# urgent-challenge/urgent2026_challenge_track1

Hardware: AMD Instinct MI355X
Metric: utterances/sec (4 s @ 48 kHz) train step (higher is better)
Workload: dtype bf16

## Files before the change

### include/urse.h

```cpp
#ifndef URSE_H_
#define URSE_H_
#include <stdint.h>

#ifdef __cplusplus
extern "C" {
#endif

#define URSE_OK 0
#define URSE_ERR_INVALID_ARG (-1)
#define URSE_ERR_LAUNCH (-2)
#define URSE_ERR_UNSUPPORTED (-3)
#define URSE_ERR_RUNTIME (-4)

#define URSE_F32 0
#define URSE_BF16 1
#define URSE_F16 2
#define URSE_BF16_ACT_F16 3

#define URSE_WIN_RECT 0
#define URSE_WIN_HANN 1

int urse_version(void);
const char* urse_last_error(void);

#define URSE_KV_NT_BRES 0
#define URSE_KV_NT_RING 1
#define URSE_KV_NT_RING_WIDE 2
#define URSE_KV_NT_128 3
#define URSE_KV_NT_GROUPED_RING 4
#define URSE_KV_NT_GROUPED_128 5
#define URSE_KV_TN_RING 6
#define URSE_KV_TN_RING_T 7
#define URSE_KV_TN_DUAL 8
#define URSE_KV_TN_128 9
#define URSE_KV_TN_GROUPED 10
#define URSE_KV_LSTM_FWD_STREAM 11
#define URSE_KV_LSTM_FWD_WIDE 12
#define URSE_KV_LSTM_FWD_CLUSTER 13
#define URSE_KV_LSTM_FWD_CLUSTER2 14
#define URSE_KV_LSTM_BWD_STREAM16 15
#define URSE_KV_LSTM_BWD_STREAM32 16
#define URSE_KV_LSTM_BWD_CLUSTER 17
#define URSE_KV_LSTM_BWD_SPLIT 18
#define URSE_KV_STFT960 19
#define URSE_KV_STFT_GENERIC 20
#define URSE_KV_ISTFT_GENERIC 21
#define URSE_KV_ISTFT960 22
#define URSE_KV_LSTM_FWD_RW 23
#define URSE_KV_TN_ACT_F16 24
#define URSE_KV_LSTM_FWD_RWX 25
#define URSE_KV_LSTM_BWD_NSPLIT 26
#define URSE_KV_LSTM_FWD_CLUSTERX 27
#define URSE_KV_COUNT 32
int urse_launch_count(int variant);
int urse_launch_counts_reset(void);

int urse_stft_fwd(const float* wav, const int32_t* lens, float* spec, int B, int L, int n_fft, int hop,
                  int window, void* stream);
int urse_istft_fwd(const float* spec, float* wav, int B, int T, int n_fft, int hop, int L_out, int window,
                   void* stream);
int urse_istft_bwd(const float* grad_wav, float* grad_spec, int B, int T, int n_fft, int hop, int L_out,
                   int window, void* stream);

int urse_gemm_nt(const void* A, int64_t lda, const void* B, int64_t ldb, void* C, int64_t ldc, const float* bias,
                 const float* resid, int64_t ldr, int64_t M, int64_t N, int64_t K, int in_dtype, int out_dtype,
                 int act, void* stream);
int urse_gemm_nt_gnstats(const void* A, int64_t lda, const void* B, int64_t ldb, float* C, int64_t ldc, const float* bias,
                         const float* resid, int64_t ldr, int64_t M, int64_t N, int64_t K, int in_dtype, int act,
                         double* stats, int64_t rows_per_group, void* stream);
int urse_gemm_nt_gnbwd(const void* A, int64_t lda, const void* B, int64_t ldb, float* C, int64_t M, int64_t N, int64_t K, int in_dtype,
                       const float* x, const double* stats, const float* gamma, double* sums, float* dgamma, float* dbeta, float* part,
                       int slots, int64_t rows_per_group, float eps, void* stream);
int urse_gemm_nt_grouped(const void* descs, int groups, int max_blocks, int in_dtype, int out_dtype, int act,
                         void* stream);
int urse_gemm_nt_grouped_h(const void* descs, const int64_t* host_descs, int groups, int in_dtype, int out_dtype,
                           int act, void* stream);
int urse_gemm_tn(const void* A, int64_t lda, const void* B, int64_t ldb, float* C, int64_t ldc, float* colsum,
                 int64_t R, int64_t Mo, int64_t No, int64_t shift, int64_t inner, int64_t period,
                 int64_t invalid_step, int64_t perm_h, int dtype, int target_workgroups, void* stream);
int urse_gemm_tn_act_f16_supported(int64_t R, int64_t Mo, int64_t No, int64_t No2, int with_colsum, int64_t inner, int64_t period);
int urse_gemm_tn_dual(const void* A, int64_t lda, const void* B, int64_t ldb, float* C, int64_t ldc, float* colsum,
                      const void* B2, int64_t ldb2, float* C2, int64_t ldc2, int64_t R, int64_t Mo, int64_t No, int64_t No2,
                      int64_t shift, int64_t inner, int64_t period, int64_t invalid_step, int64_t perm_h, int dtype,
                      int target_workgroups, void* stream);
int urse_gemm_tn_grouped(const void* descs, int groups, int max_blocks, int dtype, void* stream);

int urse_groupnorm_fwd(const float* x, const float* gamma, const float* beta, const float* add, void* y, double* stats,
                       int B, int T, int Kg, int W, int N, int Np, int gstride, float eps, int out_dtype, void* y_bf16, void* stream);
int urse_groupnorm_stats(const float* x, double* stats, int B, int T, int Kg, int W, int N, void* stream);
int urse_groupnorm_apply(const float* x, const float* gamma, const float* beta, const float* add, void* y, const double* stats,
                         int B, int T, int Kg, int W, int N, int Np, int gstride, float eps, int out_dtype, void* y_bf16, void* stream);
int urse_groupnorm_bwd(const float* x, const float* dy, const double* stats, const float* gamma, const float* dres,
                       float* dx, float* dgamma, float* dbeta, double* sums, int B, int T, int Kg, int W, int N,
                       int gstride, float eps, void* dx_packed, int ldp, void* stream);
int urse_groupnorm_bwd_apply(const float* x, const float* dy, const double* stats, const double* sums, const float* gamma,
                             const float* dres, float* dx, int B, int T, int Kg, int W, int N, int gstride, float eps, void* dx_packed,
                             int ldp, void* stream);
int urse_pack2d(const void* in, int64_t ldi, int in_dtype, void* out, int64_t ldo, int out_dtype, int rows, int cols,
                int out_rows, int out_cols, int transpose, void* stream);

int urse_pack_segments(const float* in, void* out, const void* segs, int nseg, int blocks_per_seg, int transpose,
                       int out_dtype, void* stream);

int urse_lstm_pack(const float* wih, const float* whh, const float* bih, const float* bhh, void* wih_p, void* wihT_p,
                   float* bias, void* whh_frag, void* whhT_frag, int N, int Np, int H, int Hp, int dtype,
                   void* stream);

int urse_lstm_bidir_fwd(void* gx, int64_t ldg, const void* whh, void* hout, int64_t ldh, float* c, int H, int Hp,
                        int n_seq, int seq_len, int64_t inner, int64_t outer, int64_t stride, int save, int dtype,
                        int rows16, void* hout_bf16, void* stream);
int urse_lstm_pack_quads(const float* whh, void* out, int H, int Hp, int dtype, void* stream);
int urse_lstm_cluster_plan(int H, int Hp, int n_seq, int reserved_cus, int64_t* plan);
int urse_lstm_cluster_fwd(void* gx, int64_t ldg, const void* whhq, void* hout, int64_t ldh, float* c, void* hx,
                          void* counters, void* err_flag, int H, int Hp, int n_seq, int seq_len, int64_t inner,
                          int64_t outer, int64_t stride, int save, int reserved_cus, int xcd_aware, int dtype, void* hout_bf16,
                          void* stream);
int urse_lstm_clusterx_supported(int N, int Np, int H, int Hp);
int urse_lstm_clusterx_plan(int H, int Hp, int n_seq, int reserved_cus, int64_t* plan);
int urse_lstm_clusterx_hx_elems(int H, int Hp, int n_seq, int reserved_cus, int64_t* elems);
int urse_lstm_pack_quads_x(const float* wih, void* out, int N, int Np, int H, int dtype, void* stream);
int urse_lstm_clusterx_fwd(const void* xn, int64_t ldx, const void* wihq, const float* bias, const void* whhq, void* gates, int64_t ldg, void* hout,
                           int64_t ldh, float* c, void* hx, void* counters, void* err_flag, int N, int Np, int H, int Hp, int n_seq, int seq_len,
                           int64_t inner, int64_t outer, int64_t stride, int save, int reserved_cus, int xcd_aware, int dtype, void* hout_bf16,
                           void* stream);
int urse_lstm_cluster2_plan(int H, int Hp, int n_seq, int reserved_cus, int64_t* plan);
int urse_lstm_cluster2_fwd(void* gx, int64_t ldg, const void* whhq, void* hout, int64_t ldh, float* c, void* hx, void* err_flag,
                           int H, int Hp, int n_seq, int seq_len, int64_t inner, int64_t outer, int64_t stride, int save,
                           int reserved_cus, int dtype, void* stream);
int urse_lstm_pack_bwd_quads(const float* whh, void* out, int H, int C, void* stream);
int urse_lstm_cluster_bwd(const void* dh, int64_t ldd, void* gates, int64_t ldg, const float* c, const void* whhTq,
                          void* dgx, void* counters, void* err_flag, int H, int Hp, int n_seq, int seq_len, int64_t inner,
                          int64_t outer, int64_t stride, int reserved_cus, void* stream);
int urse_lstm_wide_supported(int H, int Hp);
int urse_lstm_pack_blocks(const float* whh, void* out, int H, int Hp, void* stream);
int urse_lstm_wide_fwd(void* gx, int64_t ldg, const void* whhb, void* hout, int64_t ldh, float* c, int H, int Hp,
                       int n_seq, int seq_len, int64_t inner, int64_t outer, int64_t stride, int save, void* stream);
int urse_lstm_rw_supported(int H, int Hp);
int urse_lstm_pack_blocks_rw(const float* whh, void* out, int H, int Hp, void* stream);
int urse_lstm_rw_fwd(void* gx, int64_t ldg, const void* whhb, void* hout, int64_t ldh, float* c, int H, int Hp,
                     int n_seq, int seq_len, int64_t inner, int64_t outer, int64_t stride, int save,
                     int target_workgroups, int paired, void* stream);
int urse_lstm_pack_multi(const void* table, int n_lstm, int N, int Np, int H, int Hp, int dtype, void* stream);
int urse_lstm_pack_quads_multi(const void* table, int n_lstm, int H, int Hp, int dtype, void* stream);
int urse_lstm_pack_quads_x_multi(const void* table, int n_lstm, int N, int Np, int H, int dtype, void* stream);
int urse_lstm_pack_blocks_multi(const void* table, int n_lstm, int H, int Hp, void* stream);
int urse_lstm_pack_blocks_x_multi(const void* table, int n_lstm, int N, int Np, int H, int Hp, int dtype, void* stream);
int urse_lstm_rwx_supported(int N, int Np, int H, int Hp);
int urse_lstm_pack_blocks_x(const float* wih, const float* whh, void* out, int N, int Np, int H, int Hp, int dtype, void* stream);
int urse_lstm_rwx_fwd(const void* xn, int64_t ldx, const void* wx, const float* bias, void* gates, int64_t ldg, void* hout,
                      int64_t ldh, float* c, int N, int Np, int H, int Hp, int n_seq, int seq_len, int64_t inner,
                      int64_t outer, int64_t stride, int save, int target_workgroups, int dtype, void* hout_bf16, void* stream);
int urse_lstm_split_plan(int H, int n_seq, int reserved_cus, int64_t* plan);
int urse_lstm_split_bwd(const void* dh, int64_t ldd, void* gates, int64_t ldg, const float* c, const void* whhT, void* xbuf,
                        void* err_flag, int H, int n_seq, int seq_len, int64_t inner, int64_t outer, int64_t stride,
                        int reserved_cus, void* stream);
int urse_lstm_nsplit_plan(int H, int n_seq, int reserved_cus, int64_t* plan);
int urse_lstm_nsplit_bwd(const void* dh, int64_t ldd, void* gates, int64_t ldg, const float* c, const void* whhT, void* flags,
                         void* err_flag, int H, int n_seq, int seq_len, int64_t inner, int64_t outer, int64_t stride,
                         int reserved_cus, void* stream);
int urse_lstm_bidir_bwd(const void* dh, int64_t ldd, void* gates, int64_t ldg, const float* c, const void* whhT,
                        int H, int n_seq, int seq_len, int64_t inner, int64_t outer, int64_t stride, int dtype,
                        int rows16, void* stream);

int urse_bandsplit_norm_fwd(const float* spec, const int32_t* bands, const float* gamma, const float* beta, void* xnb,
                            double* stats, int B, int T, int F, int K, int ldx, float eps, int out_dtype,
                            void* xnb_bf16, void* stream);
int urse_bandsplit_norm_bwd(const float* spec, const float* dxnb, const int32_t* bands, const double* stats,
                            float* dgamma, float* dbeta, int B, int T, int F, int K, int ldx, float eps,
                            void* stream);
int urse_glu_mask_apply_fwd(const float* pre_m, const float* pre_r, const float* x, float* out,
                            const int32_t* bands, const int32_t* f2k, int64_t rows, int F, int ldp, void* stream);
int urse_glu_mask_apply_bwd(const float* pre_m, const float* pre_r, const float* x, const float* dout, void* dpre_m,
                            void* dpre_r, const int32_t* bands, const int32_t* f2k, int64_t rows, int F, int ldp,
                            int out_dtype, void* stream);
int urse_peak_normalize(float* x, int64_t n, float peak, void* scratch, void* stream);
int urse_nonsilence_power(const float* x, const int32_t* lens, int B, int64_t ld, double threshold, double* hop_scratch,
                          double* power, void* stream);
int urse_mix_noise(const float* speech, const float* noise_raw, const int32_t* noise_lens, int64_t ldn, const int32_t* lens,
                   const int32_t* offsets, const float* snr_db, int B, int64_t ld, float* noise_out, float* noisy_out,
                   double* scratch, void* stream);
int urse_fir_full(const float* x, const int32_t* lens, int B, int64_t ld, const float* taps, const int32_t* ntaps, int64_t ldt,
                  int taps_per_utt, float* y, void* stream);
int urse_fft_convolve_workspace_bytes(int B, int max_len, int max_ntaps, int64_t* bytes);
int urse_fft_convolve(const float* x, const int32_t* lens, int B, int64_t ld, const float* taps, const int32_t* ntaps, int64_t ldt,
                      int taps_per_utt, float* y, int max_len, int max_ntaps, void* workspace, int64_t workspace_bytes, void* stream);
int urse_filtfilt_fir(const float* x, const int32_t* lens, int B, int64_t ld, const float* taps, const int32_t* ntaps_dev,
                      int ntaps, float* y, float* scratch, int64_t lds, void* stream);
int urse_quantile_clip(float* x, const int32_t* lens, int B, int64_t ld, const float* qmin, const float* qmax, float* bounds,
                       void* stream);
int urse_zero_segments(float* x, int64_t ld, const int32_t* segments, int nseg, void* stream);
int urse_resample_table(const float* x, int64_t ldx, float* y, int64_t ldy, const double* win, const double* delta, int nwin, int P,
                        int n_orig, int n_out, double time_increment, double scale, int num_table, int index_step, void* stream);
int urse_joint_peak_scale(float* speech, float* noisy, float* noise, int B, int64_t ld, float target, void* peak_scratch,
                          void* stream);
int urse_wind_mix(float* speech, const float* x, float* noise, float* noisy, const int32_t* lens, int B, int64_t ld, const int32_t* rows,
                  int nrows, const double* params, double* c_out, void* stream);
int urse_wind_chunk(void);
int urse_axpby(const float* x, float* y, float a, float b, int64_t n, void* stream);
int urse_nan_to_num(const float* x, float* y, int64_t n, void* stream);
int urse_scale_by_device_scalar(float* x, const float* s, int64_t n, void* stream);

int urse_pair_sums(const float* target, const float* estimate, double* sums, int B, int L, void* stream);
int urse_mrl1_loss_fwd(const float* target, const float* estimate, float* loss, float* G, double* sums, double* acc,
                       int B, int L, const int32_t* windows, int n_windows, float eps, float td_weight, void* stream);
int urse_mrl1_loss_bwd(const float* target, const float* estimate, const float* G, const double* sums,
                       const float* grad_loss, float* grad_estimate, double* c1, int B, int L, float eps,
                       void* stream);
int urse_mrl1_loss_bwd_guarded(const float* target, const float* estimate, const float* G, const double* sums,
                               const float* grad_loss, const float* loss, float* grad_estimate, double* c1, int B,
                               int L, float eps, void* stream);
int urse_sisnr_fwd(const float* ref, const float* inf, float* loss, double* sums, int B, int L, void* stream);
int urse_grad_sumsq(const float* g, double* out, int64_t n, void* stream);
int urse_clip_adamw_step(float* params, float* grads, float* exp_avg, float* exp_avg_sq, int64_t n,
                         const double* normsq, float max_norm, float lr, float beta1, float beta2, float eps,
                         float weight_decay, int step, float grad_scale, int zero_grad, void* stream);
int urse_clip_adamw_step_slots(float* params, float* grads, float* exp_avg, float* exp_avg_sq, int64_t n,
                               const double* normsq, float max_norm, float lr, float beta1, float beta2, float eps,
                               float weight_decay, const uint8_t* slot, float* used, int32_t* steps, float* bias_corr,
                               int n_slot, const uint32_t* skip_flag, float grad_scale, int zero_grad, void* stream);
int urse_fill_used_flags(float* used, int n_slot, int n_used, void* stream);

int urse_fft_resample_plan_elems(int n, int64_t* elems, int64_t* tmp_elems);
int urse_fft_resample_plan(void* plan, void* tmp, int n, void* stream);
int urse_fft_resample_workspace_bytes(int P, int n, int num, int64_t* bytes);
int urse_fft_resample(const float* x, int64_t ldx, float* y, int64_t ldy, const void* plan_n, const void* plan_num,
                      void* workspace, int64_t workspace_bytes, int P, int n, int num, void* stream);
int urse_resample_poly(const float* x, float* y, const double* h_padded, int hlen, int P, int L, int Lout, int up,
                       int down, int n_pre_remove, void* stream);
int urse_estoi_batch(const float* ref10k, const float* inf10k, float* out, float* ws_x, float* ws_y, float* tob_x,
                     float* tob_y, int32_t* lens, const float* tw512, int P, int L, void* stream);
int urse_sdr_batch(const float* ref, const float* est, float* out, double* acf, double* xcorr, double* norms, int P,
                   int L, float clamp_db, void* stream);

int urse_power_spectrum_workspace_bytes(int64_t rows, int max_len, int n_fft, int hop, int64_t* bytes);
int urse_power_spectrum_mean(const float* wav, int64_t ld, const int32_t* lens, float* mean_power, int64_t rows,
                             int max_len, int n_fft, int hop, void* workspace, int64_t workspace_bytes, void* stream);
int urse_bandwidth_pick(const float* mean_power, const int32_t* row_start, int32_t* bin, int P, int F,
                        double threshold_db, void* stream);

int urse_spec_transform(const float* x, float* y, int64_t n_complex, float exponent, float factor, int inverse,
                        void* stream);
int urse_flow_prepare(const float* x0, const float* y, const float* z, const float* t, float* xt, float* cvf, int B,
                      int64_t per_b, float sigma_min, float sigma_max, void* stream);
int urse_axpy(const float* x, float* y, float a, int64_t n, void* stream);
int urse_time_embedding(const float* t, const float* W, float* out, int B, int half, void* stream);
int urse_conv5x5_fwd(const float* U, const float* W, const float* bias, float* pre, int B, int T, int F, void* stream);
int urse_conv5x5_bwd(const float* U, const float* W, const float* dpre, float* dU, float* dW, float* dbias, int B, int T,
                     int F, void* stream);
int urse_glu4_apply_fwd(const float* pre_m, const float* pre_r, const float* x, float* out, int64_t rows, int F,
                        int Fs, float sign, void* stream);
int urse_glu4_apply_bwd(const float* pre_m, const float* pre_r, const float* x, const float* dout, float* dpre_m,
                        float* dpre_r, int64_t rows, int F, int Fs, float sign, void* stream);
int urse_tanh_bwd_pack(const float* dU, const float* U, void* dst, int64_t rows, int n, int64_t ldd, int out_dtype,
                       void* stream);
int urse_flow_loss(const float* vf, const float* cvf, double* loss, float* grad, int B, int64_t per_b, float grad_scale,
                   void* stream);
int urse_ema_update(float* shadow, const float* params, float one_minus_decay, int64_t n, void* stream);

#define URSE_PESQ_TRACE 286
int urse_pesq_workspace_bytes(int pairs, int L, int fs, int64_t* bytes);
int urse_pesq_batch(const float* ref, const float* deg, int64_t ld, const int32_t* lens, int pairs, int L, int fs, int wb,
                    float* mos, float* raw, int32_t* trace, void* workspace, int64_t workspace_bytes, void* stream);

int urse_flac_info(const void* data, int64_t nbytes, int64_t* info);
int urse_flac_decode(const void* data, int64_t nbytes, int32_t* out, int64_t capacity_frames, int64_t* decoded);

int urse_pcm16_from_f32(const float* x, int64_t ldx, const int32_t* lens, int16_t* pcm, int64_t ldp, int64_t rows,
                        int max_len, float scale, void* stream);
int urse_flac_encode_workspace_bytes(const int32_t* lens, int P, int blocksize, int64_t* info);
int urse_flac_encode(const int16_t* pcm, int64_t total_samples, const int64_t* starts, const int32_t* lens,
                     const int32_t* rates, int P, int channels, int bits, int blocksize, void* workspace,
                     int64_t workspace_bytes, void* out, int64_t out_capacity, int64_t* file_bytes, int32_t* frame_bytes,
                     void* stream);

int urse_diag_stream(void* buf, float* sink, int64_t bytes, int width, int write, void* stream);

#ifdef __cplusplus
}
#endif
#endif
```

### urgent2026_challenge_track1_amd/bsrnn.py

```python
import math
import os

import numpy as np
import torch
import torch.nn as nn

from . import ops
from ._lib import call, stream_ptr

SUBBANDS_481 = tuple([5] + [4] * 19 + [10] * 6 + [40] * 7 + [60])
SUBBANDS_769 = tuple([5] + [4] * 26 + [10] * 10 + [50] * 10 + [60])
_DIAG_SKIP_WGRADS = os.environ.get("URSE_DIAG_SKIP_WGRADS", "0") == "1"
GN_EPS = 1e-5


def _ptr(t, off_elems=0):
    return t.data_ptr() + off_elems * t.element_size()


class _PackPlan:

    def __init__(self, transpose):
        self.transpose = transpose
        self.segs = []
        self.size = 0
        self._table = None
        self._out = {}

    def add(self, in_off, in_rows, in_cols, out_rows, out_cols):
        off = self.size
        self.segs.append([in_off, in_rows, in_cols, in_cols, off, out_rows, out_cols, out_cols])
        self.size += (out_rows * out_cols + 31) // 32 * 32
        return (off, out_rows, out_cols)

    def reserve(self, n):
        off = self.size
        self.size += (n + 31) // 32 * 32
        return off

    def add_at(self, in_off, in_rows, in_cols, out_off, out_rows, out_cols, out_ld):
        self.segs.append([in_off, in_rows, in_cols, in_cols, out_off, out_rows, out_cols, out_ld])

    def run(self, flat, dtype):
        if not self.segs:
            return None
        if self._table is None or self._table.device != flat.device:
            self._table = torch.tensor(self.segs, dtype=torch.int64, device=flat.device)
        key = (dtype, flat.device)
        if key not in self._out:
            self._out[key] = torch.empty(self.size, dtype=dtype, device=flat.device)
        out = self._out[key]
        big = max(s[5] * s[6] for s in self.segs)
        call("pack_segments", flat, out, self._table, len(self.segs), max(1, min(64, (big + 2047) // 2048)),
             int(self.transpose), ops._dt(out), stream_ptr())
        return out


def _view(buf, h):
    off, r, c = h
    return buf[off:off + r * c].view(r, c)


def _empty_padded(K, M, ld, n, dtype, device):
    t = torch.empty(K, M, ld, dtype=dtype, device=device)
    if ld > n:
        t[:, :, n:].zero_()
    return t


def nt_grouped(rows, device, in_dt, out_dt, act=0):
    host = np.asarray(rows, dtype=np.int64)
    assert host.ndim == 2 and host.shape[1] == 12
    call("gemm_nt_grouped_h", ops.upload(torch.from_numpy(host), device), host.ctypes.data, host.shape[0], in_dt, out_dt, act,
         stream_ptr())


class BSRNNCore(nn.Module):

    def __init__(self, input_dim=481, num_channel=16, num_layer=6, target_fs=48000, causal=False, num_spk=1,
                 compute_dtype=torch.bfloat16):
        super().__init__()
        if causal or num_spk != 1:
            raise NotImplementedError("the reference uses causal=False, num_spk=1 (models/bsrnn.py:27-34)")
        if target_fs != 48000 or input_dim not in (481, 769):
            raise NotImplementedError("band tables defined for input_dim 481 / 769 @ 48 kHz (bsrnn_flowse.py:23-40)")
        if num_channel % 4:
            raise ValueError("num_channel must be a multiple of 4")
        self.subbands = SUBBANDS_481 if input_dim == 481 else SUBBANDS_769
        self.input_dim, self.N, self.H, self.num_layer = input_dim, num_channel, 2 * num_channel, num_layer
        self.compute_dtype = compute_dtype
        N, H = self.N, self.H
        self._make_front_back()
        self.norm_time = nn.ModuleList([nn.GroupNorm(1, N) for _ in range(num_layer)])
        self.rnn_time = nn.ModuleList([nn.LSTM(N, H, batch_first=True, bidirectional=True) for _ in range(num_layer)])
        self.fc_time = nn.ModuleList([nn.Linear(2 * H, N) for _ in range(num_layer)])
        self.norm_freq = nn.ModuleList([nn.GroupNorm(1, N) for _ in range(num_layer)])
        self.rnn_freq = nn.ModuleList([nn.LSTM(N, H, batch_first=True, bidirectional=True) for _ in range(num_layer)])
        self.fc_freq = nn.ModuleList([nn.Linear(2 * H, N) for _ in range(num_layer)])
        self._flat = None
        self._flat_grad = None
        self._off = {}
        self._plans = None
        self._tables = {}
        self._packed = None
        self._packed_version = -1
        self.param_version = 0
        self.grad_ready_hook = None
        self._deferred, self._inflight, self._side = [], None, None
        self._grad_pack = None
        self._gn_stats = None

    def _make_band_split(self):
        bs = nn.Module()
        bs.norm = nn.ModuleList([nn.GroupNorm(1, 2 * sb) for sb in self.subbands])
        bs.fc = nn.ModuleList([nn.Conv1d(2 * sb, self.N, 1) for sb in self.subbands])
        return bs

    def _make_front_back(self):
        N = self.N
        self.band_split = self._make_band_split()
        md = nn.Module()
        mk = lambda sb: nn.Sequential(nn.GroupNorm(1, N), nn.Conv1d(N, 4 * N, 1), nn.Tanh(),
                                      nn.Conv1d(4 * N, 4 * sb, 1), nn.GLU(dim=1))
        md.mlp_mask = nn.ModuleList([mk(sb) for sb in self.subbands])
        md.mlp_residual = nn.ModuleList([mk(sb) for sb in self.subbands])
        self.mask_decoder = md

    @staticmethod
    def _bs_params(prefix, bs):
        return [(prefix + ".gamma", [m.weight for m in bs.norm]), (prefix + ".beta", [m.bias for m in bs.norm]),
                (prefix + ".w", [m.weight for m in bs.fc]), (prefix + ".b", [m.bias for m in bs.fc])]

    def _front_params(self):
        return self._bs_params("bs", self.band_split)

    def _back_params(self):
        order = []
        for tag, mlps in (("m", self.mask_decoder.mlp_mask), ("r", self.mask_decoder.mlp_residual)):
            p = "md%s." % tag
            order += [(p + "gamma", [s[0].weight for s in mlps]), (p + "beta", [s[0].bias for s in mlps]),
                      (p + "w1", [s[1].weight for s in mlps]), (p + "b1", [s[1].bias for s in mlps]),
                      (p + "w2", [s[3].weight for s in mlps]), (p + "b2", [s[3].bias for s in mlps])]
        return order

    back_tag = "md"
    band_groups = ("bs", "mdm", "mdr")

    def _ordered_params(self):
        L = self.num_layer
        order = list(self._front_params())
        for l in range(L):
            for path, norm, rnn, fc in (("t", self.norm_time[l], self.rnn_time[l], self.fc_time[l]),
                                        ("f", self.norm_freq[l], self.rnn_freq[l], self.fc_freq[l])):
                p = "l%d%s." % (l, path)
                order += [(p + "gamma", [norm.weight]), (p + "beta", [norm.bias]),
                          (p + "wih", [rnn.weight_ih_l0, rnn.weight_ih_l0_reverse]),
                          (p + "bih", [rnn.bias_ih_l0, rnn.bias_ih_l0_reverse]),
                          (p + "bhh", [rnn.bias_hh_l0, rnn.bias_hh_l0_reverse]),
                          (p + "whh", [rnn.weight_hh_l0, rnn.weight_hh_l0_reverse]),
                          (p + "wfc", [fc.weight]), (p + "bfc", [fc.bias])]
        return order + list(self._back_params())

    def _ensure_flat(self):
        first = next(self.parameters())
        if self._flat is not None and self._flat.device == first.device and \
                first.data_ptr() == self._flat.data_ptr() + 4 * self._first_off:
            return
        order = self._ordered_params()
        total = 0
        offs = {}
        plist = []
        for name, ps in order:
            total = (total + 3) // 4 * 4
            offs[name] = total
            for p in ps:
                plist.append((p, total))
                total += p.numel()
        assert len(plist) == len([q for q in self.parameters() if q.requires_grad])
        nb = len(self.subbands)
        slot = np.zeros(total, dtype=np.uint8)
        for name, ps in order:
            if len(ps) == nb and name.split(".")[0] in self.band_groups:
                o = offs[name]
                for k, q in enumerate(ps):
                    slot[o:o + q.numel()] = 1 + k
                    o += q.numel()
        self.n_slot = 1 + nb
        self._slot_map = torch.from_numpy(slot).to(first.device)
        flat = torch.zeros(total, dtype=torch.float32, device=first.device)
        self._n_params = total
        grad = torch.zeros(total + (self.n_slot + 3) // 4 * 4, dtype=torch.float32, device=first.device)
        with torch.no_grad():
            for p, o in plist:
                flat[o:o + p.numel()].copy_(p.data.reshape(-1).float())
                p.data = flat[o:o + p.numel()].view(p.shape)
                p.grad = grad[o:o + p.numel()].view(p.shape)
        self._flat, self._flat_grad, self._off = flat, grad, offs
        self._first_off = [o for p, o in plist if p is first][0]
        self._plans = None
        self._packed_version = -1
        self._tables = {}

    @property
    def flat_params(self):
        self._ensure_flat()
        return self._flat

    @property
    def flat_grads(self):
        self._ensure_flat()
        return self._flat_grad

    @property
    def used_flags(self):
        self._ensure_flat()
        return self._flat_grad[self._n_params:self._n_params + self.n_slot]

    @property
    def slot_map(self):
        self._ensure_flat()
        return self._slot_map

    def mark_used_bands(self, K):
        call("fill_used_flags", self.used_flags, self.n_slot, 1 + K, stream_ptr())

    def grad_groups(self):
        self._ensure_flat()
        names = list(self._off.keys())
        ends = [self._off[n] for n in names[1:]] + [self._flat_grad.numel()]
        spans = {n: (self._off[n], e - self._off[n]) for n, e in zip(names, ends)}
        groups = []

        def span(ns):
            lo = min(spans[n][0] for n in ns)
            hi = max(spans[n][0] + spans[n][1] for n in ns)
            return lo, hi - lo
        is_layer = lambda n: n[0] == "l" and n[1].isdigit()
        first = min(i for i, n in enumerate(names) if is_layer(n))
        last = max(i for i, n in enumerate(names) if is_layer(n))
        groups.append((self.back_tag,) + span(names[last + 1:]))
        for l in reversed(range(self.num_layer)):
            groups.append(("l%df" % l,) + span([n for n in names if n.startswith("l%df." % l)]))
            groups.append(("l%dt" % l,) + span([n for n in names if n.startswith("l%dt." % l)]))
        groups.append(("bs",) + span(names[:first]))
        return groups

    def _g(self, name, numel=None, off=0):
        o = self._off[name] + off
        n = numel if numel is not None else 0
        return self._flat_grad[o:o + n] if numel is not None else self._flat_grad[o:]

    def _p(self, name, numel, off=0):
        o = self._off[name] + off
        return self._flat[o:o + numel]

    def _ready(self, tag):
        if self.grad_ready_hook is not None:
            self.grad_ready_hook(tag)

    def _build_plans(self, dtype):
        N, H = self.N, self.H
        Np, Hp = ops.kpad(N, dtype), ops.kpad(ops.pad_to(H, 16), dtype)
        ld2H, ld4N = ops.kpad(2 * H, dtype), ops.kpad(4 * N, dtype)
        pn, pt = _PackPlan(False), _PackPlan(True)
        h = {}
        o = self._off
        self._dims = dict(Np=Np, Hp=Hp, ld2H=ld2H, ld4N=ld4N)
        self._plan_front(pn, pt, h, dtype)
        for l in range(self.num_layer):
            for path in "tf":
                p = "l%d%s." % (l, path)
                h[p + "wfc"] = pn.add(o[p + "wfc"], N, 2 * H, N, ld2H)
                h[p + "wfcT"] = pt.add(o[p + "wfc"], N, 2 * H, 2 * H, Np)
        self._plan_back(pn, pt, h, dtype)
        self._plans = (dtype, pn, pt, h)

    def _plan_band_split(self, prefix, pn, pt, h, dtype):
        N, Np, o = self.N, self._dims["Np"], self._off
        w_off = 0
        for k, sb in enumerate(self.subbands):
            xpad = ops.kpad(2 * sb, dtype)
            h[prefix + ".w", k] = pn.add(o[prefix + ".w"] + w_off, N, 2 * sb, N, xpad)
            h[prefix + ".wT", k] = pt.add(o[prefix + ".w"] + w_off, N, 2 * sb, 2 * sb, Np)
            w_off += N * 2 * sb

    def _plan_front(self, pn, pt, h, dtype):
        self._plan_band_split("bs", pn, pt, h, dtype)

    def _plan_back(self, pn, pt, h, dtype):
        N, Np, ld4N, o = self.N, self._dims["Np"], self._dims["ld4N"], self._off
        for tag in "mr":
            p = "md%s." % tag
            w2_off = 0
            for k, sb in enumerate(self.subbands):
                ppad = ops.kpad(4 * sb, dtype)
                h[p + "w1", k] = pn.add(o[p + "w1"] + k * 4 * N * N, 4 * N, N, 4 * N, Np)
                h[p + "w1T", k] = pt.add(o[p + "w1"] + k * 4 * N * N, 4 * N, N, N, ld4N)
                h[p + "w2", k] = pn.add(o[p + "w2"] + w2_off, 4 * sb, 4 * N, 4 * sb, ld4N)
                h[p + "w2T", k] = pt.add(o[p + "w2"] + w2_off, 4 * sb, 4 * N, 4 * N, ppad)
                w2_off += 4 * sb * 4 * N

    @property
    def bwd_dtype(self):
        return ops.bwd_dtype(self.compute_dtype)

    def _prepare(self):
        self._ensure_flat()
        dtype = self.compute_dtype
        if self._plans is None or self._plans[0] != dtype:
            self._build_plans(dtype)
            self._packed_version = -1
        if self._packed_version == self.param_version:
            return
        _, pn, pt, h = self._plans
        bn, bt = pn.run(self._flat, dtype), pt.run(self._flat, self.bwd_dtype)
        H = self.H
        pk = {}
        for key, hd in h.items():
            name = key[0] if isinstance(key, tuple) else key
            pk[key] = _view(bt if name.endswith("T") else bn, hd)
        N, d = self.N, self._dims
        if not hasattr(self, "_lstm_bufs") or self._lstm_bufs.get("key") != (dtype, self._flat.device):
            self._lstm_bufs = {"key": (dtype, self._flat.device)}
        names = ["l%d%s." % (l, path) for l in range(self.num_layer) for path in "tf"]
        srcs = {p: (self._p(p + "wih", 8 * H * N), self._p(p + "whh", 8 * H * H), self._p(p + "bih", 8 * H), self._p(p + "bhh", 8 * H))
                for p in names}
        lays = {path: ops.lstm_layouts(H, d["Hp"], N, d["Np"], dtype, path) for path in "tf"}
        multi = ops.PACK_MULTI and self._flat.is_cuda and all(
            p in self._lstm_bufs and lays[p[-2]] <= self._lstm_bufs[p].keys() and lays[p[-2]] <= ops.PACK_MULTI_LAYOUTS for p in names)
        if multi:
            self._lstm_bufs["table"] = ops.lstm_pack_multi([srcs[p] + (self._lstm_bufs[p],) for p in names], N, H, dtype,
                                                           table=self._lstm_bufs.get("table"))
        for p in names:
            lp = self._lstm_bufs[p] if multi else ops.lstm_pack(*srcs[p], N, H, dtype, out=self._lstm_bufs.get(p), layouts=lays[p[-2]])
            self._lstm_bufs[p] = lp
            pk.update((p + k, v) for k, v in lp.items() if torch.is_tensor(v))
        self._packed = pk
        self._packed_version = self.param_version

    def _band_tables(self, F, dtype, device):
        key = (F, dtype, device)
        if key in self._tables:
            return self._tables[key]
        rows, f2k = [], [-1] * F
        f0 = xoff = poff = 0
        K = 0
        for k, sb in enumerate(self.subbands):
            if 2 * sb > 128:
                raise ValueError("band %d is %d bins wide: the band split's affine backward covers one (re, im) column per thread of "
                                 "its 128-thread blocks, 64 bins at the most" % (k, sb))
            xpad, ppad = ops.kpad(2 * sb, dtype), ops.kpad(4 * sb, dtype)
            rows.append([f0, sb, xoff, xpad, 2 * f0, poff, ppad, 0])
            for f in range(f0, min(F, f0 + sb)):
                f2k[f] = k
            f0 += sb
            xoff += xpad
            poff += ppad
            K = k + 1
            if f0 >= F:
                break
        tb = dict(K=K, rows=rows, ldx=xoff, P=poff,
                  bands=torch.tensor(rows, dtype=torch.int32, device=device),
                  f2k=torch.tensor(f2k, dtype=torch.int32, device=device))
        self._tables[key] = tb
        return tb

    def bandsplit_fwd(self, spec, prefix="bs", out=None, width=None, col0=0, save=True):
        B, T, F, _ = spec.shape
        dt, dev, N = self.compute_dtype, spec.device, self.N
        tb = self._band_tables(F, dt, dev)
        K, pk = tb["K"], self._packed
        n_gb = 2 * sum(self.subbands)
        xnb = torch.empty(B * T, tb["ldx"], dtype=dt, device=dev)
        xnb_b = torch.empty_like(xnb, dtype=torch.bfloat16) if (save and dt == torch.float16) else None
        stats = torch.empty(B * K * 2, dtype=torch.float64, device=dev)
        call("bandsplit_norm_fwd", spec, tb["bands"], self._p(prefix + ".gamma", n_gb), self._p(prefix + ".beta", n_gb),
             xnb, stats, B, T, F, K, tb["ldx"], GN_EPS, ops._dt(xnb), xnb_b, stream_ptr())
        if out is None:
            out, width = torch.empty(B, T, K, N, dtype=torch.float32, device=dev), N
        M = B * T
        rows = []
        for k in range(K):
            r = tb["rows"][k]
            w = pk[prefix + ".w", k]
            rows.append([_ptr(xnb, r[2]), _ptr(w), _ptr(out, k * width + col0),
                         _ptr(self._flat, self._off[prefix + ".b"] + k * N), 0,
                         tb["ldx"], w.shape[1], K * width, M, N, r[3], 0])
        nt_grouped(rows, dev, ops._dt(xnb), ops._dt(out))
        return out, ((xnb_b if xnb_b is not None else xnb), stats, tb)

    def bandsplit_bwd(self, spec, saved, dz, prefix="bs", dzT=None, width=None, col0=0, ready=True):
        xnb, stats, tb = saved
        B, T, F, _ = spec.shape
        dt, dev, N = self.bwd_dtype, spec.device, self.N
        K, pk, Np = tb["K"], self._packed, self._dims["Np"]
        M = B * T
        tail_overlap = ops.TN_OVERLAP and ops.TN_OVERLAP_TAIL and spec.is_cuda and bool(self._deferred)
        if tail_overlap:
            self._run_deferred_wgrads(dev, 256)
        else:
            self._flush_deferred_wgrads()
        if dzT is None:
            dzT, width = ops.pack2d(dz.reshape(M * K, N), M * K, Np, dt), Np
        dxnb = torch.empty(M, tb["ldx"], dtype=torch.float32, device=dev)
        rows, tn_rows = [], []
        w_off = 0
        for k in range(K):
            r = tb["rows"][k]
            sb = r[1]
            a = dzT.view(M, K * width)[:, k * width + col0:k * width + col0 + Np]
            gw = self._g(prefix + ".w", N * 2 * sb, w_off).view(N, 2 * sb)
            tn_rows.append(ops.tn_desc(a, xnb[:, r[2]:r[2] + r[3]], gw, colsum=self._g(prefix + ".b", N, k * N), Mo=N,
                                       No=2 * sb))
            wT = pk[prefix + ".wT", k]
            rows.append([_ptr(dzT, k * width + col0), _ptr(wT), _ptr(dxnb, r[2]), 0, 0, K * width, Np, tb["ldx"], M,
                         2 * sb, Np, 0])
            w_off += N * 2 * sb
        ops.gemm_tn_grouped(tn_rows, dt, dev)
        nt_grouped(rows, dev, ops._dt(dzT), ops.F32)
        n_gb = 2 * sum(self.subbands)
        call("bandsplit_norm_bwd", spec, dxnb, tb["bands"], stats, self._g(prefix + ".gamma", n_gb),
             self._g(prefix + ".beta", n_gb), B, T, F, K, tb["ldx"], GN_EPS, stream_ptr())
        if tail_overlap:
            self._flush_deferred_wgrads()
        if ready:
            self._ready("bs")

    def _seqmap(self, path, B, T, K):
        if path == "t":
            return dict(n_seq=B * K, seq_len=T, inner=K, outer=T * K, stride=K)
        return dict(n_seq=B * T, seq_len=K, inner=1, outer=K, stride=1)

    def dualpath_fwd(self, skip, l, path, save, temb=None):
        B, T, K, N = skip.shape
        H, dt, pk, d = self.H, self.compute_dtype, self._packed, self._dims
        p = "l%d%s." % (l, path)
        M = B * T * K
        pre = self._gn_stats[1] if (self._gn_stats is not None and self._gn_stats[0].data_ptr() == skip.data_ptr() and
                                    self._gn_stats[0].shape == skip.shape) else None
        self._gn_stats = None
        sm = self._seqmap(path, B, T, K)
        two = save and dt == torch.float16
        if two and ops.tn_act_f16_supported(M, N, 2 * H, 0, True) and \
                ops.tn_act_f16_supported(M, 4 * H, N, H, True, sm["stride"], sm["seq_len"]):
            two = False
        xn, stats, xn_b = ops.groupnorm_fwd(skip, self._p(p + "gamma", N), self._p(p + "beta", N), B, T, 1, K * N, N,
                                            d["Np"], 0, dt, GN_EPS, add=temb, stats=pre, bf16_copy=two or None)
        Hp = d["Hp"]
        kern = ops.lstm_fwd_kernel(H, Hp, N, d["Np"], dt, path, sm, two)
        if kern == "clusterx":
            r = ops.lstm_fwd_clusterx(xn, pk[p + "wihq"], pk[p + "whhq"], pk[p + "bias"], N, H, Hp, save=save, bf16_copy=two, **sm)
            gx, hout, c, self._cluster_err = r[:4]
        elif kern == "rwx":
            r = ops.lstm_fwd_rwx(xn, pk[p + "wx"], pk[p + "bias"], N, H, Hp, save=save, bf16_copy=two, **sm)
            gx, hout, c = r[:3]
        else:
            gx = ops.gemm_nt(xn, pk[p + "wih"], pk[p + "bias"])
            if kern == "cluster2":
                r = ops.lstm_fwd_cluster2(gx, pk[p + "whhq"], H, Hp, save=save, **sm)
            elif kern == "cluster":
                r = ops.lstm_fwd_cluster(gx, pk[p + "whhq"], H, Hp, save=save, bf16_copy=two, **sm)
            elif kern == "rw":
                r = ops.lstm_fwd_rw(gx, pk[p + "whhb"], H, Hp, save=save, **sm)
            elif kern == "wide":
                r = ops.lstm_fwd_wide(gx, pk[p + "whhb"], H, Hp, save=save, **sm)
            else:
                r = ops.lstm_fwd(gx, pk[p + "whh"], H, Hp, save=save, bf16_copy=two, **sm)
            hout, c = r[:2]
            if kern in ("cluster2", "cluster"):
                self._cluster_err = r[2]
            if dt == torch.float16:
                gx = gx.view(torch.bfloat16)
        hout_b = r[-1] if two else None
        out = torch.empty_like(skip)
        if ops.FUSE_GN_STATS and dt in ops.HALF_TYPES and N % 4 == 0 and not (path == "f" and l == self.num_layer - 1):
            _, st = ops.gemm_nt(hout, pk[p + "wfc"], self._p(p + "bfc", N), resid=skip.view(M, N), out=out.view(M, N), gn_rows=T * K)
            self._gn_stats = (out, st)
        else:
            ops.gemm_nt(hout, pk[p + "wfc"], self._p(p + "bfc", N), resid=skip.view(M, N), out=out.view(M, N))
        return out, ((stats, xn_b, gx, c, (hout_b if hout_b is not None else hout)) if save else None)

    def dualpath_bwd(self, skip, saved, l, path, dout):
        stats, xn, gates, c, hout = saved
        B, T, K, N = skip.shape
        H, dt, pk, d = self.H, self.bwd_dtype, self._packed, self._dims
        p = "l%d%s." % (l, path)
        M = B * T * K
        dout2 = dout.reshape(M, N)
        if self._grad_pack is not None and self._grad_pack[0] == dout.data_ptr() and self._grad_pack[1].shape == (M, d["Np"]):
            doT = self._grad_pack[1]
        else:
            doT = ops.pack2d(dout2, M, d["Np"], dt)
        self._grad_pack = None
        dh = torch.empty(M, d["ld2H"], dtype=dt, device=skip.device)
        ops.gemm_nt(doT, pk[p + "wfcT"], out=dh, N=2 * H)
        sm = self._seqmap(path, B, T, K)
        overlap = ops.TN_OVERLAP and skip.is_cuda
        limit = None if path == "t" else ops.TN_BAND_PARTS
        shadow = overlap and (path == "t" or ops.TN_OVERLAP_BAND) and bool(self._deferred) and limit != 0
        with ops.reserve_cus(co_resident=ops.wgrad_shadow_wgs(path, False) if shadow else None):
            kern = ops.lstm_bwd_kernel(H, d["Hp"], N, d["Np"], self.compute_dtype, path, sm)
        if shadow:
            self._run_deferred_wgrads(skip.device, ops.wgrad_shadow_wgs(path, kern == "nsplit"), limit)
        if kern == "cluster":
            dg, self._cluster_err = ops.lstm_bwd_cluster(dh, gates, c, pk[p + "whhTq"], H, d["Hp"], **sm)
        elif kern == "split":
            dg, self._cluster_err = ops.lstm_bwd_split(dh, gates, c, pk[p + "whhT"], H, **sm)
        elif kern == "nsplit":
            dg, self._cluster_err = ops.lstm_bwd_nsplit(dh, gates, c, pk[p + "whhT"], H, **sm)
        else:
            dg = ops.lstm_bwd(dh, gates, c, pk[p + "whhT"], H, rows16=ops.BWD_ROWS16.get(path, 0), **sm)
        if overlap and path == "t":
            self._join_deferred_wgrads(keep=ops.TN_JOIN_LAG)
        st, L = sm["stride"], sm["seq_len"]
        tag = "l%d%s" % (l, path)

        def wg_fc(target_wgs=0):
            if _DIAG_SKIP_WGRADS:
                return
            ops.gemm_tn(doT, hout, self._g(p + "wfc", N * 2 * H).view(N, 2 * H), colsum=self._g(p + "bfc", N), Mo=N, No=2 * H,
                        target_wgs=target_wgs)

        def wg_dir(dr, sh, inv, last):
            def run(target_wgs=0):
                if _DIAG_SKIP_WGRADS:
                    return
                gb = self._g(p + "bih", 8 * H)
                gwih = self._g(p + "wih", 8 * H * N).view(8 * H, N)
                ops.gemm_tn_dual(dg[:, dr * 4 * H:(dr + 1) * 4 * H], xn, gwih[dr * 4 * H:(dr + 1) * 4 * H],
                                 gb[dr * 4 * H:(dr + 1) * 4 * H], hout[:, dr * H:(dr + 1) * H],
                                 self._g(p + "whh", 4 * H * H, dr * 4 * H * H).view(4 * H, H), 4 * H, N, H, sh, st, L, inv,
                                 perm_h=H, target_wgs=target_wgs)
                if last:
                    call("axpby", gb, self._g(p + "bhh", 8 * H), 1.0, 1.0, 8 * H, stream_ptr())
            return run

        parts = [(wg_fc, None), (wg_dir(0, -st, 0, False), None), (wg_dir(1, st, L - 1, True), tag)]
        if overlap:
            self._deferred.extend(parts)
        else:
            for fn, _ in parts:
                fn()
        gn_sums = None
        if ops.FUSE_GN_BWD and ops.gemm_nt_gnbwd_supported(M, N, dg.shape[1], T * K, dt):
            dxn, gn_sums = ops.gemm_nt_gnbwd(dg, pk[p + "wihT"], N, skip, stats, self._p(p + "gamma", N), self._g(p + "gamma", N),
                                             self._g(p + "beta", N), T * K, GN_EPS)
        else:
            dxn = ops.gemm_nt(dg, pk[p + "wihT"], out_dtype=torch.float32, N=N)
        if dt == torch.bfloat16 and N % 4 == 0:
            dskip, packed = ops.groupnorm_bwd(skip, dxn, stats, self._p(p + "gamma", N), dout, self._g(p + "gamma", N),
                                              self._g(p + "beta", N), B, T, 1, K * N, N, 0, GN_EPS, pack_ld=d["Np"], sums=gn_sums)
            self._grad_pack = (dskip.data_ptr(), packed)
        else:
            dskip = ops.groupnorm_bwd(skip, dxn, stats, self._p(p + "gamma", N), dout, self._g(p + "gamma", N),
                                      self._g(p + "beta", N), B, T, 1, K * N, N, 0, GN_EPS)
        if not overlap:
            self._ready(tag)
        return dskip

    def _run_deferred_wgrads(self, device, target_wgs, limit=None):
        if not self._deferred or limit == 0:
            return
        now, later = (self._deferred, []) if limit is None else (self._deferred[:limit], self._deferred[limit:])
        if self._side is None:
            self._side = ops.low_priority_stream(device)
        start = torch.cuda.Event()
        start.record(torch.cuda.current_stream())
        self._side.wait_event(start)
        with torch.cuda.stream(self._side):
            for fn, _ in now:
                fn(target_wgs)
            done = torch.cuda.Event()
            done.record(self._side)
        self._inflight = (self._inflight or []) + [(done, now)]
        self._deferred = later
        ops.CO_RESIDENT_WGS = target_wgs

    def _join_deferred_wgrads(self, keep=0):
        if self._inflight is None:
            return
        n = len(self._inflight) - keep
        if n <= 0:
            return
        batches, rest = self._inflight[:n], self._inflight[n:]
        self._inflight = rest or None
        if not rest:
            ops.CO_RESIDENT_WGS = 0
        for done, items in batches:
            torch.cuda.current_stream().wait_event(done)
            for _, tag in items:
                if tag is not None:
                    self._ready(tag)

    def _flush_deferred_wgrads(self):
        self._join_deferred_wgrads()
        items, self._deferred = self._deferred, []
        for fn, tag in items:
            fn()
            if tag is not None:
                self._ready(tag)

    def maskdec_fwd(self, skip, spec, save):
        B, T, K, N = skip.shape
        F = spec.shape[2]
        dt, dev, pk, d = self.compute_dtype, skip.device, self._packed, self._dims
        tb = self._band_tables(F, dt, dev)
        assert tb["K"] == K
        M, Np, ld4N, P = B * T, d["Np"], d["ld4N"], tb["P"]
        Kf = len(self.subbands)
        xns, sts, hids, pres, keep = [], [], [], [], []
        rows1, rows2 = [], []
        for tag in "mr":
            p = "md%s." % tag
            two = save and dt == torch.float16
            if two:
                xn, st, xn_b = ops.groupnorm_fwd(skip, self._p(p + "gamma", Kf * N), self._p(p + "beta", Kf * N), B, T, K, N, N,
                                                 Np, N, dt, GN_EPS, bf16_copy=True)
            else:
                xn, st = ops.groupnorm_fwd(skip, self._p(p + "gamma", Kf * N), self._p(p + "beta", Kf * N), B, T, K, N, N,
                                           Np, N, dt, GN_EPS)
                xn_b = xn
            hid = _empty_padded(K, M, ld4N, 4 * N, dt, dev)
            hid_b = _empty_padded(K, M, ld4N, 4 * N, torch.bfloat16, dev) if two else hid
            pre = torch.empty(M, P, dtype=torch.float32, device=dev)
            b2_off = 0
            for k in range(K):
                sb = self.subbands[k]
                r = tb["rows"][k]
                w1, w2 = pk[p + "w1", k], pk[p + "w2", k]
                rows1.append([_ptr(xn, k * Np), _ptr(w1), _ptr(hid, k * M * ld4N),
                              _ptr(self._flat, self._off[p + "b1"] + k * 4 * N), _ptr(hid_b, k * M * ld4N) if two else 0, K * Np, Np, ld4N, M, 4 * N, Np,
                              ld4N if two else 0])
                rows2.append([_ptr(hid, k * M * ld4N), _ptr(w2), _ptr(pre, r[5]),
                              _ptr(self._flat, self._off[p + "b2"] + b2_off), 0, ld4N, ld4N, P, M, 4 * sb, ld4N, 0])
                b2_off += 4 * sb
            xns.append(xn_b); sts.append(st); hids.append(hid_b); pres.append(pre)
            keep += [xn, hid]
        fdt = ops.dtype_code(dt)
        nt_grouped(rows1, dev, fdt, fdt, act=1)
        nt_grouped(rows2, dev, fdt, ops.F32)
        del keep
        out = torch.empty(B, T, F, 2, dtype=torch.float32, device=dev)
        call("glu_mask_apply_fwd", pres[0], pres[1], spec, out, tb["bands"], tb["f2k"], M, F, P, stream_ptr())
        return out, ((xns, sts, hids, pres, tb) if save else None)

    def maskdec_bwd(self, skip, spec, saved, dout):
        xns, sts, hids, pres, tb = saved
        B, T, K, N = skip.shape
        F = spec.shape[2]
        dt, dev, pk, d = self.bwd_dtype, skip.device, self._packed, self._dims
        M, Np, ld4N, P = B * T, d["Np"], d["ld4N"], tb["P"]
        Kf = len(self.subbands)
        dpre = [torch.zeros(M, P, dtype=dt, device=dev) for _ in range(2)]
        call("glu_mask_apply_bwd", pres[0], pres[1], spec, dout, dpre[0], dpre[1], tb["bands"], tb["f2k"], M, F, P,
             ops._dt(dpre[0]), stream_ptr())
        dhp = [_empty_padded(K, M, ld4N, 4 * N, dt, dev) for _ in range(2)]
        dxn = [torch.empty(M * K, N, dtype=torch.float32, device=dev) for _ in range(2)]
        rows_a, rows_b = [], []
        for i, tag in enumerate("mr"):
            p = "md%s." % tag
            for k in range(K):
                r = tb["rows"][k]
                rows_a.append([_ptr(dpre[i], r[5]), _ptr(pk[p + "w2T", k]), _ptr(dhp[i], k * M * ld4N), 0,
                               _ptr(hids[i], k * M * ld4N), P, r[6], ld4N, M, 4 * N, r[6], ld4N])
                rows_b.append([_ptr(dhp[i], k * M * ld4N), _ptr(pk[p + "w1T", k]), _ptr(dxn[i], k * N), 0, 0, ld4N,
                               ld4N, K * N, M, N, ld4N, 0])
        nt_grouped(rows_a, dev, ops._dt(dpre[0]), ops._dt(dhp[0]), act=2)
        tn_rows = []
        for i, tag in enumerate("mr"):
            p = "md%s." % tag
            w2_off = b2_off = 0
            for k in range(K):
                sb = self.subbands[k]
                r = tb["rows"][k]
                tn_rows.append(ops.tn_desc(dpre[i][:, r[5]:r[5] + r[6]], hids[i][k],
                                           self._g(p + "w2", 16 * sb * N, w2_off).view(4 * sb, 4 * N),
                                           colsum=self._g(p + "b2", 4 * sb, b2_off), Mo=4 * sb, No=4 * N))
                xk = xns[i].view(M, K * Np)[:, k * Np:(k + 1) * Np]
                tn_rows.append(ops.tn_desc(dhp[i][k], xk, self._g(p + "w1", 4 * N * N, k * 4 * N * N).view(4 * N, N),
                                           colsum=self._g(p + "b1", 4 * N, k * 4 * N), Mo=4 * N, No=N))
                w2_off += 16 * sb * N
                b2_off += 4 * sb
        defer_md = ops.TN_OVERLAP and ops.DEFER_MASKDEC_WGRADS and skip.is_cuda
        if defer_md:
            keep = (dpre, hids, dhp, xns)

            def wg_md(target_wgs=0, _rows=tn_rows, _keep=keep):
                ops.gemm_tn_grouped(_rows, dt, dev)
            self._deferred.append((wg_md, "md"))
        else:
            ops.gemm_tn_grouped(tn_rows, dt, dev)
        nt_grouped(rows_b, dev, ops._dt(dhp[0]), ops.F32)
        dskip = None
        for i, tag in enumerate("mr"):
            p = "md%s." % tag
            last = i == 1 and dt == torch.bfloat16 and N % 4 == 0
            dskip = ops.groupnorm_bwd(skip, dxn[i].view(B, T, K, N), sts[i], self._p(p + "gamma", Kf * N), dskip,
                                      self._g(p + "gamma", Kf * N), self._g(p + "beta", Kf * N), B, T, K, N, N, N,
                                      GN_EPS, pack_ld=Np if last else 0)
            if last:
                dskip, packed = dskip
                self._grad_pack = (dskip.data_ptr(), packed)
        if not defer_md:
            self._ready("md")
        return dskip

    def forward(self, spec_ri):
        ops.require_cuda(spec_ri)
        self._prepare()
        if self._inflight is not None or self._deferred:
            if self._side is not None:
                torch.cuda.current_stream().wait_stream(self._side)
        self._deferred, self._inflight, self._grad_pack = [], None, None
        ops.CO_RESIDENT_WGS = 0
        ops.COMM_RESERVED_CUS = 0
        spec_ri = spec_ri.contiguous().float()
        train = torch.is_grad_enabled() and any(p.requires_grad for p in self.parameters())
        if not train:
            z, _ = self.bandsplit_fwd(spec_ri, save=False)
            for l in range(self.num_layer):
                z, _ = self.dualpath_fwd(z, l, "t", False)
                z, _ = self.dualpath_fwd(z, l, "f", False)
            out = self.maskdec_fwd(z, spec_ri, False)[0]
            ops.poll_kernel_errors(spec_ri.device, sync=True)
            return out
        ops.poll_kernel_errors(spec_ri.device)
        anchor = self._flat.new_zeros((), requires_grad=True)
        self.mark_used_bands(self._band_tables(spec_ri.shape[2], self.compute_dtype, spec_ri.device)["K"])
        z = _BandSplitFn.apply(anchor, spec_ri, self)
        for l in range(self.num_layer):
            z = _DualPathFn.apply(z, self, l, "t")
            z = _DualPathFn.apply(z, self, l, "f")
        return _MaskDecFn.apply(z, spec_ri, self)


class _BandSplitFn(torch.autograd.Function):
    @staticmethod
    def forward(ctx, anchor, spec, core):
        z, saved = core.bandsplit_fwd(spec)
        ctx.core, ctx.saved, ctx.spec = core, saved, spec
        return z

    @staticmethod
    def backward(ctx, dz):
        ctx.core.bandsplit_bwd(ctx.spec, ctx.saved, dz.contiguous())
        ctx.saved = None
        return None, None, None


class _DualPathFn(torch.autograd.Function):
    @staticmethod
    def forward(ctx, skip, core, l, path, temb=None):
        out, saved = core.dualpath_fwd(skip, l, path, True, temb)
        ctx.core, ctx.saved, ctx.skip, ctx.l, ctx.path = core, saved, skip, l, path
        return out

    @staticmethod
    def backward(ctx, dout):
        d = ctx.core.dualpath_bwd(ctx.skip, ctx.saved, ctx.l, ctx.path, dout.contiguous())
        ctx.saved = None
        return d, None, None, None, None


class _MaskDecFn(torch.autograd.Function):
    @staticmethod
    def forward(ctx, skip, spec, core):
        out, saved = core.maskdec_fwd(skip, spec, True)
        ctx.core, ctx.saved, ctx.skip, ctx.spec = core, saved, skip, spec
        return out

    @staticmethod
    def backward(ctx, dout):
        d = ctx.core.maskdec_bwd(ctx.skip, ctx.spec, ctx.saved, dout.contiguous())
        ctx.saved = None
        return d, None, None


class BSRNNSeparator(nn.Module):

    def __init__(self, input_dim, num_spk=1, num_channels=16, num_layers=6, target_fs=48000, causal=True,
                 compute_dtype=torch.bfloat16):
        super().__init__()
        self.bsrnn = BSRNNCore(input_dim, num_channels, num_layers, target_fs, causal, num_spk, compute_dtype)

    def forward(self, input, ilens=None, additional=None):
        spec_ri = torch.view_as_real(input) if input.is_complex() else input
        out = self.bsrnn(spec_ri)
        return [torch.view_as_complex(out)], ilens, {}


class _StftCfg(nn.Module):

    def __init__(self, n_fft, hop_length, default_fs):
        super().__init__()
        self.n_fft, self.hop_length, self.default_fs = n_fft, hop_length, default_fs
        self.output_dim = n_fft // 2 + 1

    def reconfig(self, fs):
        if fs is None:
            return self.n_fft, self.hop_length
        fs = int(fs)
        return self.n_fft * fs // self.default_fs, self.hop_length * fs // self.default_fs


class BSRNN_SE(nn.Module):

    def __init__(self, num_channel=192, num_layer=6, compute_dtype=torch.bfloat16):
        super().__init__()
        self.encoder = _StftCfg(960, 480, 48000)
        self.decoder = _StftCfg(960, 480, 48000)
        self.bsrnn = BSRNNSeparator(self.encoder.output_dim, 1, num_channel, num_layer, 48000, False, compute_dtype)

    @property
    def core(self):
        return self.bsrnn.bsrnn

    def forward(self, speech_mix, speech_lengths, fs):
        ops.require_cuda(speech_mix)
        n_fft, hop = self.encoder.reconfig(fs)
        lens = torch.as_tensor(speech_lengths)
        feature_mix = ops.stft_forward(speech_mix.float(), n_fft, hop, ops.WIN_HANN, lens)
        feature_pre, _, _ = self.bsrnn(feature_mix, None, None)
        enhanced_feature = feature_pre[0]
        n_fft_d, hop_d = self.decoder.reconfig(fs)
        enhanced_wav = ops.istft_forward(enhanced_feature, n_fft_d, hop_d, int(lens.max()))
        return enhanced_wav, enhanced_feature
```

### urgent2026_challenge_track1_amd/csrc/lstm.hip

```cpp
#include <type_traits>

#include "urse_common.h"

namespace urse {

typedef __bf16 bf16x8_t __attribute__((ext_vector_type(8)));
typedef float f32x4_t __attribute__((ext_vector_type(4)));

struct SeqMap {
  long inner, outer, stride;
  int n_seq, seq_len;
};

struct LstmFwdArgs {
  void* gx; long ldg;
  const void* whh;
  void* hout; long ldh;
  void* hout2;
  float* c;
  int H, Hp, save;
  int xcd;
  SeqMap m;
};

struct LstmBwdArgs {
  const void* dh; long ldd;
  void* gates; long ldg;
  const float* c;
  const void* whhT;
  int H;
  int dbuf;
  int xcd;
  SeqMap m;
};

template <typename T> struct Vec4;
template <> struct Vec4<bf16_t> {
  typedef uint2 raw;
  static __device__ __forceinline__ void unpack(raw v, float (&o)[4]) {
    o[0] = __uint_as_float(v.x << 16); o[1] = __uint_as_float(v.x & 0xffff0000u);
    o[2] = __uint_as_float(v.y << 16); o[3] = __uint_as_float(v.y & 0xffff0000u);
  }
  static __device__ __forceinline__ raw pack(const float (&i)[4]) {
    raw v;
    v.x = (unsigned)f32_to_bf16(i[0]) | ((unsigned)f32_to_bf16(i[1]) << 16);
    v.y = (unsigned)f32_to_bf16(i[2]) | ((unsigned)f32_to_bf16(i[3]) << 16);
    return v;
  }
};
template <> struct Vec4<f16_t> {
  typedef uint2 raw;
  static __device__ __forceinline__ void unpack(raw v, float (&o)[4]) { unpack2<f16_t>(v.x, o[0], o[1]); unpack2<f16_t>(v.y, o[2], o[3]); }
  static __device__ __forceinline__ raw pack(const float (&i)[4]) {
    raw v;
    v.x = pack2<f16_t>(i[0], i[1]);
    v.y = pack2<f16_t>(i[2], i[3]);
    return v;
  }
};
template <> struct Vec4<float> {
  typedef float4 raw;
  static __device__ __forceinline__ void unpack(raw v, float (&o)[4]) { o[0] = v.x; o[1] = v.y; o[2] = v.z; o[3] = v.w; }
  static __device__ __forceinline__ raw pack(const float (&i)[4]) { return make_float4(i[0], i[1], i[2], i[3]); }
};

template <typename T, int RT>
__device__ __forceinline__ void mma_slab(const uint4 (&a)[RT], const uint4& b, f32x4_t (&acc)[RT]) {
  if constexpr (sizeof(T) == 2) {
#pragma unroll
    for (int rt = 0; rt < RT; ++rt) acc[rt] = mfma16<T>(a[rt], b, acc[rt]);
  } else {
    const float bf[4] = {__uint_as_float(b.x), __uint_as_float(b.y), __uint_as_float(b.z), __uint_as_float(b.w)};
#pragma unroll
    for (int rt = 0; rt < RT; ++rt) {
      const float af[4] = {__uint_as_float(a[rt].x), __uint_as_float(a[rt].y), __uint_as_float(a[rt].z),
                           __uint_as_float(a[rt].w)};
#pragma unroll
      for (int s = 0; s < 4; ++s) acc[rt] = __builtin_amdgcn_mfma_f32_16x16x4f32(af[s], bf[s], acc[rt], 0, 0, 0);
    }
  }
}

template <typename T, int RT, int MAXUT, int NW>
__global__ void __launch_bounds__(NW * 64) lstm_fwd_kernel(LstmFwdArgs p) {
  constexpr int NTHR = NW * 64;
  extern __shared__ __attribute__((aligned(16))) char smem[];
  constexpr int ES = sizeof(T), R = 16 * RT;
  typedef typename Vec4<T>::raw V4;
  typedef typename std::conditional<__is_same(T, f16_t), bf16_t, T>::type TS;
  const int tid = threadIdx.x, lane = tid & 63, w = tid >> 6, lr = lane >> 4, lc = lane & 15;
  int dir, tile_;
  xcd_dir_tile(p.xcd, dir, tile_);
  const int s0 = tile_ * R;
  const int H = p.H, Hp = p.Hp, nut = (H + 15) >> 4;
  const int pitch = lds_frag_pitch(Hp * ES);
  for (int i = tid; i < 2 * R * pitch / 4; i += NTHR) reinterpret_cast<unsigned*>(smem)[i] = 0u;

  float cst[MAXUT][RT][4];
#pragma unroll
  for (int a = 0; a < MAXUT; ++a)
#pragma unroll
    for (int b = 0; b < RT; ++b)
#pragma unroll
      for (int c = 0; c < 4; ++c) cst[a][b][c] = 0.f;
  int rowbase[RT][4];
  bool rvalid[RT][4];
#pragma unroll
  for (int rt = 0; rt < RT; ++rt)
#pragma unroll
    for (int r = 0; r < 4; ++r) {
      int seq = s0 + rt * 16 + lr * 4 + r;
      rvalid[rt][r] = seq < p.m.n_seq;
      if (seq >= p.m.n_seq) seq = p.m.n_seq - 1;
      rowbase[rt][r] = (int)((seq / p.m.inner) * p.m.outer + (seq % p.m.inner));
    }
  const int nslab = Hp * ES / 64;
  const char* whh = reinterpret_cast<const char*>(p.whh) + ((long)dir * nut * nslab * 4) * 1024 + lane * 16;
  T* gx = reinterpret_cast<T*>(p.gx);
  T* hout = reinterpret_cast<T*>(p.hout);
  const long gcol0 = (long)dir * 4 * H;
  __syncthreads();

  for (int step = 0; step < p.m.seq_len; ++step) {
    const int t = dir ? (p.m.seq_len - 1 - step) : step;
    char* hc = smem + (step & 1) * R * pitch;
    char* hn = smem + ((step & 1) ^ 1) * R * pitch;
    const long toff = (long)t * p.m.stride;
#pragma unroll
    for (int ui = 0; ui < MAXUT; ++ui) {
      const int ut = w + NW * ui;
      if (ut < nut) {
        const int u = ut * 16 + lc;
        const bool uvalid = u < H;
        const int uc = uvalid ? u : H - 1;
        V4 gxv[RT][4];
#ifndef ABL_NO_PW
#pragma unroll
        for (int rt = 0; rt < RT; ++rt)
#pragma unroll
          for (int r = 0; r < 4; ++r)
            gxv[rt][r] = *reinterpret_cast<const V4*>(gx + ((long)rowbase[rt][r] + toff) * p.ldg + gcol0 + uc * 4);
#endif
        f32x4_t acc[4][RT];
#pragma unroll
        for (int g = 0; g < 4; ++g)
#pragma unroll
          for (int rt = 0; rt < RT; ++rt) acc[g][rt] = f32x4_t{0.f, 0.f, 0.f, 0.f};
        const char* wr = whh + ((long)ut * nslab * 4) * 1024;
        const char* ar = hc + lc * pitch + 16 * lr;
#ifndef URSE_FWD_KB
#define URSE_FWD_KB 3
#endif
        constexpr int KB = (RT == 1 && sizeof(T) == 2) ? URSE_FWD_KB : 3;
        for (int k0 = 0; k0 < nslab; k0 += KB) {
          uint4 b[KB][4];
#pragma unroll
          for (int i = 0; i < KB; ++i) {
            const int ks = (k0 + i < nslab) ? k0 + i : nslab - 1;
#pragma unroll
            for (int g = 0; g < 4; ++g) b[i][g] = *reinterpret_cast<const uint4*>(wr + (ks * 4 + g) * 1024);
          }
#pragma unroll
          for (int i = 0; i < KB; ++i) {
            if (k0 + i < nslab) {
              uint4 a[RT];
#pragma unroll
              for (int rt = 0; rt < RT; ++rt)
                a[rt] = *reinterpret_cast<const uint4*>(ar + rt * 16 * pitch + (k0 + i) * 64);
#pragma unroll
              for (int g = 0; g < 4; ++g) mma_slab<T, RT>(a, b[i][g], acc[g]);
            }
          }
        }
#pragma unroll
        for (int rt = 0; rt < RT; ++rt)
#pragma unroll
          for (int r = 0; r < 4; ++r) {
            const long row = (long)rowbase[rt][r] + toff;
            float pre[4] = {0.f, 0.f, 0.f, 0.f};
#ifndef ABL_NO_PW
            Vec4<T>::unpack(gxv[rt][r], pre);
#endif
            const float iv = sigmoidf_(acc[0][rt][r] + pre[0]), fv = sigmoidf_(acc[1][rt][r] + pre[1]);
            const float gv = tanhf_(acc[2][rt][r] + pre[2]), ov = sigmoidf_(acc[3][rt][r] + pre[3]);
            const float cv = fv * cst[ui][rt][r] + iv * gv;
            cst[ui][rt][r] = cv;
            const float hv = uvalid ? ov * tanhf_(cv) : 0.f;
            const T hT = from_f32<T>(hv);
            *reinterpret_cast<T*>(hn + (rt * 16 + lr * 4 + r) * pitch + u * ES) = hT;
#ifdef ABL_NO_PW
            if (rvalid[rt][r] && uvalid && step == p.m.seq_len - 1) {
#else
            if (rvalid[rt][r] && uvalid) {
#endif
              hout[row * p.ldh + (long)dir * H + u] = hT;
              if constexpr (__is_same(T, f16_t)) {
                if (p.hout2) reinterpret_cast<bf16_t*>(p.hout2)[row * p.ldh + (long)dir * H + u] = f32_to_bf16(to_f32<T>(hT));
              }
              if (p.save) {
                const float act[4] = {iv, fv, gv, ov};
                *reinterpret_cast<V4*>(gx + row * p.ldg + gcol0 + u * 4) = Vec4<TS>::pack(act);
                p.c[row * 2 * H + (long)dir * H + u] = cv;
              }
            }
          }
      }
    }
    __syncthreads();
  }
}

#ifndef URSE_BWD_PRIO
#define URSE_BWD_PRIO 0
#endif
#ifdef BWSTAMP
__device__ unsigned long long g_bwstamps[512 * 16];
#define BWST(slot) do { if (stamp_on && step < 512) { const unsigned long long t_ = __builtin_amdgcn_s_memtime(); if (lane == 0) g_bwstamps[step * 16 + (slot)] = t_; } } while (0)
#else
#define BWST(slot) do { } while (0)
#endif
#pragma clang diagnostic push
#pragma clang diagnostic ignored "-Winline-asm"
__device__ __forceinline__ void bw_glds16(const char* gsrc, unsigned dst) {
  asm volatile("s_mov_b32 m0, %1\n\ts_nop 0\n\tglobal_load_lds_dwordx4 %0, off" :: "v"(gsrc), "s"(dst) : "memory", "m0");
}
#pragma clang diagnostic pop
template <typename T, int RT, int MAXUT, int NW, int HC = 0, int HPC = 0, int PF = 0, int STG = 0, int KH = 1>
__global__ void __launch_bounds__(NW * 64) lstm_bwd_kernel(LstmBwdArgs p) {
  static_assert(KH == 1 || (KH == 2 && !HC && !HPC && !PF && !STG), "the half-tile form exists for the plain variant only");
#ifdef BWSTAMP
  const bool stamp_on = blockIdx.x == BWSTAMP && (threadIdx.x >> 6) == 0;
#endif
#if URSE_BWD_PRIO
  __builtin_amdgcn_s_setprio(URSE_BWD_PRIO);
#endif
  extern __shared__ __attribute__((aligned(16))) char smem[];
  constexpr int ES = sizeof(T), R = 16 * RT;
  typedef typename Vec4<T>::raw V4;
  const int tid = threadIdx.x, lane = tid & 63, w = tid >> 6, lr = lane >> 4, lc = lane & 15;
  int dir, tile_;
  xcd_dir_tile(p.xcd, dir, tile_);
  const int s0 = tile_ * R;
  const int H = HC ? HC : p.H, nut = (H + 15) >> 4, G4 = 4 * H;
  const int pitch = HPC ? lds_frag_pitch(4 * HPC * ES) : lds_frag_pitch(G4 / KH * ES);
  const int nbuf = (p.dbuf && KH == 1) ? 2 : 1;
  float dcs[MAXUT][RT][4], dhr[MAXUT][RT][4], ccur[MAXUT][RT][4];
  int rowbase[RT][4];
#pragma unroll
  for (int rt = 0; rt < RT; ++rt)
#pragma unroll
    for (int r = 0; r < 4; ++r) {
      int seq = s0 + rt * 16 + lr * 4 + r;
      const bool ok = seq < p.m.n_seq;
      if (!ok) seq = p.m.n_seq - 1;
      const int rb = (int)((seq / p.m.inner) * p.m.outer + (seq % p.m.inner));
      rowbase[rt][r] = ok ? rb : -rb - 1;
    }
  auto rowb = [&](int rt, int r) -> long { return rowbase[rt][r] >= 0 ? rowbase[rt][r] : -(rowbase[rt][r] + 1); };
  if constexpr (STG) {
    int* rowtab = reinterpret_cast<int*>(smem + nbuf * R * pitch);
    if (tid < R) {
      const int seq = s0 + tid;
      rowtab[tid] = seq < p.m.n_seq ? (int)((seq / p.m.inner) * p.m.outer + (seq % p.m.inner)) : -1;
    }
  }
  const int nslab = G4 * ES / 64;
  const char* whhT = reinterpret_cast<const char*>(p.whhT) + ((long)dir * nut * nslab) * 1024 + lane * 16;
  const T* dh = reinterpret_cast<const T*>(p.dh);
  T* gates = reinterpret_cast<T*>(p.gates);
  const int ldg_i = (int)p.ldg, ldd_i = (int)p.ldd, ldc_i = 2 * H, stride_i = (int)p.m.stride;
#ifdef BABL_ALIGNED
  const int gcol_i = 0, hcol_i = 0, prev_i = dir ? stride_i : -stride_i;
#else
  const int gcol_i = dir * G4, hcol_i = dir * H, prev_i = dir ? stride_i : -stride_i;
#endif

  {
    const long toff0 = (long)(dir ? 0 : p.m.seq_len - 1) * p.m.stride;
#pragma unroll
    for (int ui = 0; ui < MAXUT; ++ui) {
      const int u = (w + NW * ui) * 16 + lc;
      const int uc = u < H ? u : H - 1;
#pragma unroll
      for (int rt = 0; rt < RT; ++rt)
#pragma unroll
        for (int r = 0; r < 4; ++r) {
          dcs[ui][rt][r] = 0.f;
          dhr[ui][rt][r] = 0.f;
          ccur[ui][rt][r] = p.c[(rowb(rt, r) + toff0) * 2 * H + (long)dir * H + uc];
        }
    }
  }
  constexpr int PU = PF == 3 ? 2 : (PF == 4 ? 1 : (PF ? MAXUT : 1));
  static_assert(PF != 4 || (STG && RT == 2 && sizeof(T) == 2 && KH == 1 && HPC), "PF 4: the 32-row staged-store bf16 form (row table in LDS)");
  V4 gpf[PU][RT][4];
  float cpf[PU][RT][4];
  T dhpf[PU][RT][4];
  V4 dgk[KH == 2 ? MAXUT : 1][RT][4];
  auto load_step = [&](int ui, int slot, int tt) {
    const int u = (w + NW * ui) * 16 + lc;
    const bool first_ = dir ? (tt == p.m.seq_len - 1) : (tt == 0);
#pragma unroll
    for (int rt = 0; rt < RT; ++rt)
#pragma unroll
      for (int r = 0; r < 4; ++r) {
#ifdef BABL_HOT_INPUTS
#if BABL_HOT_INPUTS >= 2
        const int row = (int)rowb(rt, r) + (p.m.seq_len / 2) * stride_i + 0 * tt;
#else
        const int row = rt * 16 + lr * 4 + r + 0 * tt;
#endif
#else
        const int row = (int)rowb(rt, r) + tt * stride_i;
#endif
#ifdef BABL_NO_P1LOAD
        gpf[slot][rt][r] = V4{}; cpf[slot][rt][r] = (float)row; dhpf[slot][rt][r] = T(row & 1);
#else
#ifdef BABL_NO_G
        gpf[slot][rt][r] = V4{};
#else
        gpf[slot][rt][r] = *reinterpret_cast<const V4*>(gates + ((long)row * ldg_i + (gcol_i + u * 4)));
#endif
#ifdef BABL_NO_C
        cpf[slot][rt][r] = (float)row;
#else
#ifdef BABL_HOT_INPUTS
        cpf[slot][rt][r] = first_ ? 0.f : p.c[(long)row * ldc_i + (hcol_i + u)];
#else
        cpf[slot][rt][r] = first_ ? 0.f : p.c[(long)(row + prev_i) * ldc_i + (hcol_i + u)];
#endif
#endif
#ifdef BABL_NO_DH
        dhpf[slot][rt][r] = T(row & 1);
#else
        dhpf[slot][rt][r] = dh[(long)row * ldd_i + (hcol_i + u)];
#endif
#endif
      }
  };
  auto load_all = [&](int tt) {
#pragma unroll
    for (int ui = 0; ui < MAXUT; ++ui)
      if ((w + NW * ui) * 16 + lc < H) load_step(ui, PF ? ui : 0, tt);
  };
  char* pfb = smem + nbuf * R * pitch + R * (int)sizeof(int) + w * 7168;
  const unsigned pfb_u = __builtin_amdgcn_readfirstlane((unsigned)(size_t)(__attribute__((address_space(3))) char*)pfb);
  auto dma_tile = [&](int ui, int tt) __attribute__((always_inline)) {
    const int utd = __builtin_amdgcn_readfirstlane(w) + NW * ui;
    int opq = 0;
    asm volatile("" : "+v"(opq));
    const int* rowtab = reinterpret_cast<const int*>(smem + nbuf * R * pitch);
    const int ln = lane + opq;
    const int toff_ = tt * stride_i;
    const bool first_ = dir ? (tt == p.m.seq_len - 1) : (tt == 0);
    const int nu = H - utd * 16 < 16 ? H - utd * 16 : 16;
    {
      const int ch = ln & 7, chc = ch < nu / 2 ? ch : nu / 2 - 1;
#pragma unroll
      for (int i = 0; i < 4; ++i) {
        int grow = rowtab[i * 8 + (ln >> 3)];
        grow = grow < 0 ? rowtab[0] : grow;
        bw_glds16(reinterpret_cast<const char*>(gates) + ((long)(grow + toff_) * ldg_i + (gcol_i + utd * 64)) * 2 + chc * 16, __builtin_amdgcn_readfirstlane(pfb_u + (unsigned)i * 1024u));
      }
    }
    {
      const int ch = ln & 3, chc = ch < nu / 4 ? ch : nu / 4 - 1;
#pragma unroll
      for (int i = 0; i < 2; ++i) {
        int grow = rowtab[i * 16 + (ln >> 2)];
        grow = grow < 0 ? rowtab[0] : grow;
        const int crow = grow + toff_ + (first_ ? 0 : prev_i);
        bw_glds16(reinterpret_cast<const char*>(p.c) + ((long)crow * ldc_i + (hcol_i + utd * 16)) * 4 + chc * 16, __builtin_amdgcn_readfirstlane(pfb_u + 4096u + (unsigned)i * 1024u));
      }
    }
    {
      const int ch = ln & 1, chc = ch < nu / 8 ? ch : nu / 8 - 1;
      int grow = rowtab[ln >> 1];
      grow = grow < 0 ? rowtab[0] : grow;
      bw_glds16(reinterpret_cast<const char*>(dh) + ((long)(grow + toff_) * ldd_i + (hcol_i + utd * 16)) * 2 + chc * 16, __builtin_amdgcn_readfirstlane(pfb_u + 6144u));
    }
  };
  if constexpr (PF == 1) load_all(dir ? 0 : p.m.seq_len - 1);
  if constexpr (PF == 4) __syncthreads();
  for (int step = 0; step < p.m.seq_len; ++step) {
    const int t = dir ? step : (p.m.seq_len - 1 - step);
    char* tile = smem + (step % nbuf) * R * pitch;
    BWST(0);
    if constexpr (PF == 2) load_all(t);
    if constexpr (PF == 3) {
      if (w * 16 + lc < H) load_step(0, 0, t);
    }
#pragma unroll
    for (int ui = 0; ui < MAXUT; ++ui) {
      const int ut = w + NW * ui;
      if (ut < nut) {
        const int u = ut * 16 + lc;
        if constexpr (PF == 4) {
          if ((ui & 1) == 0) {
            if (ui + 1 < MAXUT && w + NW * (ui + 1) < nut) dma_tile(ui + 1, t);
          } else {
            asm volatile("s_waitcnt vmcnt(0)" ::: "memory");
          }
        }
        if (u < H) {
          if constexpr (!PF) load_step(ui, 0, t);
          if constexpr (PF == 4) {
            if ((ui & 1) == 0) {
              load_step(ui, 0, t);
            } else {
              const bool first_ = dir ? (t == p.m.seq_len - 1) : (t == 0);
#pragma unroll
              for (int rt = 0; rt < RT; ++rt)
#pragma unroll
                for (int r = 0; r < 4; ++r) {
                  const int lrow = rt * 16 + lr * 4 + r;
                  gpf[0][rt][r] = *reinterpret_cast<const V4*>(pfb + lrow * 128 + lc * 8);
                  cpf[0][rt][r] = first_ ? 0.f : *reinterpret_cast<const float*>(pfb + 4096 + lrow * 64 + lc * 4);
                  dhpf[0][rt][r] = *reinterpret_cast<const T*>(pfb + 6144 + lrow * 32 + lc * 2);
                }
            }
          }
          if constexpr (PF == 3) {
            if (ui + 1 < MAXUT && (w + NW * (ui + 1)) * 16 + lc < H) load_step(ui + 1, (ui + 1) & 1, t);
          }
          const int SL = PF == 3 ? (ui & 1) : ((PF && PF != 4) ? ui : 0);
          V4 (&gpre)[RT][4] = gpf[SL];
          float (&cpre)[RT][4] = cpf[SL];
          T (&dhpre)[RT][4] = dhpf[SL];
#pragma unroll
          for (int rt = 0; rt < RT; ++rt)
#pragma unroll
            for (int r = 0; r < 4; ++r) {
              float a[4];
              Vec4<T>::unpack(gpre[rt][r], a);
              const float iv = a[0], fv = a[1], gv = a[2], ov = a[3];
              const float dht = to_f32<T>(dhpre[rt][r]) + dhr[ui][rt][r];
              const float tc = tanhf_(ccur[ui][rt][r]);
              const float dct = dcs[ui][rt][r] + dht * ov * (1.f - tc * tc);
              float dg[4];
              dg[0] = dct * gv * iv * (1.f - iv);
              dg[1] = dct * cpre[rt][r] * fv * (1.f - fv);
              dg[2] = dct * iv * (1.f - gv * gv);
              dg[3] = dht * tc * ov * (1.f - ov);
              dcs[ui][rt][r] = dct * fv;
              ccur[ui][rt][r] = cpre[rt][r];
              const V4 pk = Vec4<T>::pack(dg);
              if constexpr (KH == 2) dgk[ui][rt][r] = pk;
              else *reinterpret_cast<V4*>(tile + (rt * 16 + lr * 4 + r) * pitch + (u * 4) * ES) = pk;
#ifndef BABL_NO_STORE
#if defined(BABL_HOT_INPUTS) && BABL_HOT_INPUTS == 3
              if (rowbase[rt][r] >= 0)
                *reinterpret_cast<V4*>(gates + ((long)(rowbase[rt][r] + (p.m.seq_len / 2) * stride_i) * ldg_i + (gcol_i + u * 4))) = pk;
#else
              if (!STG && rowbase[rt][r] >= 0)
                *reinterpret_cast<V4*>(gates + ((long)(rowbase[rt][r] + t * stride_i) * ldg_i + (gcol_i + u * 4))) = pk;
#endif
#endif
            }
        }
      }
      BWST(1 + ui);
    }
    if constexpr (!STG) {
      if (step + 1 == p.m.seq_len) break;
    }
    if constexpr (KH == 2) {
      f32x4_t accs[MAXUT][RT];
#pragma unroll
      for (int ui = 0; ui < MAXUT; ++ui)
#pragma unroll
        for (int rt = 0; rt < RT; ++rt) accs[ui][rt] = f32x4_t{0.f, 0.f, 0.f, 0.f};
      const int hu = H / 2, hs = nslab / 2;
#pragma unroll 1
      for (int half = 0; half < 2; ++half) {
#pragma unroll
        for (int ui = 0; ui < MAXUT; ++ui) {
          const int u = (w + NW * ui) * 16 + lc;
          if (u < H && (u >= hu) == (half == 1)) {
#pragma unroll
            for (int rt = 0; rt < RT; ++rt)
#pragma unroll
              for (int r = 0; r < 4; ++r)
                *reinterpret_cast<V4*>(tile + (rt * 16 + lr * 4 + r) * pitch + ((u - half * hu) * 4) * ES) = dgk[ui][rt][r];
          }
        }
        __syncthreads();
#pragma unroll
        for (int ui = 0; ui < MAXUT; ++ui) {
          const int ut = w + NW * ui;
          if (ut < nut) {
            const char* wr = whhT + ((long)ut * nslab + half * hs) * 1024;
            const char* ar = tile + lc * pitch + 16 * lr;
            constexpr int KB = 8;
#pragma unroll 1
            for (int k0 = 0; k0 < hs; k0 += KB) {
              uint4 b[KB];
#pragma unroll
              for (int i = 0; i < KB; ++i) b[i] = *reinterpret_cast<const uint4*>(wr + ((k0 + i < hs) ? k0 + i : hs - 1) * 1024);
#pragma unroll
              for (int i = 0; i < KB; ++i) {
                if (k0 + i < hs) {
                  uint4 a[RT];
#pragma unroll
                  for (int rt = 0; rt < RT; ++rt) a[rt] = *reinterpret_cast<const uint4*>(ar + rt * 16 * pitch + (k0 + i) * 64);
                  mma_slab<T, RT>(a, b[i], accs[ui]);
                }
              }
            }
          }
        }
        __syncthreads();
      }
#pragma unroll
      for (int ui = 0; ui < MAXUT; ++ui)
#pragma unroll
        for (int rt = 0; rt < RT; ++rt)
#pragma unroll
          for (int r = 0; r < 4; ++r) dhr[ui][rt][r] = accs[ui][rt][r];
      continue;
    }
    if constexpr (PF == 1) load_all(dir ? t + 1 : t - 1);
    BWST(5);
    __syncthreads();
    BWST(6);
    if constexpr (STG) {
#ifndef BABL_NO_STORE
      constexpr int CPR = 4 * HPC * ES / 16;
      const int* rowtab = reinterpret_cast<const int*>(smem + nbuf * R * pitch);
      for (int idx = tid; idx < R * CPR; idx += NW * 64) {
        const int row = idx / CPR, cc = idx - row * CPR;
        const int grow = rowtab[row];
        if (grow >= 0)
          *reinterpret_cast<uint4*>(reinterpret_cast<char*>(gates) + ((long)(grow + t * stride_i) * ldg_i + gcol_i) * ES + cc * 16) =
              *reinterpret_cast<const uint4*>(tile + row * pitch + cc * 16);
      }
#endif
      BWST(7);
      if (step + 1 == p.m.seq_len) break;
    }
#ifdef BABL_NO_MM
    if (p.m.seq_len > 0) continue;
#endif
#pragma unroll
    for (int ui = 0; ui < MAXUT; ++ui) {
      const int ut = w + NW * ui;
      if (ut < nut) {
        f32x4_t acc[RT];
#pragma unroll
        for (int rt = 0; rt < RT; ++rt) acc[rt] = f32x4_t{0.f, 0.f, 0.f, 0.f};
        const char* wr = whhT + ((long)ut * nslab) * 1024;
        const char* ar = tile + lc * pitch + 16 * lr;
#ifndef URSE_BWD_KB
#define URSE_BWD_KB 13
#endif
#ifndef URSE_BWD_KB2
#define URSE_BWD_KB2 17
#endif
#ifndef URSE_BWD_KB8
#define URSE_BWD_KB8 17
#endif
#ifndef URSE_BWD_KBPF16
#define URSE_BWD_KBPF16 8
#endif
#ifndef URSE_BWD_KBPF12
#define URSE_BWD_KBPF12 14
#endif
#ifndef URSE_BWD_KB2_PF3
#define URSE_BWD_KB2_PF3 9
#endif
#ifndef URSE_BWD_KB2_STG
#define URSE_BWD_KB2_STG 25
#endif
#ifndef URSE_BWD_KB2_PF4
#define URSE_BWD_KB2_PF4 17
#endif
#ifndef URSE_BWD_KB3
#define URSE_BWD_KB3 13
#endif
        constexpr int KB = (sizeof(T) == 2) ? (RT >= 3 ? URSE_BWD_KB3 : RT >= 2 ? (PF == 3 ? URSE_BWD_KB2_PF3 : (PF == 4 ? URSE_BWD_KB2_PF4 : (STG ? URSE_BWD_KB2_STG : URSE_BWD_KB2))) : (NW == 8 ? URSE_BWD_KB8 : (PF == 1 ? (NW == 12 ? URSE_BWD_KBPF12 : URSE_BWD_KBPF16) : URSE_BWD_KB))) : 8;
        #pragma unroll 1
        for (int k0 = 0; k0 < nslab; k0 += KB) {
          uint4 b[KB];
#pragma unroll
          for (int i = 0; i < KB; ++i) {
            const int ks = (k0 + i < nslab) ? k0 + i : nslab - 1;
#ifdef BABL_PIN_W
            b[i] = *reinterpret_cast<const uint4*>(whhT + (ks & 7) * 1024);
#else
            b[i] = *reinterpret_cast<const uint4*>(wr + ks * 1024);
#endif
          }
#pragma unroll
          for (int i = 0; i < KB; ++i) {
            if (k0 + i < nslab) {
              uint4 a[RT];
#pragma unroll
              for (int rt = 0; rt < RT; ++rt)
                a[rt] = *reinterpret_cast<const uint4*>(ar + rt * 16 * pitch + (k0 + i) * 64);
              mma_slab<T, RT>(a, b[i], acc);
            }
          }
        }
#pragma unroll
        for (int rt = 0; rt < RT; ++rt)
#pragma unroll
          for (int r = 0; r < 4; ++r) dhr[ui][rt][r] = acc[rt][r];
      }
      BWST(8 + ui);
    }
    if (nbuf == 1) __syncthreads();
  }
}

template <int H>
__global__ void __launch_bounds__(512) lstm_bwd_roles_kernel(LstmBwdArgs p) {
  constexpr int R = 32, NUT = (H + 15) / 16, G4 = 4 * H, NSLAB = G4 * 2 / 64, PITCH = lds_frag_pitch(G4 * 2);
  constexpr int NCW = 7, UPW = H / NCW, EPL = R * UPW / 64, KC = UPW / 8;
  constexpr int DP = H + 12;
  static_assert(H % NCW == 0 && UPW % 8 == 0 && EPL * 64 == R * UPW && EPL == 4 * KC, "element map: row = (k / KC) * 8 + lane / 8, unit = (k % KC) * 8 + lane % 8");
  extern __shared__ __attribute__((aligned(16))) char smem[];
  char* tile = smem;
  float* dhrec = reinterpret_cast<float*>(smem + R * PITCH);
  int* rowtab = reinterpret_cast<int*>(smem + R * PITCH + R * DP * 4);
  const int tid = threadIdx.x, lane = tid & 63;
  const int w = __builtin_amdgcn_readfirstlane(tid >> 6);
  int dir, tile_;
  xcd_dir_tile(p.xcd, dir, tile_);
  const int s0 = tile_ * R;
  const int ldg_i = (int)p.ldg, ldd_i = (int)p.ldd, ldc_i = 2 * H, stride_i = (int)p.m.stride;
  const int gcol_i = dir * G4, hcol_i = dir * H, prev_i = dir ? stride_i : -stride_i;
  if (tid < R) {
    const int seq = s0 + tid;
    rowtab[tid] = seq < p.m.n_seq ? (int)((seq / p.m.inner) * p.m.outer + (seq % p.m.inner)) : -1;
  }
  for (int i = tid; i < R * DP; i += 512) dhrec[i] = 0.f;
  for (int i = tid; i < R * PITCH / 16; i += 512) reinterpret_cast<uint4*>(tile)[i] = make_uint4(0, 0, 0, 0);
  __syncthreads();
  const bf16_t* dh = reinterpret_cast<const bf16_t*>(p.dh);
  bf16_t* gates = reinterpret_cast<bf16_t*>(p.gates);

  if (w < NCW) {
    const int r8 = lane >> 3, c8 = lane & 7;
    int rowb[4];
#pragma unroll
    for (int kr = 0; kr < 4; ++kr) {
      int seq = s0 + kr * 8 + r8;
      if (seq >= p.m.n_seq) seq = p.m.n_seq - 1;
      rowb[kr] = (int)((seq / p.m.inner) * p.m.outer + (seq % p.m.inner));
    }
    const int u0 = w * UPW + c8;
    float dcs[EPL], ccur[EPL];
    uint2 gp[EPL];
    float cp[EPL];
    bf16_t dp[EPL];
    const __amdgpu_buffer_rsrc_t rs_g = __builtin_amdgcn_make_buffer_rsrc(p.gates, 0, (int)0xFFFFF000u, 0x00020000);
    const __amdgpu_buffer_rsrc_t rs_c = __builtin_amdgcn_make_buffer_rsrc(const_cast<float*>(p.c), 0, (int)0xFFFFF000u, 0x00020000);
    const __amdgpu_buffer_rsrc_t rs_d = __builtin_amdgcn_make_buffer_rsrc(const_cast<void*>(p.dh), 0, (int)0xFFFFF000u, 0x00020000);
    auto load_inputs = [&](int tt) __attribute__((always_inline)) {
      const int toff_ = tt * stride_i;
      const bool first_ = dir ? (tt == p.m.seq_len - 1) : (tt == 0);
      unsigned og[4], oc[4], od[4];
#pragma unroll
      for (int kr = 0; kr < 4; ++kr) {
        const int row = rowb[kr] + toff_;
        og[kr] = (unsigned)(row * ldg_i + gcol_i + u0 * 4) * 2u;
        oc[kr] = (unsigned)((row + (first_ ? 0 : prev_i)) * ldc_i + hcol_i + u0) * 4u;
        od[kr] = (unsigned)(row * ldd_i + hcol_i + u0) * 2u;
      }
#pragma unroll
      for (int k = 0; k < EPL; ++k) {
        typedef unsigned u32x2_ __attribute__((ext_vector_type(2)));
        const u32x2_ g2 = __builtin_amdgcn_raw_buffer_load_b64(rs_g, (int)(og[k / KC] + (unsigned)((k % KC) * 64)), 0, 0);
        gp[k] = make_uint2(g2[0], g2[1]);
        const float cv = __uint_as_float(__builtin_amdgcn_raw_buffer_load_b32(rs_c, (int)(oc[k / KC] + (unsigned)((k % KC) * 32)), 0, 0));
        cp[k] = first_ ? 0.f : cv;
        dp[k] = (bf16_t)__builtin_amdgcn_raw_buffer_load_b16(rs_d, (int)(od[k / KC] + (unsigned)((k % KC) * 16)), 0, 0);
      }
    };
    {
      const int t0 = dir ? 0 : p.m.seq_len - 1;
#pragma unroll
      for (int k = 0; k < EPL; ++k) {
        dcs[k] = 0.f;
        ccur[k] = p.c[(long)(rowb[k / KC] + t0 * stride_i) * ldc_i + (hcol_i + u0 + (k % KC) * 8)];
      }
      load_inputs(t0);
    }
    constexpr int CPR = G4 * 2 / 16, CTHR = NCW * 64;
    for (int step = 0; step < p.m.seq_len; ++step) {
      const int t = dir ? step : (p.m.seq_len - 1 - step);
      const int toff = t * stride_i;
#pragma unroll
      for (int k = 0; k < EPL; ++k) {
        const int lrow = (k / KC) * 8 + r8, u = u0 + (k % KC) * 8;
        float a[4];
        Vec4<bf16_t>::unpack(gp[k], a);
        const float iv = a[0], fv = a[1], gv = a[2], ov = a[3];
        const float dht = bf16_to_f32(dp[k]) + dhrec[lrow * DP + u];
        const float tc = tanhf_(ccur[k]);
        const float dct = dcs[k] + dht * ov * (1.f - tc * tc);
        float dg[4];
        dg[0] = dct * gv * iv * (1.f - iv);
        dg[1] = dct * cp[k] * fv * (1.f - fv);
        dg[2] = dct * iv * (1.f - gv * gv);
        dg[3] = dht * tc * ov * (1.f - ov);
        dcs[k] = dct * fv;
        ccur[k] = cp[k];
        *reinterpret_cast<uint2*>(tile + lrow * PITCH + u * 8) = Vec4<bf16_t>::pack(dg);
      }
      asm volatile("s_waitcnt lgkmcnt(0)" ::: "memory");
      __builtin_amdgcn_s_barrier();
      for (int idx = tid; idx < R * CPR; idx += CTHR) {
        const int row = idx / CPR, cc = idx - row * CPR;
        const int grow = rowtab[row];
        if (grow >= 0)
          *reinterpret_cast<uint4*>(reinterpret_cast<char*>(gates) + ((long)(grow + toff) * ldg_i + gcol_i) * 2 + cc * 16) =
              *reinterpret_cast<const uint4*>(tile + row * PITCH + cc * 16);
      }
      if (step + 1 == p.m.seq_len) break;
      load_inputs(dir ? t + 1 : t - 1);
      asm volatile("s_waitcnt lgkmcnt(0)" ::: "memory");
      __builtin_amdgcn_s_barrier();
    }
    return;
  }

  const int lr = lane >> 4, lc = lane & 15;
  const char* whhT = reinterpret_cast<const char*>(p.whhT) + ((long)dir * NUT * NSLAB) * 1024 + lane * 16;
  const char* ar = tile + lc * PITCH + 16 * lr;
  uint4 b[NSLAB];
#pragma unroll
  for (int i = 0; i < NSLAB; ++i) b[i] = *reinterpret_cast<const uint4*>(whhT + (long)i * 1024);
  for (int step = 0; step < p.m.seq_len; ++step) {
    __builtin_amdgcn_s_barrier();
    if (step + 1 == p.m.seq_len) break;
#pragma unroll 1
    for (int ut = 0; ut < NUT; ++ut) {
      f32x4_t acc[2] = {f32x4_t{0.f, 0.f, 0.f, 0.f}, f32x4_t{0.f, 0.f, 0.f, 0.f}};
      const char* wn = whhT + (long)(ut + 1 < NUT ? ut + 1 : 0) * NSLAB * 1024;
#pragma unroll
      for (int i = 0; i < NSLAB; ++i) {
        uint4 a[2];
#pragma unroll
        for (int rt = 0; rt < 2; ++rt) a[rt] = *reinterpret_cast<const uint4*>(ar + rt * 16 * PITCH + i * 64);
        mma_slab<bf16_t, 2>(a, b[i], acc);
        b[i] = *reinterpret_cast<const uint4*>(wn + (long)i * 1024);
      }
      const int u = ut * 16 + lc;
      if (u < H) {
#pragma unroll
        for (int rt = 0; rt < 2; ++rt)
#pragma unroll
          for (int r = 0; r < 4; ++r) dhrec[(rt * 16 + lr * 4 + r) * DP + u] = acc[rt][r];
      }
    }
    asm volatile("s_waitcnt lgkmcnt(0)" ::: "memory");
    __builtin_amdgcn_s_barrier();
  }
  asm volatile("s_waitcnt vmcnt(0)" ::: "memory");
}

template <int RT, int MAXUT, int NW, int HC>
__global__ void __launch_bounds__(NW * 64) lstm_bwd_tr_kernel(LstmBwdArgs p) {
  extern __shared__ __attribute__((aligned(16))) char smem[];
  constexpr int R = 16 * RT;
  const int tid = threadIdx.x, lane = tid & 63, w = tid >> 6, lr = lane >> 4, lc = lane & 15;
  int dir, tile_;
  xcd_dir_tile(p.xcd, dir, tile_);
  const int s0 = tile_ * R;
  const int H = HC ? HC : p.H, nut = (H + 15) >> 4, G4 = 4 * H;
  const int pitch = lds_frag_pitch(G4 * 2);
  const int nbuf = p.dbuf ? 2 : 1;
  float dcs[MAXUT][RT][4], dhr[MAXUT][RT][4], ccur[MAXUT][RT][4];
  int rowbase[RT];
#pragma unroll
  for (int rt = 0; rt < RT; ++rt) {
    int seq = s0 + rt * 16 + lc;
    const bool ok = seq < p.m.n_seq;
    if (!ok) seq = p.m.n_seq - 1;
    const int rb = (int)((seq / p.m.inner) * p.m.outer + (seq % p.m.inner));
    rowbase[rt] = ok ? rb : -rb - 1;
  }
  auto rowb = [&](int rt) -> int { return rowbase[rt] >= 0 ? rowbase[rt] : -(rowbase[rt] + 1); };
  const int nslab = G4 * 2 / 64;
  const char* whhT = reinterpret_cast<const char*>(p.whhT) + ((long)dir * nut * nslab) * 1024 + lane * 16;
  const bf16_t* dh = reinterpret_cast<const bf16_t*>(p.dh);
  bf16_t* gates = reinterpret_cast<bf16_t*>(p.gates);
  const int ldg_i = (int)p.ldg, ldd_i = (int)p.ldd, ldc_i = 2 * H, stride_i = (int)p.m.stride;
  const int gcol_i = dir * G4, hcol_i = dir * H, prev_i = dir ? stride_i : -stride_i;
  auto quad = [&](int ui) -> int { return (w + NW * ui) * 16 + lr * 4; };

  {
    const int t0 = dir ? 0 : p.m.seq_len - 1;
#pragma unroll
    for (int ui = 0; ui < MAXUT; ++ui) {
      const int u0 = quad(ui) < H ? quad(ui) : H - 4;
#pragma unroll
      for (int rt = 0; rt < RT; ++rt) {
        const float4 cv = *reinterpret_cast<const float4*>(p.c + (long)(rowb(rt) + t0 * stride_i) * ldc_i + (hcol_i + u0));
        const float c4[4] = {cv.x, cv.y, cv.z, cv.w};
#pragma unroll
        for (int r = 0; r < 4; ++r) {
          dcs[ui][rt][r] = 0.f;
          dhr[ui][rt][r] = 0.f;
          ccur[ui][rt][r] = c4[r];
        }
      }
    }
  }
  uint4 gpf[MAXUT][RT][2];
  float4 cpf[MAXUT][RT];
  uint2 dpf[MAXUT][RT];
  auto load_all = [&](int tt) {
    const bool first_ = dir ? (tt == p.m.seq_len - 1) : (tt == 0);
#pragma unroll
    for (int ui = 0; ui < MAXUT; ++ui) {
      const int u0 = quad(ui);
      if (u0 < H) {
#pragma unroll
        for (int rt = 0; rt < RT; ++rt) {
          const int row = rowb(rt) + tt * stride_i;
          const bf16_t* gp = gates + ((long)row * ldg_i + (gcol_i + u0 * 4));
          gpf[ui][rt][0] = *reinterpret_cast<const uint4*>(gp);
          gpf[ui][rt][1] = *reinterpret_cast<const uint4*>(gp + 8);
          cpf[ui][rt] = first_ ? make_float4(0.f, 0.f, 0.f, 0.f)
                               : *reinterpret_cast<const float4*>(p.c + (long)(row + prev_i) * ldc_i + (hcol_i + u0));
          dpf[ui][rt] = *reinterpret_cast<const uint2*>(dh + (long)row * ldd_i + (hcol_i + u0));
        }
      }
    }
  };
  load_all(dir ? 0 : p.m.seq_len - 1);
  for (int step = 0; step < p.m.seq_len; ++step) {
    const int t = dir ? step : (p.m.seq_len - 1 - step);
    char* tile = smem + (step % nbuf) * R * pitch;
#pragma unroll
    for (int ui = 0; ui < MAXUT; ++ui) {
      const int u0 = quad(ui);
      if (u0 < H) {
#pragma unroll
        for (int rt = 0; rt < RT; ++rt) {
          const unsigned gw[8] = {gpf[ui][rt][0].x, gpf[ui][rt][0].y, gpf[ui][rt][0].z, gpf[ui][rt][0].w,
                                  gpf[ui][rt][1].x, gpf[ui][rt][1].y, gpf[ui][rt][1].z, gpf[ui][rt][1].w};
          const float c4[4] = {cpf[ui][rt].x, cpf[ui][rt].y, cpf[ui][rt].z, cpf[ui][rt].w};
          const unsigned dw[2] = {dpf[ui][rt].x, dpf[ui][rt].y};
          unsigned ow[8];
#pragma unroll
          for (int r = 0; r < 4; ++r) {
            const float iv = __uint_as_float(gw[2 * r] << 16), fv = __uint_as_float(gw[2 * r] & 0xffff0000u);
            const float gv = __uint_as_float(gw[2 * r + 1] << 16), ov = __uint_as_float(gw[2 * r + 1] & 0xffff0000u);
            const float dhv = __uint_as_float((r & 1) ? (dw[r >> 1] & 0xffff0000u) : (dw[r >> 1] << 16));
            const float dht = dhv + dhr[ui][rt][r];
            const float tc = tanhf_(ccur[ui][rt][r]);
            const float dct = dcs[ui][rt][r] + dht * ov * (1.f - tc * tc);
            const float d0 = dct * gv * iv * (1.f - iv);
            const float d1 = dct * c4[r] * fv * (1.f - fv);
            const float d2 = dct * iv * (1.f - gv * gv);
            const float d3 = dht * tc * ov * (1.f - ov);
            dcs[ui][rt][r] = dct * fv;
            ccur[ui][rt][r] = c4[r];
            ow[2 * r] = (unsigned)f32_to_bf16(d0) | ((unsigned)f32_to_bf16(d1) << 16);
            ow[2 * r + 1] = (unsigned)f32_to_bf16(d2) | ((unsigned)f32_to_bf16(d3) << 16);
          }
          const uint4 o0 = make_uint4(ow[0], ow[1], ow[2], ow[3]), o1 = make_uint4(ow[4], ow[5], ow[6], ow[7]);
          char* tp = tile + (rt * 16 + lc) * pitch + (u0 * 4) * 2;
          *reinterpret_cast<uint4*>(tp) = o0;
          *reinterpret_cast<uint4*>(tp + 16) = o1;
#ifndef BABL_NO_STORE
          if (rowbase[rt] >= 0) {
            bf16_t* gp = gates + ((long)(rowbase[rt] + t * stride_i) * ldg_i + (gcol_i + u0 * 4));
            *reinterpret_cast<uint4*>(gp) = o0;
            *reinterpret_cast<uint4*>(gp + 8) = o1;
          }
#endif
        }
      }
    }
    if (step + 1 == p.m.seq_len) break;
    load_all(dir ? t + 1 : t - 1);
    __syncthreads();
#pragma unroll
    for (int ui = 0; ui < MAXUT; ++ui) {
      const int ut = w + NW * ui;
      if (ut < nut) {
        f32x4_t acc[RT];
#pragma unroll
        for (int rt = 0; rt < RT; ++rt) acc[rt] = f32x4_t{0.f, 0.f, 0.f, 0.f};
        const char* wr = whhT + ((long)ut * nslab) * 1024;
        const char* ar = tile + lc * pitch + 16 * lr;
#ifndef URSE_BWD_TR_KB
#define URSE_BWD_TR_KB 17
#endif
        constexpr int KB = URSE_BWD_TR_KB;
        #pragma unroll 1
        for (int k0 = 0; k0 < nslab; k0 += KB) {
          uint4 b[KB];
#pragma unroll
          for (int i = 0; i < KB; ++i) {
            const int ks = (k0 + i < nslab) ? k0 + i : nslab - 1;
            b[i] = *reinterpret_cast<const uint4*>(wr + ks * 1024);
          }
#pragma unroll
          for (int i = 0; i < KB; ++i) {
            if (k0 + i < nslab) {
#pragma unroll
              for (int rt = 0; rt < RT; ++rt) {
                const uint4 a = *reinterpret_cast<const uint4*>(ar + rt * 16 * pitch + (k0 + i) * 64);
                acc[rt] = __builtin_amdgcn_mfma_f32_16x16x32_bf16(__builtin_bit_cast(bf16x8_t, b[i]),
                                                                  __builtin_bit_cast(bf16x8_t, a), acc[rt], 0, 0, 0);
              }
            }
          }
        }
#pragma unroll
        for (int rt = 0; rt < RT; ++rt)
#pragma unroll
          for (int r = 0; r < 4; ++r) dhr[ui][rt][r] = acc[rt][r];
      }
    }
    if (nbuf == 1) __syncthreads();
  }
}

template <typename T, typename TB = T>
__device__ __forceinline__ void lstm_pack_dev(const float* __restrict__ wih, const float* __restrict__ whh,
                                              const float* __restrict__ bih, const float* __restrict__ bhh,
                                              T* __restrict__ wih_p, TB* __restrict__ wihT_p,
                                              float* __restrict__ bias, T* __restrict__ whh_f,
                                              TB* __restrict__ whhT_f, int N, int Np, int H, int Hp) {
  static_assert(sizeof(T) == sizeof(TB), "one element size per pack");
  constexpr int ES = sizeof(T), EPL = 16 / ES, SK = 64 / ES;
  const int nut = (H + 15) >> 4, G4 = 4 * H;
  const long stride = (long)gridDim.x * blockDim.x, i0 = (long)blockIdx.x * blockDim.x + threadIdx.x;
  const int which = blockIdx.y;
  if (which == 0) {
    for (long idx = i0; idx < (long)2 * G4 * Np; idx += stride) {
      const int rp = (int)(idx / Np), n = (int)(idx - (long)rp * Np);
      const int d = rp / G4, r = rp - d * G4, u = r >> 2, g = r & 3;
      wih_p[idx] = from_f32<T>(n < N ? wih[((long)d * G4 + g * H + u) * N + n] : 0.f);
    }
  } else if (which == 1) {
    for (long idx = i0; idx < (long)N * 2 * G4; idx += stride) {
      const int n = (int)(idx / (2 * G4)), rp = (int)(idx - (long)n * 2 * G4);
      const int d = rp / G4, r = rp - d * G4, u = r >> 2, g = r & 3;
      wihT_p[idx] = from_f32<TB>(wih[((long)d * G4 + g * H + u) * N + n]);
    }
  } else if (which == 2) {
    for (long idx = i0; idx < 2 * G4; idx += stride) {
      const int d = (int)idx / G4, r = (int)idx - d * G4, u = r >> 2, g = r & 3;
      const int src = d * G4 + g * H + u;
      bias[idx] = bih[src] + bhh[src];
    }
  } else if (which == 3) {
    const int nslab = Hp / SK;
    const long total = (long)2 * nut * nslab * 4 * 64 * EPL;
    for (long idx = i0; idx < total; idx += stride) {
      long q = idx;
      const int j = (int)(q % EPL); q /= EPL;
      const int lane = (int)(q % 64); q /= 64;
      const int g = (int)(q % 4); q /= 4;
      const int ks = (int)(q % nslab); q /= nslab;
      const int ut = (int)(q % nut);
      const int d = (int)(q / nut);
      const int u = ut * 16 + (lane & 15), k = ks * SK + EPL * (lane >> 4) + j;
      whh_f[idx] = from_f32<T>((u < H && k < H) ? whh[((long)d * G4 + g * H + u) * H + k] : 0.f);
    }
  } else {
    const int nslab = G4 / SK;
    const long total = (long)2 * nut * nslab * 64 * EPL;
    for (long idx = i0; idx < total; idx += stride) {
      long q = idx;
      const int j = (int)(q % EPL); q /= EPL;
      const int lane = (int)(q % 64); q /= 64;
      const int ks = (int)(q % nslab); q /= nslab;
      const int ut = (int)(q % nut);
      const int d = (int)(q / nut);
      const int n = ut * 16 + (lane & 15), kk = ks * SK + EPL * (lane >> 4) + j;
      const int up = kk >> 2, gp = kk & 3;
      whhT_f[idx] = from_f32<TB>(n < H ? whh[((long)d * G4 + gp * H + up) * H + n] : 0.f);
    }
  }
}

template <typename T, typename TB = T>
__global__ void __launch_bounds__(256) lstm_pack_kernel(const float* __restrict__ wih, const float* __restrict__ whh,
                                                        const float* __restrict__ bih, const float* __restrict__ bhh,
                                                        T* __restrict__ wih_p, TB* __restrict__ wihT_p,
                                                        float* __restrict__ bias, T* __restrict__ whh_f,
                                                        TB* __restrict__ whhT_f, int N, int Np, int H, int Hp) {
  lstm_pack_dev<T, TB>(wih, whh, bih, bhh, wih_p, wihT_p, bias, whh_f, whhT_f, N, Np, H, Hp);
}
template <typename T, typename TB = T>
__global__ void __launch_bounds__(256) lstm_pack_multi_kernel(const PackRow* __restrict__ tab, int N, int Np, int H, int Hp) {
  const PackRow r = tab[blockIdx.z];
  lstm_pack_dev<T, TB>(r.wih, r.whh, r.bih, r.bhh, (T*)r.wih_p, (TB*)r.wihT_p, r.bias, (T*)r.whh_f, (TB*)r.whhT_f, N, Np, H, Hp);
}

template <typename K>
static void allow_big_lds(K kernel) {
  (void)hipFuncSetAttribute(reinterpret_cast<const void*>(kernel), hipFuncAttributeMaxDynamicSharedMemorySize,
                            160 * 1024);
}

template <typename T, int RT, int NW>
static int launch_fwd(const LstmFwdArgs& p, hipStream_t st) {
  constexpr int R = 16 * RT;
  const size_t lds = (size_t)2 * R * lds_frag_pitch(p.Hp * (int)sizeof(T));
  URSE_CHECK_ARG(lds <= 160 * 1024, "urse_lstm_fwd: Hp %d with %d rows exceeds LDS", p.Hp, R);
  dim3 grid(ceil_div(p.m.n_seq, R), 2);
  const int upw = ((p.H + 15) / 16 + NW - 1) / NW;
#define URSE_LF(MU)                                                                              \
  {                                                                                              \
    static bool once = (allow_big_lds(lstm_fwd_kernel<T, RT, MU, NW>), true);                    \
    (void)once;                                                                                  \
    hipLaunchKernelGGL((lstm_fwd_kernel<T, RT, MU, NW>), grid, dim3(NW * 64), lds, st, p);       \
  }
  if (upw <= 2) URSE_LF(2) else if (upw <= 4) URSE_LF(4) else URSE_LF(6)
#undef URSE_LF
  URSE_CHECK_LAUNCH("urse_lstm_fwd");
  return URSE_OK;
}

#ifdef URSE_EXPERIMENTS
static int bwd_variant() {
  const char* e = getenv("URSE_BWD_VARIANT");
  return e ? atoi(e) : 0;
}
#else
static constexpr int bwd_variant() { return 0; }
#endif

template <typename T, int RT, int NW>
static int launch_bwd(const LstmBwdArgs& p, hipStream_t st) {
  constexpr int R = 16 * RT;
  size_t lds = (size_t)R * lds_frag_pitch(4 * p.H * (int)sizeof(T));
  if constexpr (sizeof(T) == 4 && RT == 1 && NW == 16) {
    if (lds > 160 * 1024 && p.H % 8 == 0 && (size_t)R * lds_frag_pitch(2 * p.H * 4) <= 160 * 1024) {
      LstmBwdArgs pa = p;
      pa.dbuf = 0;
      pa.xcd = xcd_dir_env() & 1;
      const size_t lds2 = (size_t)R * lds_frag_pitch(2 * p.H * 4);
      dim3 grid(ceil_div(p.m.n_seq, R), 2);
      const int upw = ((p.H + 15) / 16 + NW - 1) / NW;
      if (upw <= 3) {
        static bool once = (allow_big_lds(lstm_bwd_kernel<T, 1, 3, 16, 0, 0, 0, 0, 2>), true);
        (void)once;
        hipLaunchKernelGGL((lstm_bwd_kernel<T, 1, 3, 16, 0, 0, 0, 0, 2>), grid, dim3(NW * 64), lds2, st, pa);
      } else {
        static bool once = (allow_big_lds(lstm_bwd_kernel<T, 1, 6, 16, 0, 0, 0, 0, 2>), true);
        (void)once;
        hipLaunchKernelGGL((lstm_bwd_kernel<T, 1, 6, 16, 0, 0, 0, 0, 2>), grid, dim3(NW * 64), lds2, st, pa);
      }
      URSE_CHECK_LAUNCH("urse_lstm_bwd");
      return URSE_OK;
    }
  }
  URSE_CHECK_ARG(lds <= 160 * 1024, "urse_lstm_bwd: H %d with %d rows exceeds LDS", p.H, R);
  LstmBwdArgs pa = p;
  pa.dbuf = (2 * lds <= 150 * 1024) ? 1 : 0;
  pa.xcd = xcd_dir_env() & 1;
  if (pa.dbuf) lds *= 2;
  dim3 grid(ceil_div(p.m.n_seq, R), 2);
  const int upw = ((p.H + 15) / 16 + NW - 1) / NW;
#define URSE_LB(MU)                                                                              \
  {                                                                                              \
    static bool once = (allow_big_lds(lstm_bwd_kernel<T, RT, MU, NW>), true);                    \
    (void)once;                                                                                  \
    hipLaunchKernelGGL((lstm_bwd_kernel<T, RT, MU, NW>), grid, dim3(NW * 64), lds, st, pa);      \
  }
  if constexpr (sizeof(T) == 2 && NW == 8 && RT == 2) {
    if (p.H == 392 && upw <= 4) {
      static const bool stg_on = !(getenv("URSE_BWD_STAGED_STORES") && atoi(getenv("URSE_BWD_STAGED_STORES")) == 0);
      const bool stg = stg_on && (p.ldg * 2) % 16 == 0 && (reinterpret_cast<uintptr_t>(p.gates) % 16) == 0;
#ifdef URSE_EXPERIMENTS
      if (stg && bwd_variant() == 7) {
        static bool once = (allow_big_lds(lstm_bwd_kernel<T, 2, 4, 8, 0, 392, 3, 1>), true);
        (void)once;
        hipLaunchKernelGGL((lstm_bwd_kernel<T, 2, 4, 8, 0, 392, 3, 1>), grid, dim3(NW * 64), lds + R * sizeof(int), st, pa);
      } else
#endif
#ifdef URSE_EXPERIMENTS
      const bool roles = getenv("URSE_BWD_ROLES") && atoi(getenv("URSE_BWD_ROLES")) != 0;
      const long rows_ = p.m.stride * (p.m.seq_len - 1) + ((long)(p.m.n_seq - 1) / p.m.inner) * p.m.outer + (p.m.n_seq - 1) % p.m.inner + 1;
      if (stg && roles && (size_t)R * lds_frag_pitch(4 * 392 * 2) + R * (392 + 12) * 4 + R * sizeof(int) <= 160 * 1024 &&
          rows_ * p.ldg * 2 < 0xFFFFF000L && rows_ * 2L * p.H * 4 < 0xFFFFF000L && rows_ * p.ldd * 2 < 0xFFFFF000L && rows_ * p.ldg < (1L << 31)) {
        static bool once = (allow_big_lds(lstm_bwd_roles_kernel<392>), true);
        (void)once;
        hipLaunchKernelGGL((lstm_bwd_roles_kernel<392>), grid, dim3(512), (size_t)R * lds_frag_pitch(4 * 392 * 2) + R * (392 + 12) * 4 + R * sizeof(int), st, pa);
        URSE_CHECK_LAUNCH("urse_lstm_bwd");
        return URSE_OK;
      }
      static const bool pairs = getenv("URSE_BWD_PAIRS") && atoi(getenv("URSE_BWD_PAIRS")) != 0;
      if (stg && pairs && !pa.dbuf && lds + R * sizeof(int) + NW * 7168 <= 160 * 1024 && (p.ldd * 2) % 16 == 0 && (reinterpret_cast<uintptr_t>(p.dh) % 16) == 0 &&
          (reinterpret_cast<uintptr_t>(p.c) % 16) == 0) {
        static bool once = (allow_big_lds(lstm_bwd_kernel<T, 2, 4, 8, 0, 392, 4, 1>), true);
        (void)once;
        hipLaunchKernelGGL((lstm_bwd_kernel<T, 2, 4, 8, 0, 392, 4, 1>), grid, dim3(NW * 64), lds + R * sizeof(int) + NW * 7168, st, pa);
      } else
#endif
      if (stg) {
        static bool once = (allow_big_lds(lstm_bwd_kernel<T, 2, 4, 8, 0, 392, 0, 1>), true);
        (void)once;
        hipLaunchKernelGGL((lstm_bwd_kernel<T, 2, 4, 8, 0, 392, 0, 1>), grid, dim3(NW * 64), lds + R * sizeof(int), st, pa);
      } else {
        static bool once = (allow_big_lds(lstm_bwd_kernel<T, 2, 4, 8, 0, 392>), true);
        (void)once;
        hipLaunchKernelGGL((lstm_bwd_kernel<T, 2, 4, 8, 0, 392>), grid, dim3(NW * 64), lds, st, pa);
      }
      URSE_CHECK_LAUNCH("urse_lstm_bwd");
      return URSE_OK;
    }
  }
#ifdef URSE_EXPERIMENTS
  if constexpr (sizeof(T) == 2 && NW == 4 && RT == 3) {
    static bool once = (allow_big_lds(lstm_bwd_kernel<T, 3, 7, 4, 0, 392, 0, 1>), true);
    (void)once;
    pa.dbuf = 0;
    hipLaunchKernelGGL((lstm_bwd_kernel<T, 3, 7, 4, 0, 392, 0, 1>), grid, dim3(NW * 64), (size_t)R * lds_frag_pitch(4 * p.H * 2) + R * sizeof(int), st, pa);
    URSE_CHECK_LAUNCH("urse_lstm_bwd");
    return URSE_OK;
  } else
#endif
  {
  if constexpr (sizeof(T) == 2 && NW == 8 && RT == 1) {
#ifdef URSE_EXPERIMENTS
    if (p.H == 392 && bwd_variant() == 6) {
      static bool once = (allow_big_lds(lstm_bwd_tr_kernel<1, 4, 8, 392>), true);
      (void)once;
      hipLaunchKernelGGL((lstm_bwd_tr_kernel<1, 4, 8, 392>), grid, dim3(NW * 64), lds, st, pa);
      URSE_CHECK_LAUNCH("urse_lstm_bwd");
      return URSE_OK;
    }
#endif
    if (p.H == 392) {
      static bool once = (allow_big_lds(lstm_bwd_kernel<T, 1, 4, 8, 392, 0, 1>), true);
      (void)once;
      hipLaunchKernelGGL((lstm_bwd_kernel<T, 1, 4, 8, 392, 0, 1>), grid, dim3(NW * 64), lds, st, pa);
      URSE_CHECK_LAUNCH("urse_lstm_bwd");
      return URSE_OK;
    }
  }
  if constexpr (sizeof(T) == 2 && NW == 16 && RT == 1) {
#ifdef URSE_EXPERIMENTS
    if (p.H == 392 && (bwd_variant() == 4 || bwd_variant() == 5)) {
      const int nw = bwd_variant() == 4 ? 13 : 12;
      if (nw == 13) {
        static bool once = (allow_big_lds(lstm_bwd_kernel<T, 1, 2, 13, 392, 0, 1>), true);
        (void)once;
        hipLaunchKernelGGL((lstm_bwd_kernel<T, 1, 2, 13, 392, 0, 1>), grid, dim3(nw * 64), lds, st, pa);
      } else {
        static bool once = (allow_big_lds(lstm_bwd_kernel<T, 1, 3, 12, 392, 0, 1>), true);
        (void)once;
        hipLaunchKernelGGL((lstm_bwd_kernel<T, 1, 3, 12, 392, 0, 1>), grid, dim3(nw * 64), lds, st, pa);
      }
      URSE_CHECK_LAUNCH("urse_lstm_bwd");
      return URSE_OK;
    }
    if (p.H == 392 && bwd_variant() == 3) {
      static bool once = (allow_big_lds(lstm_bwd_kernel<T, 1, 2, 16, 392, 0, 2>), true);
      (void)once;
      hipLaunchKernelGGL((lstm_bwd_kernel<T, 1, 2, 16, 392, 0, 2>), grid, dim3(NW * 64), lds, st, pa);
      URSE_CHECK_LAUNCH("urse_lstm_bwd");
      return URSE_OK;
    }
    if (p.H == 392 && bwd_variant() == 1) {
      static bool once = (allow_big_lds(lstm_bwd_kernel<T, 1, 2, 16, 392, 0, 1>), true);
      (void)once;
      hipLaunchKernelGGL((lstm_bwd_kernel<T, 1, 2, 16, 392, 0, 1>), grid, dim3(NW * 64), lds, st, pa);
      URSE_CHECK_LAUNCH("urse_lstm_bwd");
      return URSE_OK;
    }
#endif
    if (p.H == 392) {
      static bool once = (allow_big_lds(lstm_bwd_kernel<T, 1, 2, 16, 392>), true);
      (void)once;
      hipLaunchKernelGGL((lstm_bwd_kernel<T, 1, 2, 16, 392>), grid, dim3(NW * 64), lds, st, pa);
      URSE_CHECK_LAUNCH("urse_lstm_bwd");
      return URSE_OK;
    }
  }
  if (upw <= 2) URSE_LB(2) else if (upw <= 3) URSE_LB(3) else if (upw <= 4) URSE_LB(4) else URSE_LB(6)
#undef URSE_LB
  URSE_CHECK_LAUNCH("urse_lstm_bwd");
  return URSE_OK;
  }
}

}

using namespace urse;

static int check_map(const SeqMap& m, int H, int es, const char* who) {
  URSE_CHECK_ARG(m.n_seq > 0 && m.seq_len > 0 && m.inner > 0 && m.outer > 0 && m.stride > 0, "%s: bad sequence map",
                 who);
  URSE_CHECK_ARG(H > 0 && (4 * H * es) % 64 == 0, "%s: 4H*elemsize must be a multiple of 64 bytes (H=%d)", who, H);
  URSE_CHECK_ARG((H + 15) / 16 <= 48, "%s: H=%d too large (<= 768)", who, H);
  return URSE_OK;
}

extern "C" int urse_lstm_pack(const float* wih, const float* whh, const float* bih, const float* bhh, void* wih_p,
                              void* wihT_p, float* bias, void* whh_frag, void* whhT_frag, int N, int Np, int H, int Hp,
                              int dtype, void* stream) {
  URSE_CHECK_ARG(wih && whh && bih && bhh && wih_p && wihT_p && bias && whh_frag && whhT_frag, "urse_lstm_pack: null pointer");
  const int es = dtype == URSE_F32 ? 4 : 2;
  URSE_CHECK_ARG(dtype == URSE_F32 || dtype == URSE_BF16 || dtype == URSE_F16, "urse_lstm_pack: bad dtype %d", dtype);
  URSE_CHECK_ARG(N > 0 && H > 0 && Np >= N && (Hp * es) % 64 == 0 && Hp >= ((H + 15) / 16) * 16 && (4 * H * es) % 64 == 0,
                 "urse_lstm_pack: bad shape N%d Np%d H%d Hp%d", N, Np, H, Hp);
  dim3 grid(256, 5), blk(256);
  if (dtype == URSE_F16)
    hipLaunchKernelGGL((lstm_pack_kernel<f16_t, bf16_t>), grid, blk, 0, (hipStream_t)stream, wih, whh, bih, bhh, (f16_t*)wih_p,
                       (bf16_t*)wihT_p, bias, (f16_t*)whh_frag, (bf16_t*)whhT_frag, N, Np, H, Hp);
  else if (dtype == URSE_BF16)
    hipLaunchKernelGGL(lstm_pack_kernel<bf16_t>, grid, blk, 0, (hipStream_t)stream, wih, whh, bih, bhh, (bf16_t*)wih_p,
                       (bf16_t*)wihT_p, bias, (bf16_t*)whh_frag, (bf16_t*)whhT_frag, N, Np, H, Hp);
  else
    hipLaunchKernelGGL(lstm_pack_kernel<float>, grid, blk, 0, (hipStream_t)stream, wih, whh, bih, bhh, (float*)wih_p,
                       (float*)wihT_p, bias, (float*)whh_frag, (float*)whhT_frag, N, Np, H, Hp);
  URSE_CHECK_LAUNCH("urse_lstm_pack");
  return URSE_OK;
}

extern "C" int urse_lstm_pack_multi(const void* table, int n_lstm, int N, int Np, int H, int Hp, int dtype, void* stream) {
  const int es = dtype == URSE_F32 ? 4 : 2;
  URSE_CHECK_ARG(dtype == URSE_F32 || dtype == URSE_BF16 || dtype == URSE_F16, "urse_lstm_pack_multi: bad dtype %d", dtype);
  URSE_CHECK_ARG(table && n_lstm > 0 && n_lstm < 65536 && N > 0 && H > 0 && Np >= N && (Hp * es) % 64 == 0 && Hp >= ((H + 15) / 16) * 16 &&
                     (4 * H * es) % 64 == 0, "urse_lstm_pack_multi: bad argument N%d Np%d H%d Hp%d", N, Np, H, Hp);
  dim3 grid(256, 5, (unsigned)n_lstm), blk(256);
  if (dtype == URSE_F16)
    hipLaunchKernelGGL((lstm_pack_multi_kernel<f16_t, bf16_t>), grid, blk, 0, (hipStream_t)stream, (const PackRow*)table, N, Np, H, Hp);
  else if (dtype == URSE_BF16)
    hipLaunchKernelGGL(lstm_pack_multi_kernel<bf16_t>, grid, blk, 0, (hipStream_t)stream, (const PackRow*)table, N, Np, H, Hp);
  else
    hipLaunchKernelGGL(lstm_pack_multi_kernel<float>, grid, blk, 0, (hipStream_t)stream, (const PackRow*)table, N, Np, H, Hp);
  URSE_CHECK_LAUNCH("urse_lstm_pack_multi");
  return URSE_OK;
}

extern "C" int urse_lstm_bidir_fwd(void* gx, int64_t ldg, const void* whh, void* hout, int64_t ldh, float* c, int H,
                                   int Hp, int n_seq, int seq_len, int64_t inner, int64_t outer, int64_t stride,
                                   int save, int dtype, int rows16, void* hout_bf16, void* stream) {
  URSE_CHECK_ARG(gx && whh && hout && (c || !save), "urse_lstm_bidir_fwd: null pointer");
  URSE_CHECK_ARG(dtype == URSE_F32 || dtype == URSE_BF16 || dtype == URSE_F16, "urse_lstm_bidir_fwd: bad dtype %d", dtype);
  URSE_CHECK_ARG(!hout_bf16 || dtype == URSE_F16, "urse_lstm_bidir_fwd: the bf16 copy of h goes with f16 operands only");
  LstmFwdArgs p;
  p.gx = gx; p.ldg = ldg; p.whh = whh; p.hout = hout; p.hout2 = hout_bf16; p.ldh = ldh; p.c = c; p.H = H; p.Hp = Hp; p.save = save;
  p.xcd = (xcd_dir_env() >> 2) & 1;
  p.m.inner = inner; p.m.outer = outer; p.m.stride = stride; p.m.n_seq = n_seq; p.m.seq_len = seq_len;
  const int es = dtype == URSE_F32 ? 4 : 2;
  int rc = check_map(p.m, H, es, "urse_lstm_bidir_fwd");
  if (rc) return rc;
  URSE_CHECK_ARG((Hp * es) % 64 == 0 && Hp >= ((H + 15) / 16) * 16, "urse_lstm_bidir_fwd: bad Hp %d for H %d", Hp, H);
  URSE_CHECK_ARG(ldg >= 8L * H && ldh >= 2L * H && ldg % 4 == 0, "urse_lstm_bidir_fwd: leading dimension too small");
  hipStream_t st = (hipStream_t)stream;
  int rt = rows16 & 15;
  bool nw8 = (rows16 >> 4) & 1;
  if (rt == 0) { rt = 1; nw8 = false; }
  note_launch(URSE_KV_LSTM_FWD_STREAM);
  if (dtype == URSE_F16) return launch_fwd<f16_t, 1, 16>(p, st);
  if (dtype == URSE_BF16) {
    if (nw8) {
      if (rt >= 4) return launch_fwd<bf16_t, 4, 8>(p, st);
      if (rt == 2) return launch_fwd<bf16_t, 2, 8>(p, st);
      return launch_fwd<bf16_t, 1, 8>(p, st);
    }
    if (rt >= 2 && H <= 256) return launch_fwd<bf16_t, 2, 16>(p, st);
    return launch_fwd<bf16_t, 1, 16>(p, st);
  }
  return launch_fwd<float, 1, 16>(p, st);
}

extern "C" int urse_lstm_bidir_bwd(const void* dh, int64_t ldd, void* gates, int64_t ldg, const float* c,
                                   const void* whhT, int H, int n_seq, int seq_len, int64_t inner, int64_t outer,
                                   int64_t stride, int dtype, int rows16, void* stream) {
  URSE_CHECK_ARG(dh && gates && c && whhT, "urse_lstm_bidir_bwd: null pointer");
  LstmBwdArgs p;
  p.dh = dh; p.ldd = ldd; p.gates = gates; p.ldg = ldg; p.c = c; p.whhT = whhT; p.H = H;
  p.m.inner = inner; p.m.outer = outer; p.m.stride = stride; p.m.n_seq = n_seq; p.m.seq_len = seq_len;
  const int es = dtype == URSE_BF16 ? 2 : 4;
  int rc = check_map(p.m, H, es, "urse_lstm_bidir_bwd");
  if (rc) return rc;
  URSE_CHECK_ARG(ldg >= 8L * H && ldd >= 2L * H && ldg % 4 == 0, "urse_lstm_bidir_bwd: leading dimension too small");
  URSE_CHECK_ARG(ldg < (1L << 31) && ldd < (1L << 31) && stride * seq_len + (n_seq / inner + 1) * outer < (1L << 31),
                 "urse_lstm_bidir_bwd: row indices must fit 32 bits");
  hipStream_t st = (hipStream_t)stream;
  int rt = rows16 & 15;
  bool nw8 = (rows16 >> 4) & 1;
  const bool fits2 = (size_t)32 * lds_frag_pitch(8 * H) <= 160 * 1024;
  if (rt == 0) {
    const bool many = (long)n_seq >= 32L * 128;
    rt = (many && fits2) ? 2 : 1;
    nw8 = many && fits2;
  }
  if (rt == 1 && (bwd_variant() == 2 || bwd_variant() == 6)) nw8 = true;
#ifdef URSE_EXPERIMENTS
  const bool fits3 = (size_t)48 * lds_frag_pitch(8 * H) + 48 * sizeof(int) <= 160 * 1024;
  if (dtype == URSE_BF16 && H == 392 && rt == 2 && fits3 && bwd_variant() == 8 && (ldg * 2) % 16 == 0 && ((uintptr_t)gates % 16) == 0) {
    note_launch(URSE_KV_LSTM_BWD_STREAM32);
    return launch_bwd<bf16_t, 3, 4>(p, st);
  }
#endif
  note_launch(dtype == URSE_BF16 && rt >= 2 && fits2 ? URSE_KV_LSTM_BWD_STREAM32 : URSE_KV_LSTM_BWD_STREAM16);
  if (dtype == URSE_BF16) {
    if (nw8) return (rt >= 2 && fits2) ? launch_bwd<bf16_t, 2, 8>(p, st) : launch_bwd<bf16_t, 1, 8>(p, st);
    if (rt >= 2 && fits2) return launch_bwd<bf16_t, 2, 16>(p, st);
    return launch_bwd<bf16_t, 1, 16>(p, st);
  }
  return launch_bwd<float, 1, 16>(p, st);
}

#ifdef BWSTAMP
extern "C" int urse_diag_bwd_stamps(void* host_out) {
  return (int)hipMemcpyFromSymbol(host_out, HIP_SYMBOL(urse::g_bwstamps), sizeof(unsigned long long) * 512 * 16);
}
#endif
```

### urgent2026_challenge_track1_amd/csrc/urse_common.h

```cpp
#pragma once
#include <hip/hip_runtime.h>
#include <hip/hip_bf16.h>
#include <stdint.h>
#include <stdio.h>
#include <stdlib.h>
#include <string.h>

#include "../../include/urse.h"

namespace urse {

void set_error(const char* fmt, ...);
void note_launch(int variant);

#define URSE_CHECK_ARG(cond, ...)                      \
  do {                                                 \
    if (!(cond)) {                                     \
      ::urse::set_error(__VA_ARGS__);                  \
      return URSE_ERR_INVALID_ARG;                     \
    }                                                  \
  } while (0)

#define URSE_CHECK_LAUNCH(name)                                               \
  do {                                                                        \
    hipError_t e__ = hipGetLastError();                                       \
    if (e__ != hipSuccess) {                                                  \
      ::urse::set_error("%s: launch failed: %s", name, hipGetErrorString(e__)); \
      return URSE_ERR_LAUNCH;                                                 \
    }                                                                         \
  } while (0)

typedef unsigned short bf16_t;
typedef _Float16 f16_t;

__device__ __forceinline__ float bf16_to_f32(bf16_t v) { return __uint_as_float(((unsigned)v) << 16); }
__device__ __forceinline__ bf16_t f32_to_bf16(float f) {
  __hip_bfloat16 b = __float2bfloat16(f);
  return *reinterpret_cast<bf16_t*>(&b);
}

template <typename T> __device__ __forceinline__ float to_f32(T v);
template <> __device__ __forceinline__ float to_f32<float>(float v) { return v; }
template <> __device__ __forceinline__ float to_f32<bf16_t>(bf16_t v) { return bf16_to_f32(v); }
template <typename T> __device__ __forceinline__ T from_f32(float v);
template <> __device__ __forceinline__ float from_f32<float>(float v) { return v; }
template <> __device__ __forceinline__ bf16_t from_f32<bf16_t>(float v) { return f32_to_bf16(v); }
template <> __device__ __forceinline__ float to_f32<f16_t>(f16_t v) { return (float)v; }
template <> __device__ __forceinline__ f16_t from_f32<f16_t>(float v) { return (f16_t)v; }

template <typename T> __device__ __forceinline__ unsigned pack2(float a, float b);
template <> __device__ __forceinline__ unsigned pack2<bf16_t>(float a, float b) {
  typedef float f32x2_ __attribute__((ext_vector_type(2)));
  typedef __bf16 bf16x2_ __attribute__((ext_vector_type(2)));
  return __builtin_bit_cast(unsigned, __builtin_convertvector(f32x2_{a, b}, bf16x2_));
}
template <> __device__ __forceinline__ unsigned pack2<f16_t>(float a, float b) {
  typedef float f32x2_ __attribute__((ext_vector_type(2)));
  typedef _Float16 f16x2_ __attribute__((ext_vector_type(2)));
  return __builtin_bit_cast(unsigned, __builtin_convertvector(f32x2_{a, b}, f16x2_));
}
template <typename T> __device__ __forceinline__ void unpack2(unsigned v, float& a, float& b);
template <> __device__ __forceinline__ void unpack2<bf16_t>(unsigned v, float& a, float& b) {
  a = __uint_as_float(v << 16); b = __uint_as_float(v & 0xffff0000u);
}
template <> __device__ __forceinline__ void unpack2<f16_t>(unsigned v, float& a, float& b) {
  typedef _Float16 f16x2_ __attribute__((ext_vector_type(2)));
  const f16x2_ h = __builtin_bit_cast(f16x2_, v);
  a = (float)h[0]; b = (float)h[1];
}
template <typename T> __device__ __forceinline__ float __attribute__((ext_vector_type(4)))
mfma16(const uint4& a, const uint4& b, float __attribute__((ext_vector_type(4))) c) {
  if constexpr (__is_same(T, f16_t)) {
    typedef _Float16 f16x8_ __attribute__((ext_vector_type(8)));
    return __builtin_amdgcn_mfma_f32_16x16x32_f16(__builtin_bit_cast(f16x8_, a), __builtin_bit_cast(f16x8_, b), c, 0, 0, 0);
  } else {
    typedef __bf16 bf16x8_ __attribute__((ext_vector_type(8)));
    return __builtin_amdgcn_mfma_f32_16x16x32_bf16(__builtin_bit_cast(bf16x8_, a), __builtin_bit_cast(bf16x8_, b), c, 0, 0, 0);
  }
}

__device__ __forceinline__ float wave_sum(float v) {
#pragma unroll
  for (int o = 32; o > 0; o >>= 1) v += __shfl_xor(v, o, 64);
  return v;
}
__device__ __forceinline__ double wave_sum_d(double v) {
#pragma unroll
  for (int o = 32; o > 0; o >>= 1) v += __shfl_xor(v, o, 64);
  return v;
}

__device__ __forceinline__ float block_sum(float v, float* red) {
  v = wave_sum(v);
  const int lane = threadIdx.x & 63, w = threadIdx.x >> 6, nw = (blockDim.x + 63) >> 6;
  __syncthreads();
  if (lane == 0) red[w] = v;
  __syncthreads();
  float r = 0.f;
  for (int i = 0; i < nw; ++i) r += red[i];
  return r;
}

__host__ __device__ constexpr int lds_frag_pitch(int row_bytes) { return (row_bytes - 32 + 63) / 64 * 64 + 32; }

__device__ __forceinline__ float sigmoidf_(float x) { return __builtin_amdgcn_rcpf(1.0f + __expf(-x)); }
__device__ __forceinline__ float tanhf_(float x) {
  const float e = __expf(2.0f * x);
  return 1.0f - 2.0f * __builtin_amdgcn_rcpf(e + 1.0f);
}

__device__ __forceinline__ void xcd_dir_tile(int on, int& dir, int& tile) {
  if (on) {
    const int lin = blockIdx.x + gridDim.x * blockIdx.y, r = lin & 7;
    dir = r & 1;
    tile = (lin >> 3) * 4 + (r >> 1);
  } else {
    dir = blockIdx.y;
    tile = blockIdx.x;
  }
}
static inline int xcd_dir_env() {
  static const int v = getenv("URSE_LSTM_XCD_DIR") ? atoi(getenv("URSE_LSTM_XCD_DIR")) : 5;
  return v;
}

static inline int ceil_div(long a, long b) { return (int)((a + b - 1) / b); }

int device_cu_count();

struct PackRow {
  const float* wih; const float* whh; const float* bih; const float* bhh;
  void* wih_p; void* wihT_p; float* bias; void* whh_f; void* whhT_f;
  void* whhq; void* whhb; void* wx;
  void* wihq;
};

}
```

### urgent2026_challenge_track1_amd/ops.py

```python
import os

import torch

from . import _lib
from ._lib import call, require_cuda, stream_ptr

WIN_RECT, WIN_HANN = 0, 1
F32, BF16, F16 = 0, 1, 2
BF16_ACT_F16 = 3
HALF_TYPES = (torch.bfloat16, torch.float16)


def bwd_dtype(dtype):
    return torch.bfloat16 if dtype == torch.float16 else dtype

_timing = None


def enable_timing(names):
    global _timing
    _timing = {n: [] for n in names}


def disable_timing():
    global _timing
    t, _timing = _timing, None
    return t


def timed_call(tname, name, *args):
    if _timing is not None and tname in _timing:
        a, b = torch.cuda.Event(enable_timing=True), torch.cuda.Event(enable_timing=True)
        a.record()
        call(name, *args)
        b.record()
        _timing[tname].append((a, b))
    else:
        call(name, *args)


KERNEL_VARIANTS = ("nt_bres", "nt_ring", "nt_ring_wide", "nt_128", "nt_grouped_ring", "nt_grouped_128", "tn_ring", "tn_ring_t",
                   "tn_dual", "tn_128", "tn_grouped", "lstm_fwd_stream", "lstm_fwd_wide", "lstm_fwd_cluster",
                   "lstm_fwd_cluster2", "lstm_bwd_stream16", "lstm_bwd_stream32", "lstm_bwd_cluster", "lstm_bwd_split",
                   "stft960", "stft_generic", "istft_generic", "istft960", "lstm_fwd_rw", "tn_act_f16", "lstm_fwd_rwx", "lstm_bwd_nsplit",
                   "lstm_fwd_clusterx", "_unused28")


_PAGEABLE_UPLOADS = os.environ.get("URSE_PAGEABLE_UPLOADS", "0") == "1"


def upload(host_tensor, device, cached=False):
    if torch.device(device).type != "cuda":
        return host_tensor
    if _PAGEABLE_UPLOADS:
        return host_tensor.to(device)
    out = host_tensor.contiguous().pin_memory().to(device, non_blocking=True)
    if cached:
        ev = torch.cuda.Event()
        ev.record(torch.cuda.current_stream(device))
        ev.synchronize()
    return out


def launch_counts(reset=False):
    lib = _lib.load()
    out = {n: lib.urse_launch_count(i) for i, n in enumerate(KERNEL_VARIANTS)}
    if reset:
        lib.urse_launch_counts_reset()
    return out


def _f32c(t):
    return t.contiguous().float() if (t.dtype != torch.float32 or not t.is_contiguous()) else t


def stft_forward(wav, n_fft, hop, window=WIN_HANN, lens=None):
    require_cuda(wav)
    wav = _f32c(wav)
    B, L = wav.shape
    T, Fb = L // hop + 1, n_fft // 2 + 1
    spec = torch.empty(B, T, Fb, 2, device=wav.device, dtype=torch.float32)
    if lens is not None:
        if lens.device.type == "cpu":
            lens = upload(lens.to(torch.int32), wav.device)
        else:
            lens = lens.to(device=wav.device, dtype=torch.int32).contiguous()
    timed_call("stft_fwd", "stft_fwd", wav, lens, spec, B, L, n_fft, hop, window, stream_ptr())
    return torch.view_as_complex(spec)


class _ISTFT(torch.autograd.Function):
    @staticmethod
    def forward(ctx, spec_ri, n_fft, hop, length, window):
        B, T, Fb, _ = spec_ri.shape
        wav = torch.empty(B, length, device=spec_ri.device, dtype=torch.float32)
        call("istft_fwd", spec_ri, wav, B, T, n_fft, hop, length, window, stream_ptr())
        ctx.cfg = (B, T, Fb, n_fft, hop, length, window)
        return wav

    @staticmethod
    def backward(ctx, g):
        B, T, Fb, n_fft, hop, length, window = ctx.cfg
        g = _f32c(g)
        gs = torch.empty(B, T, Fb, 2, device=g.device, dtype=torch.float32)
        call("istft_bwd", g, gs, B, T, n_fft, hop, length, window, stream_ptr())
        return gs, None, None, None, None


def istft_forward(spec, n_fft, hop, length, window=WIN_HANN):
    if spec.is_complex():
        spec = torch.view_as_real(spec)
    require_cuda(spec)
    return _ISTFT.apply(_f32c(spec), n_fft, hop, int(length), window)


def _dt(t):
    if t.dtype == torch.bfloat16:
        return BF16
    if t.dtype == torch.float32:
        return F32
    if t.dtype == torch.float16:
        return F16
    raise TypeError("URSE GEMM operands are bf16, f16 or f32, got %s" % t.dtype)


def dtype_code(dtype):
    return {torch.float32: F32, torch.bfloat16: BF16, torch.float16: F16}[dtype]


def gemm_nt(A, W, bias=None, resid=None, act=0, out=None, out_dtype=None, N=None, gn_rows=0):
    require_cuda(A, W)
    M, K = A.shape
    Nw = W.shape[0] if N is None else N
    assert W.shape[1] == K and A.stride(1) == 1 and W.stride(1) == 1 and A.dtype == W.dtype
    if out is None:
        out = torch.empty(M, Nw, device=A.device, dtype=out_dtype or A.dtype)
    assert out.stride(1) == 1
    if gn_rows:
        assert out.dtype == torch.float32 and out.stride(0) == Nw and M % gn_rows == 0
        stats = torch.empty(M // gn_rows * 2, device=A.device, dtype=torch.float64)
        call("gemm_nt_gnstats", A, A.stride(0), W, W.stride(0), out, out.stride(0), bias, resid,
             0 if resid is None else resid.stride(0), M, Nw, K, _dt(A), act, stats, gn_rows, stream_ptr())
        return out, stats
    call("gemm_nt", A, A.stride(0), W, W.stride(0), out, out.stride(0), bias, resid,
         0 if resid is None else resid.stride(0), M, Nw, K, _dt(A), _dt(out), act, stream_ptr())
    return out


def gemm_tn(A, Bm, out, colsum=None, Mo=None, No=None, shift=0, inner=1, period=0, invalid_step=0, perm_h=0, target_wgs=0):
    require_cuda(A, Bm, out)
    R = A.shape[0]
    Mo = A.shape[1] if Mo is None else Mo
    No = Bm.shape[1] if No is None else No
    assert Bm.shape[0] == R and A.stride(1) == 1 and Bm.stride(1) == 1
    assert out.dtype == torch.float32 and out.stride(-1) == 1
    call("gemm_tn", A, A.stride(0), Bm, Bm.stride(0), out, out.stride(0), colsum, R, Mo, No, shift, inner, period,
         invalid_step, perm_h, _tn_dt(A, Bm), int(target_wgs), stream_ptr())
    return out


def _tn_dt(A, *Bs):
    if A.dtype == torch.bfloat16 and all(b.dtype == torch.float16 for b in Bs):
        return BF16_ACT_F16
    assert all(b.dtype == A.dtype for b in Bs), (A.dtype, [b.dtype for b in Bs])
    return _dt(A)


TN_ACT_F16 = os.environ.get("URSE_TN_ACT_F16", "1") != "0"


def tn_act_f16_supported(R, Mo, No, No2=0, with_colsum=True, inner=1, period=0):
    return TN_ACT_F16 and bool(_lib.load().urse_gemm_tn_act_f16_supported(int(R), int(Mo), int(No), int(No2), int(bool(with_colsum)),
                                                                        int(inner), int(period)))


def gemm_tn_dual(A, Bm, out, colsum, B2, out2, Mo, No, No2, shift, inner, period, invalid_step, perm_h=0, target_wgs=0):
    require_cuda(A, Bm, B2, out, out2)
    R = A.shape[0]
    assert Bm.shape[0] == R and B2.shape[0] == R and A.stride(1) == 1 and Bm.stride(1) == 1 and B2.stride(1) == 1
    assert out.dtype == torch.float32 and out2.dtype == torch.float32
    call("gemm_tn_dual", A, A.stride(0), Bm, Bm.stride(0), out, out.stride(0), colsum, B2, B2.stride(0), out2, out2.stride(0), R,
         Mo, No, No2, shift, inner, period, invalid_step, perm_h, _tn_dt(A, Bm, B2), int(target_wgs), stream_ptr())


def tn_desc(A, Bm, out, colsum=None, Mo=None, No=None, shift=0, inner=1, period=0, invalid_step=0, perm_h=0):
    R = A.shape[0]
    Mo = A.shape[1] if Mo is None else Mo
    No = Bm.shape[1] if No is None else No
    assert Bm.shape[0] == R and A.stride(1) == 1 and Bm.stride(1) == 1 and A.dtype == Bm.dtype
    assert out.dtype == torch.float32 and out.stride(-1) == 1 and out.stride(0) >= No
    epc = 16 // A.element_size()
    for t, n in ((A, Mo), (Bm, No)):
        last = t.storage_offset() + (R - 1) * t.stride(0) + (n + epc - 1) // epc * epc
        assert last * t.element_size() <= t.untyped_storage().nbytes(), "tn_desc: operand rows are not padded to 16 bytes"
    return [A.data_ptr(), Bm.data_ptr(), out.data_ptr(), 0 if colsum is None else colsum.data_ptr(), A.stride(0),
            Bm.stride(0), out.stride(0), R, Mo, No, shift, max(1, inner), period, invalid_step, 0, perm_h] + [0] * 8


def gemm_tn_grouped(rows, dtype, device, target_blocks=1024):
    bkr = 32 if dtype == torch.bfloat16 else 16
    tiles = [((r[8] + 127) // 128) * ((r[9] + 127) // 128) for r in rows]
    per_group = max(1, target_blocks // max(1, sum(tiles)))
    max_blocks = 0
    for r, tl in zip(rows, tiles):
        R = r[7]
        slices = max(1, min(per_group, (R + 4 * bkr - 1) // (4 * bkr)))
        rps = (R + slices - 1) // slices
        rps = (rps + bkr - 1) // bkr * bkr
        r[14] = rps
        max_blocks = max(max_blocks, tl * ((R + rps - 1) // rps))
    descs = upload(torch.tensor(rows, dtype=torch.int64), device)
    call("gemm_tn_grouped", descs, len(rows), max_blocks, BF16 if dtype == torch.bfloat16 else F32, stream_ptr())


def pad_to(n, m):
    return (n + m - 1) // m * m


def kpad(n, dtype):
    return pad_to(n, 32 if dtype in HALF_TYPES else 16)


def pack2d(inp, out_rows, out_cols, dtype, transpose=False, out=None):
    require_cuda(inp)
    assert inp.dim() == 2 and inp.stride(1) == 1
    rows, cols = (inp.shape[1], inp.shape[0]) if transpose else inp.shape
    if out is None:
        out = torch.empty(out_rows, out_cols, device=inp.device, dtype=dtype)
    call("pack2d", inp, inp.stride(0), _dt(inp), out, out.stride(0), _dt(out), rows, cols, out_rows, out_cols,
         int(transpose), stream_ptr())
    return out


def groupnorm_fwd(x, gamma, beta, B, T, Kg, W, N, Np, gstride, dtype, eps=1e-5, add=None, stats=None, bf16_copy=False):
    require_cuda(x)
    y = torch.empty(B * T * Kg * (W // N), Np, device=x.device, dtype=dtype)
    y2 = torch.empty_like(y, dtype=torch.bfloat16) if (bf16_copy and dtype == torch.float16) else None
    if stats is not None:
        assert stats.numel() == B * Kg * 2 and stats.dtype == torch.float64
        call("groupnorm_apply", x, gamma, beta, add, y, stats, B, T, Kg, W, N, Np, gstride, float(eps), _dt(y), y2, stream_ptr())
    else:
        stats = torch.empty(B * Kg * 2, device=x.device, dtype=torch.float64)
        call("groupnorm_fwd", x, gamma, beta, add, y, stats, B, T, Kg, W, N, Np, gstride, float(eps), _dt(y), y2, stream_ptr())
    if bf16_copy is None:
        return y, stats, y
    return (y, stats, (y2 if y2 is not None else y)) if bf16_copy else (y, stats)


def groupnorm_bwd(x, dy, stats, gamma, dres, dgamma, dbeta, B, T, Kg, W, N, gstride, eps=1e-5, pack_ld=0, sums=None):
    dx = torch.empty_like(x)
    dxp = torch.empty(x.numel() // N, pack_ld, device=x.device, dtype=torch.bfloat16) if pack_ld else None
    if sums is not None:
        call("groupnorm_bwd_apply", x, dy, stats, sums, gamma, dres, dx, B, T, Kg, W, N, gstride, float(eps), dxp, pack_ld, stream_ptr())
        return (dx, dxp) if pack_ld else dx
    sums = torch.empty(B * Kg * 2, device=x.device, dtype=torch.float64)
    call("groupnorm_bwd", x, dy, stats, gamma, dres, dx, dgamma, dbeta, sums, B, T, Kg, W, N, gstride, float(eps), dxp,
         pack_ld, stream_ptr())
    return (dx, dxp) if pack_ld else dx


FUSE_GN_BWD = os.environ.get("URSE_FUSE_GN_BWD", "1") != "0"
GN_BWD_SLOTS = 16


def gemm_nt_gnbwd_supported(M, N, K, rows_per_group, dtype):
    return (dtype == torch.bfloat16 and M >= 2048 and 160 <= N <= 224 and N % 4 == 0 and K % 32 == 0 and K >= 96 and
            rows_per_group >= 256 and M % rows_per_group == 0 and not os.environ.get("URSE_NT_NO_DMA"))


def gemm_nt_gnbwd(A, W, N, x, stats, gamma, dgamma, dbeta, rows_per_group, eps=1e-5):
    require_cuda(A, W, x)
    M, K = A.shape
    assert W.shape[1] == K and A.stride(1) == 1 and W.stride(1) == 1 and A.dtype == W.dtype and x.is_contiguous() and x.numel() == M * N
    dy = torch.empty(M, N, device=A.device, dtype=torch.float32)
    ng = M // rows_per_group * 2
    ws = torch.empty(ng + GN_BWD_SLOTS * N, device=A.device, dtype=torch.float64)
    sums, part = ws[:ng], ws[ng:].view(torch.float32)
    call("gemm_nt_gnbwd", A, A.stride(0), W, W.stride(0), dy, M, N, K, _dt(A), x, stats, gamma, sums, dgamma, dbeta, part, GN_BWD_SLOTS,
         rows_per_group, float(eps), stream_ptr())
    return dy, sums


LSTM_LAYOUTS = ("whhq", "wihq", "whhb", "wx", "whhTq")
PACK_MULTI_LAYOUTS = {"whhq", "wihq", "whhb", "wx"}


def lstm_layout_ok(name, N, Np, H, Hp, dtype):
    lib = _lib.load()
    if dtype not in HALF_TYPES or Hp % 32:
        return False
    if name == "whhq":
        return True
    if name == "wihq":
        return bool(lib.urse_lstm_clusterx_supported(N, Np, H, Hp))
    if name == "wx":
        return bool(lib.urse_lstm_rwx_supported(N, Np, H, Hp))
    if dtype != torch.bfloat16:
        return False
    if name == "whhb":
        return bool(lib.urse_lstm_wide_supported(H, Hp))
    return name == "whhTq" and H % 8 == 0


def lstm_pack(wih, whh, bih, bhh, N, H, dtype, out=None, layouts=None):
    dev = wih.device
    Np, Hp = kpad(N, dtype), kpad(pad_to(H, 16), dtype)
    nu = pad_to(H, 16)
    bdt = bwd_dtype(dtype)
    if out is None:
        out = dict(wih=torch.empty(8 * H, Np, device=dev, dtype=dtype),
                   wihT=torch.empty(N, 8 * H, device=dev, dtype=bdt),
                   bias=torch.empty(8 * H, device=dev, dtype=torch.float32),
                   whh=torch.empty(2 * nu * 4 * Hp, device=dev, dtype=dtype),
                   whhT=torch.empty(2 * nu * 4 * H, device=dev, dtype=bdt), Np=Np, Hp=Hp)
    fdt = _dt(out["wih"])
    call("lstm_pack", wih, whh, bih, bhh, out["wih"], out["wihT"], out["bias"], out["whh"], out["whhT"], N, Np, H, Hp, fdt, stream_ptr())
    want = lambda name: (layouts is None or name in layouts) and lstm_layout_ok(name, N, Np, H, Hp, dtype)

    def buf(name, n):
        if name not in out:
            out[name] = torch.empty(n, device=dev, dtype=dtype)
        return out[name]
    if want("whhq"):
        call("lstm_pack_quads", whh, buf("whhq", 2 * ((H + 3) // 4) * (Hp // 32) * 512), H, Hp, fdt, stream_ptr())
    if want("wihq"):
        call("lstm_pack_quads_x", wih, buf("wihq", 2 * ((H + 3) // 4) * (Np // 32) * 512), N, Np, H, fdt, stream_ptr())
    if want("whhb"):
        call("lstm_pack_blocks", whh, buf("whhb", 2 * ((H + 15) // 16) * (Hp // 32) * 4 * 512), H, Hp, stream_ptr())
    if want("wx"):
        call("lstm_pack_blocks_x", wih, whh, buf("wx", 2 * ((H + 15) // 16) * (Hp // 32 + Np // 32) * 4 * 512), N, Np, H, Hp, fdt, stream_ptr())
    if want("whhTq"):
        C = ((H + 3) // 4 + 13) // 14
        call("lstm_pack_bwd_quads", whh, buf("whhTq", 2 * C * 4 * (H // 8) * 512), H, C, stream_ptr())
    return out


PACK_MULTI = os.environ.get("URSE_LSTM_PACK_MULTI", "1") != "0"


def lstm_pack_multi(entries, N, H, dtype, table=None):
    first = entries[0][4]
    Np, Hp = first["Np"], first["Hp"]
    dev = entries[0][0].device
    ptr = lambda t: 0 if t is None else t.data_ptr()
    rows = [[ptr(wih), ptr(whh), ptr(bih), ptr(bhh), ptr(o["wih"]), ptr(o["wihT"]), ptr(o["bias"]), ptr(o["whh"]), ptr(o["whhT"]),
             ptr(o.get("whhq")), ptr(o.get("whhb")), ptr(o.get("wx")), ptr(o.get("wihq"))] for wih, whh, bih, bhh, o in entries]
    if table is None or table[1] != rows:
        table = (upload(torch.tensor(rows, dtype=torch.int64), dev, cached=True), rows)
    n = len(rows)
    fdt = _dt(first["wih"])
    call("lstm_pack_multi", table[0], n, N, Np, H, Hp, fdt, stream_ptr())
    if any(r[9] for r in rows):
        call("lstm_pack_quads_multi", table[0], n, H, Hp, fdt, stream_ptr())
    if any(r[10] for r in rows):
        assert fdt == BF16
        call("lstm_pack_blocks_multi", table[0], n, H, Hp, stream_ptr())
    if any(r[11] for r in rows):
        call("lstm_pack_blocks_x_multi", table[0], n, N, Np, H, Hp, fdt, stream_ptr())
    if any(r[12] for r in rows):
        call("lstm_pack_quads_x_multi", table[0], n, N, Np, H, fdt, stream_ptr())
    return table


_err_state = {}


def kernel_error_flag(device):
    st = _err_state.get(device)
    if st is None:
        st = _err_state[device] = {"flag": torch.zeros(1, device=device, dtype=torch.int32),
                                   "host": torch.zeros(1, dtype=torch.int32).pin_memory(), "event": None}
    return st["flag"]


def poll_kernel_errors(device, sync=False):
    kernel_error_flag(device)
    st = _err_state[device]
    if sync:
        bad = int(st["flag"].item()) != 0
    else:
        bad = st["event"] is not None and st["event"].query() and int(st["host"][0]) != 0
        st["host"].copy_(st["flag"], non_blocking=True)
        st["event"] = torch.cuda.Event()
        st["event"].record(torch.cuda.current_stream(device))
    if bad:
        raise _lib.UrseError("a cooperative LSTM kernel (cluster / split) timed out waiting for a peer workgroup: the device did "
                             "not keep all its workgroups resident; results of that step are invalid "
                             "(URSE_LSTM_CLUSTER=0 selects the streaming kernels)")


def _hout_buffer(M, ldh, H, like, dtype=None):
    hout = torch.empty(M, ldh, device=like.device, dtype=dtype or like.dtype)
    if ldh > 2 * H:
        hout[:, 2 * H:].zero_()
    return hout


_cluster_ws = {}
USE_CLUSTER_LSTM = os.environ.get("URSE_LSTM_CLUSTER", "1") != "0"
USE_CLUSTER_LSTM_BWD = os.environ.get("URSE_LSTM_CLUSTER_BWD", "0") == "1"


CO_RESIDENT_WGS = 0
PREFETCH_RESERVED_CUS = 0


COMM_RESERVED_CUS = 0
SHARED_GPU_RANKS = 1
RCCL_MAX_CHANNELS = int(os.environ.get("URSE_RCCL_MAX_CHANNELS", "32"))
COOP_REFUSALS = 0


def cap_rccl_channels():
    os.environ.setdefault("NCCL_MAX_NCHANNELS", str(RCCL_MAX_CHANNELS))
    return rccl_reserved_cus()


def rccl_reserved_cus():
    v = os.environ.get("NCCL_MAX_NCHANNELS")
    try:
        return max(1, int(v)) if v is not None else 64
    except ValueError:
        return 64


def reserved_cus():
    return int(CO_RESIDENT_WGS) + int(PREFETCH_RESERVED_CUS) + int(COMM_RESERVED_CUS)


class reserve_cus:

    def __init__(self, co_resident=None, prefetch=None, comm=None):
        self.new = (co_resident, prefetch, comm)

    def __enter__(self):
        global CO_RESIDENT_WGS, PREFETCH_RESERVED_CUS, COMM_RESERVED_CUS
        self.old = (CO_RESIDENT_WGS, PREFETCH_RESERVED_CUS, COMM_RESERVED_CUS)
        co, pf, cm = self.new
        if co is not None:
            CO_RESIDENT_WGS = co
        if pf is not None:
            PREFETCH_RESERVED_CUS = pf
        if cm is not None:
            COMM_RESERVED_CUS = cm
        return self

    def __exit__(self, *exc):
        global CO_RESIDENT_WGS, PREFETCH_RESERVED_CUS, COMM_RESERVED_CUS
        CO_RESIDENT_WGS, PREFETCH_RESERVED_CUS, COMM_RESERVED_CUS = self.old
        return False


def _note_refusal(fits_without_reservation):
    global COOP_REFUSALS
    if reserved_cus() > 0 and fits_without_reservation():
        COOP_REFUSALS += 1


def lstm_cluster_plan(H, Hp, n_seq):
    import ctypes
    if SHARED_GPU_RANKS > 1:
        return None
    plan = (ctypes.c_int64 * 6)()
    lib = _lib.load()
    if lib.urse_lstm_cluster_plan(H, Hp, n_seq, reserved_cus(), plan) != 0:
        _note_refusal(lambda: lib.urse_lstm_cluster_plan(H, Hp, n_seq, 0, plan) == 0)
        return None
    return list(plan)


CLUSTER_XCD_AWARE = os.environ.get("URSE_LSTM_CLUSTER_XCD", "1") != "0"


def lstm_fwd_cluster(gx, whhq, H, Hp, n_seq, seq_len, inner, outer, stride, save=True, xcd_aware=None, bf16_copy=False):
    xcd_aware = CLUSTER_XCD_AWARE if xcd_aware is None else xcd_aware
    plan = lstm_cluster_plan(H, Hp, n_seq)
    M, dev = gx.shape[0], gx.device
    key = (dev, H, Hp, n_seq, plan[4], plan[5])
    if key not in _cluster_ws:
        _cluster_ws[key] = (torch.zeros(plan[4], device=dev, dtype=torch.bfloat16),
                            torch.zeros(plan[5], device=dev, dtype=torch.int32),
                            kernel_error_flag(dev))
    hx, cnt, err = _cluster_ws[key]
    ldh = kpad(2 * H, gx.dtype)
    hout = _hout_buffer(M, ldh, H, gx)
    hout2 = _hout_buffer(M, ldh, H, gx, torch.bfloat16) if (bf16_copy and gx.dtype == torch.float16) else None
    c = torch.empty(M, 2 * H, device=dev, dtype=torch.float32) if save else None
    timed_call("lstm_fwd_time" if stride > 1 else "lstm_fwd_band", "lstm_cluster_fwd", gx, gx.stride(0), whhq, hout, ldh,
               c, hx, cnt, err, H, Hp, n_seq, seq_len, inner, outer, stride, int(save), reserved_cus(), int(bool(xcd_aware)), _dt(gx), hout2,
               stream_ptr())
    return (hout, c, err, hout2 if hout2 is not None else hout) if bf16_copy else (hout, c, err)


USE_CLUSTERX_LSTM = os.environ.get("URSE_LSTM_CLUSTERX", "1") != "0"


def lstm_clusterx_supported(N, Np, H, Hp):
    return bool(_lib.load().urse_lstm_clusterx_supported(N, Np, H, Hp))


BAND_CLUSTERX = os.environ.get("URSE_LSTM_BAND_CLUSTERX", "1") != "0"
TIME_CLUSTERX_ROUNDS = os.environ.get("URSE_LSTM_TIME_CLUSTERX_ROUNDS", "1") != "0"


def lstm_clusterx_plan(H, Hp, n_seq):
    import ctypes
    if SHARED_GPU_RANKS > 1:
        return None
    plan = (ctypes.c_int64 * 7)()
    lib = _lib.load()
    if lib.urse_lstm_clusterx_plan(H, Hp, n_seq, reserved_cus(), plan) != 0:
        _note_refusal(lambda: lib.urse_lstm_clusterx_plan(H, Hp, n_seq, 0, plan) == 0)
        return None
    return list(plan)


CLUSTERX_US_PER_STEP, CLUSTERX_US_PROLOGUE, RWX_NS_PER_SEQ_STEP, RWX_US_PER_STEP_FLOOR = 6.3, 50.0, 3.5, 36.0


def band_clusterx_pays(H, Hp, n_seq, seq_len=34):
    plan = lstm_clusterx_plan(H, Hp, n_seq)
    if plan is None or plan[6] <= 1:
        return False
    cx = plan[6] * seq_len * CLUSTERX_US_PER_STEP + CLUSTERX_US_PROLOGUE
    rwx = seq_len * max(RWX_US_PER_STEP_FLOOR, 2 * n_seq * RWX_NS_PER_SEQ_STEP * 1e-3)
    return cx < 0.95 * rwx


def lstm_fwd_clusterx(xn, wihq, whhq, bias, N, H, Hp, n_seq, seq_len, inner, outer, stride, save=True, xcd_aware=None, bf16_copy=False):
    xcd_aware = CLUSTER_XCD_AWARE if xcd_aware is None else xcd_aware
    plan = lstm_clusterx_plan(H, Hp, n_seq)
    if plan is None:
        raise RuntimeError("lstm_fwd_clusterx: no cluster plan for H=%d n_seq=%d" % (H, n_seq))
    M, Np, dev = xn.shape[0], xn.shape[1], xn.device
    n_hx = int(plan[4])
    key = ("x", dev, H, Hp, n_seq, n_hx, plan[5])
    if key not in _cluster_ws:
        _cluster_ws[key] = (torch.zeros(n_hx, device=dev, dtype=torch.bfloat16),
                            torch.zeros(plan[5], device=dev, dtype=torch.int32),
                            kernel_error_flag(dev))
    hx, cnt, err = _cluster_ws[key]
    ldh = kpad(2 * H, xn.dtype)
    hout = _hout_buffer(M, ldh, H, xn)
    hout2 = _hout_buffer(M, ldh, H, xn, torch.bfloat16) if (bf16_copy and xn.dtype == torch.float16 and save) else None
    c = torch.empty(M, 2 * H, device=dev, dtype=torch.float32) if save else None
    gates = torch.empty(M, 8 * H, device=dev, dtype=torch.bfloat16) if save else None
    timed_call("lstm_fwd_time" if stride > 1 else "lstm_fwd_band", "lstm_clusterx_fwd", xn, xn.stride(0), wihq, bias, whhq, gates, 8 * H, hout, ldh, c,
               hx, cnt, err, N, Np, H, Hp, n_seq, seq_len, inner, outer, stride, int(save), reserved_cus(), int(bool(xcd_aware)), _dt(xn), hout2,
               stream_ptr())
    if bf16_copy:
        return gates, hout, c, err, (hout2 if hout2 is not None else hout)
    return gates, hout, c, err


CLUSTER2_H = tuple(int(v) for v in os.environ.get("URSE_LSTM_CLUSTER2_H", "768").split(",") if v)


def lstm_cluster2_plan(H, Hp, n_seq):
    import ctypes
    if SHARED_GPU_RANKS > 1:
        return None
    plan = (ctypes.c_int64 * 4)()
    if _lib.load().urse_lstm_cluster2_plan(H, Hp, n_seq, reserved_cus(), plan) != 0:
        _note_refusal(lambda: _lib.load().urse_lstm_cluster2_plan(H, Hp, n_seq, 0, plan) == 0)
        return None
    return list(plan)


def device_cus():
    return torch.cuda.get_device_properties(torch.cuda.current_device()).multi_processor_count


def lstm_cluster2_chunks(H, Hp, n_seq, seq_len, inner, outer, stride):
    if lstm_cluster2_plan(H, Hp, n_seq) is not None:
        return [(0, n_seq)]
    if not (inner == 1 and stride == 1 and outer == seq_len):
        return None
    probe = lstm_cluster2_plan(H, Hp, 1)
    if probe is None:
        return None
    cap = max(1, (device_cus() - reserved_cus() - 4) // 2 // probe[0]) * 64
    n = (n_seq + cap - 1) // cap
    if n > CLUSTER2_MAX_CHUNKS:
        return None
    per = (n_seq + n - 1) // n
    return [(s0, min(per, n_seq - s0)) for s0 in range(0, n_seq, per)]


CLUSTER2_MAX_CHUNKS = int(os.environ.get("URSE_LSTM_CLUSTER2_MAX_CHUNKS", "6"))


def lstm_fwd_cluster2(gx, whhq, H, Hp, n_seq, seq_len, inner, outer, stride, save=True):
    chunks = lstm_cluster2_chunks(H, Hp, n_seq, seq_len, inner, outer, stride)
    M, dev = gx.shape[0], gx.device
    ldh = kpad(2 * H, gx.dtype)
    hout = _hout_buffer(M, ldh, H, gx)
    c = torch.empty(M, 2 * H, device=dev, dtype=torch.float32) if save else None
    err = None
    for s0, n in chunks:
        plan = lstm_cluster2_plan(H, Hp, n)
        key = ("c2", dev, H, Hp, n, plan[3])
        if key not in _cluster_ws:
            _cluster_ws[key] = (torch.empty(plan[3], device=dev, dtype=torch.bfloat16), kernel_error_flag(dev))
        hx, err = _cluster_ws[key]
        if len(chunks) == 1:
            g_, h_, c_ = gx, hout, c
        else:
            r0, r1 = s0 * seq_len, (s0 + n) * seq_len
            g_, h_, c_ = gx[r0:r1], hout[r0:r1], (c[r0:r1] if save else None)
        timed_call("lstm_fwd_time" if stride > 1 else "lstm_fwd_band", "lstm_cluster2_fwd", g_, gx.stride(0), whhq, h_, ldh, c_, hx,
                   err, H, Hp, n, seq_len, inner, outer, stride, int(save), reserved_cus(), _dt(gx), stream_ptr())
    return hout, c, err


def lstm_fwd(gx, whh, H, Hp, n_seq, seq_len, inner, outer, stride, save=True, rows16=0, bf16_copy=False):
    M = gx.shape[0]
    ldh = kpad(2 * H, gx.dtype)
    hout = _hout_buffer(M, ldh, H, gx)
    hout2 = _hout_buffer(M, ldh, H, gx, torch.bfloat16) if (bf16_copy and gx.dtype == torch.float16) else None
    c = torch.empty(M, 2 * H, device=gx.device, dtype=torch.float32) if save else None
    timed_call("lstm_fwd_time" if stride > 1 else "lstm_fwd_band", "lstm_bidir_fwd", gx, gx.stride(0), whh, hout, ldh,
               c, H, Hp, n_seq, seq_len, inner, outer, stride, int(save), _dt(gx), rows16, hout2, stream_ptr())
    return (hout, c, hout2 if hout2 is not None else hout) if bf16_copy else (hout, c)


USE_WIDE_LSTM = os.environ.get("URSE_LSTM_WIDE", "1") != "0"
FUSE_GN_STATS = os.environ.get("URSE_FUSE_GN_STATS", "1") != "0"
TN_OVERLAP = os.environ.get("URSE_TN_OVERLAP", "1") != "0"
def low_priority_stream(device, force=False):
    if not force and os.environ.get("URSE_SIDE_STREAM_PRIORITY", "normal") != "low":
        return torch.cuda.Stream(device=device)
    import ctypes
    try:
        hip = ctypes.CDLL("libamdhip64.so")
        least, greatest = ctypes.c_int(), ctypes.c_int()
        st = ctypes.c_void_p()
        with torch.cuda.device(device):
            if hip.hipDeviceGetStreamPriorityRange(ctypes.byref(least), ctypes.byref(greatest)) != 0:
                raise RuntimeError("priority range")
            if hip.hipStreamCreateWithPriority(ctypes.byref(st), ctypes.c_uint(1), ctypes.c_int(least.value)) != 0:
                raise RuntimeError("stream create")
        return torch.cuda.ExternalStream(st.value, device=device)
    except Exception:
        return torch.cuda.Stream(device=device)


TN_SHADOW_WGS = int(os.environ.get("URSE_TN_SHADOW_WGS", "98"))
TN_SHADOW_WGS_NSPLIT = int(os.environ.get("URSE_TN_SHADOW_WGS_NSPLIT", "112"))
TN_SHADOW_WGS_BAND = int(os.environ.get("URSE_TN_SHADOW_WGS_BAND", "84"))
TN_JOIN_LAG = int(os.environ.get("URSE_TN_JOIN_LAG", "2"))
TN_BAND_PARTS = int(os.environ.get("URSE_TN_BAND_PARTS", "-1"))
TN_BAND_PARTS = None if TN_BAND_PARTS < 0 else TN_BAND_PARTS
TN_OVERLAP_TAIL = os.environ.get("URSE_TN_OVERLAP_TAIL", "0") != "0"
DEFER_MASKDEC_WGRADS = os.environ.get("URSE_DEFER_MASKDEC_WGRADS", "0") != "0"
TN_OVERLAP_BAND = os.environ.get("URSE_TN_OVERLAP_BAND", "1") != "0"
WIDE_MIN_SEQ = int(os.environ.get("URSE_LSTM_WIDE_MIN_SEQ", str(64 * 128)))
BAND_PATH_NO_CLUSTER = os.environ.get("URSE_LSTM_BAND_NO_CLUSTER", "0") == "1"


def lstm_fwd_wide(gx, whhb, H, Hp, n_seq, seq_len, inner, outer, stride, save=True):
    M = gx.shape[0]
    ldh = kpad(2 * H, gx.dtype)
    hout = _hout_buffer(M, ldh, H, gx)
    c = torch.empty(M, 2 * H, device=gx.device, dtype=torch.float32)
    timed_call("lstm_fwd_time" if stride > 1 else "lstm_fwd_band", "lstm_wide_fwd", gx, gx.stride(0), whhb, hout, ldh,
               c, H, Hp, n_seq, seq_len, inner, outer, stride, int(save), stream_ptr())
    return hout, (c if save else None)


USE_RW_LSTM = os.environ.get("URSE_LSTM_RW", "1") != "0"
RW_MIN_SEQ = int(os.environ.get("URSE_LSTM_RW_MIN_SEQ", str(16 * 6 * 64)))


def lstm_rw_supported(H, Hp):
    return bool(_lib.load().urse_lstm_rw_supported(H, Hp))


def lstm_fwd_rw(gx, whhb, H, Hp, n_seq, seq_len, inner, outer, stride, save=True, target_wgs=0, paired=False):
    M = gx.shape[0]
    ldh = kpad(2 * H, gx.dtype)
    hout = _hout_buffer(M, ldh, H, gx)
    c = torch.empty(M, 2 * H, device=gx.device, dtype=torch.float32)
    timed_call("lstm_fwd_time" if stride > 1 else "lstm_fwd_band", "lstm_rw_fwd", gx, gx.stride(0), whhb, hout, ldh,
               c, H, Hp, n_seq, seq_len, inner, outer, stride, int(save), int(target_wgs), int(paired), stream_ptr())
    return hout, (c if save else None)


USE_RWX_LSTM = os.environ.get("URSE_LSTM_RWX", "1") != "0"


def lstm_rwx_supported(N, Np, H, Hp):
    return bool(_lib.load().urse_lstm_rwx_supported(N, Np, H, Hp))


def lstm_fwd_rwx(xn, wx, bias, N, H, Hp, n_seq, seq_len, inner, outer, stride, save=True, target_wgs=0, bf16_copy=False):
    M, Np = xn.shape[0], xn.shape[1]
    ldh = kpad(2 * H, xn.dtype)
    hout = _hout_buffer(M, ldh, H, xn)
    hout2 = _hout_buffer(M, ldh, H, xn, torch.bfloat16) if (bf16_copy and xn.dtype == torch.float16 and save) else None
    c = torch.empty(M, 2 * H, device=xn.device, dtype=torch.float32)
    gates = torch.empty(M, 8 * H, device=xn.device, dtype=torch.bfloat16) if save else None
    timed_call("lstm_fwd_time" if stride > 1 else "lstm_fwd_band", "lstm_rwx_fwd", xn, xn.stride(0), wx, bias, gates, 8 * H, hout, ldh, c,
               N, Np, H, Hp, n_seq, seq_len, inner, outer, stride, int(save), int(target_wgs), _dt(xn), hout2, stream_ptr())
    if bf16_copy:
        return gates, hout, (c if save else None), (hout2 if hout2 is not None else hout)
    return gates, hout, (c if save else None)


def lstm_bwd_cluster(dh, gates, c, whhTq, H, Hp, n_seq, seq_len, inner, outer, stride):
    plan = lstm_cluster_plan(H, Hp, n_seq)
    dev = gates.device
    key = ("bwd", dev, H, Hp, n_seq, plan[1], plan[5])
    if key not in _cluster_ws:
        _cluster_ws[key] = (torch.zeros(2 * 2 * plan[1] * 64 * 4 * H, device=dev, dtype=torch.bfloat16),
                            torch.zeros(plan[5], device=dev, dtype=torch.int32),
                            kernel_error_flag(dev))
    dgx, cnt, err = _cluster_ws[key]
    timed_call("lstm_bwd_time" if stride > 1 else "lstm_bwd_band", "lstm_cluster_bwd", dh, dh.stride(0), gates,
               gates.stride(0), c, whhTq, dgx, cnt, err, H, Hp, n_seq, seq_len, inner, outer, stride, reserved_cus(), stream_ptr())
    return gates, err


USE_SPLIT_LSTM_BWD = os.environ.get("URSE_LSTM_SPLIT_BWD", "0") == "1"
SPLIT_BWD_MIN_H = int(os.environ.get("URSE_LSTM_SPLIT_BWD_MIN_H", "512"))


def lstm_split_plan(H, n_seq):
    import ctypes
    if SHARED_GPU_RANKS > 1:
        return None
    plan = (ctypes.c_int64 * 4)()
    if _lib.load().urse_lstm_split_plan(H, n_seq, reserved_cus(), plan) != 0:
        _note_refusal(lambda: _lib.load().urse_lstm_split_plan(H, n_seq, 0, plan) == 0)
        return None
    return list(plan)


SPLIT_BWD_MAX_CHUNKS = int(os.environ.get("URSE_LSTM_SPLIT_BWD_MAX_CHUNKS", "1"))


def lstm_split_chunks(H, n_seq, seq_len, inner, outer, stride):
    if lstm_split_plan(H, n_seq) is not None:
        return [(0, n_seq)]
    if not (inner == 1 and stride == 1 and outer == seq_len):
        return None
    for n in range(2, SPLIT_BWD_MAX_CHUNKS + 1):
        per = (n_seq + n - 1) // n
        if lstm_split_plan(H, per) is not None:
            return [(s0, min(per, n_seq - s0)) for s0 in range(0, n_seq, per)]
    return None


def lstm_bwd_split(dh, gates, c, whhT, H, n_seq, seq_len, inner, outer, stride):
    chunks = lstm_split_chunks(H, n_seq, seq_len, inner, outer, stride)
    dev = gates.device
    err = None
    for s0, n in chunks:
        plan = lstm_split_plan(H, n)
        key = ("split", dev, H, n, plan[2])
        if key not in _cluster_ws:
            _cluster_ws[key] = (torch.empty(plan[2], device=dev, dtype=torch.float32), kernel_error_flag(dev))
        xbuf, err = _cluster_ws[key]
        if len(chunks) == 1:
            d_, g_, c_ = dh, gates, c
        else:
            r0, r1 = s0 * seq_len, (s0 + n) * seq_len
            d_, g_, c_ = dh[r0:r1], gates[r0:r1], c[r0:r1]
        timed_call("lstm_bwd_time" if stride > 1 else "lstm_bwd_band", "lstm_split_bwd", d_, dh.stride(0), g_, gates.stride(0), c_,
                   whhT, xbuf, err, H, n, seq_len, inner, outer, stride, reserved_cus(), stream_ptr())
    return gates, err


USE_NSPLIT_LSTM_BWD = os.environ.get("URSE_LSTM_NSPLIT_BWD", "1") != "0"
NSPLIT_MAX_SEQ = int(os.environ.get("URSE_LSTM_NSPLIT_MAX_SEQ", "2304"))




def _nsplit_reserved():
    return int(COMM_RESERVED_CUS) + int(PREFETCH_RESERVED_CUS)


def lstm_nsplit_plan(H, n_seq):
    import ctypes
    if SHARED_GPU_RANKS > 1:
        return None
    plan = (ctypes.c_int64 * 3)()
    if _lib.load().urse_lstm_nsplit_plan(H, n_seq, _nsplit_reserved(), plan) != 0:
        return None
    return list(plan)


def wgrad_shadow_wgs(path, nsplit):
    if path != "t":
        return TN_SHADOW_WGS_BAND
    return TN_SHADOW_WGS_NSPLIT if nsplit else TN_SHADOW_WGS


def lstm_bwd_nsplit(dh, gates, c, whhT, H, n_seq, seq_len, inner, outer, stride):
    plan = lstm_nsplit_plan(H, n_seq)
    dev = gates.device
    key = ("nsplit", dev, plan[2])
    if key not in _cluster_ws:
        _cluster_ws[key] = (torch.zeros(plan[2], device=dev, dtype=torch.int32), kernel_error_flag(dev))
    flags, err = _cluster_ws[key]
    timed_call("lstm_bwd_time" if stride > 1 else "lstm_bwd_band", "lstm_nsplit_bwd", dh, dh.stride(0), gates, gates.stride(0), c, whhT,
               flags, err, H, n_seq, seq_len, inner, outer, stride, _nsplit_reserved(), stream_ptr())
    return gates, err


BWD_ROWS16 = {k: int(os.environ[e]) for k, e in (("t", "URSE_BWD_ROWS_T"), ("f", "URSE_BWD_ROWS_F")) if e in os.environ}


BAND_TAIL_SPLIT = os.environ.get("URSE_BAND_TAIL_SPLIT", "0") == "1"
BAND_TAIL_EXTRA = int(os.environ.get("URSE_BAND_TAIL_EXTRA", "16"))
_tail_streams = {}


def lstm_bwd(dh, gates, c, whhT, H, n_seq, seq_len, inner, outer, stride, rows16=0):
    tname = "lstm_bwd_time" if stride > 1 else "lstm_bwd_band"
    if BAND_TAIL_SPLIT and gates.is_cuda and rows16 == 0 and inner == 1 and stride == 1 and outer == seq_len and n_seq >= 32 * 128 \
            and gates.dtype == torch.bfloat16:
        per_dir = -(-n_seq // 32)
        full = (2 * per_dir // 256) * 128 - BAND_TAIL_EXTRA
        tail = per_dir - full
        if full > 0 and 0 < tail * 2 <= 192:
            dev = gates.device
            side = _tail_streams.get(dev)
            if side is None:
                side = _tail_streams[dev] = torch.cuda.Stream(device=dev)
            n_main = full * 32
            r0 = n_main * seq_len
            main = torch.cuda.current_stream(dev)
            fork = torch.cuda.Event()
            fork.record(main)
            side.wait_event(fork)
            timed_call(tname, "lstm_bidir_bwd", dh, dh.stride(0), gates, gates.stride(0), c, whhT, H, n_main, seq_len, inner, outer, stride,
                       _dt(gates), 0, stream_ptr())
            with torch.cuda.stream(side):
                call("lstm_bidir_bwd", dh[r0:], dh.stride(0), gates[r0:], gates.stride(0), c[r0:], whhT, H, n_seq - n_main, seq_len, inner,
                     outer, stride, _dt(gates), 1, stream_ptr())
                join = torch.cuda.Event()
                join.record(side)
            main.wait_event(join)
            return gates
    timed_call(tname, "lstm_bidir_bwd", dh, dh.stride(0), gates,
               gates.stride(0), c, whhT, H, n_seq, seq_len, inner, outer, stride, _dt(gates), rows16, stream_ptr())
    return gates


def _once(fn):
    memo = []

    def get():
        if not memo:
            memo.append(fn())
        return memo[0]
    return get


def _fwd_candidates(H, Hp, path, sm, bf16_copy, dtype):
    band = path == "f"
    cluster_ok = USE_CLUSTER_LSTM and not (band and BAND_PATH_NO_CLUSTER)
    cluster = _once(lambda: lstm_cluster_plan(H, Hp, sm["n_seq"]) is not None)
    cx = USE_CLUSTERX_LSTM and cluster_ok and H not in CLUSTER2_H and not (H == 392 and band and not BAND_CLUSTERX)
    return [
        ("clusterx", ("wihq", "whhq"), cx,
         lambda: (band and BAND_CLUSTERX and band_clusterx_pays(H, Hp, sm["n_seq"], sm["seq_len"])) or cluster()),
        ("rwx", ("wx",), USE_RWX_LSTM and USE_RW_LSTM and not (H == 392 and not band),
         lambda: sm["n_seq"] >= RW_MIN_SEQ and not (cluster_ok and cluster())),
        ("clusterx", ("wihq", "whhq"), cx and not band and TIME_CLUSTERX_ROUNDS, lambda: lstm_clusterx_plan(H, Hp, sm["n_seq"]) is not None),
        ("cluster2", ("whhq",), USE_CLUSTER_LSTM and H in CLUSTER2_H,
         lambda: not bf16_copy and lstm_cluster2_chunks(H, Hp, **sm) is not None),
        ("cluster", ("whhq",), cluster_ok and not (dtype == torch.float16 and H in CLUSTER2_H), cluster),
        ("rw", ("whhb",), USE_RW_LSTM and lstm_rw_supported(H, Hp), lambda: sm["n_seq"] >= RW_MIN_SEQ),
        ("wide", ("whhb",), USE_WIDE_LSTM, lambda: sm["n_seq"] >= WIDE_MIN_SEQ),
        ("stream", (), True, lambda: True)]


def _bwd_candidates(H, Hp, path, sm, dtype):
    bf16 = bwd_dtype(dtype) == torch.bfloat16
    return [
        ("cluster", ("whhTq",), USE_CLUSTER_LSTM_BWD, lambda: lstm_cluster_plan(H, Hp, sm["n_seq"]) is not None),
        ("split", (), (USE_SPLIT_LSTM_BWD or H >= SPLIT_BWD_MIN_H) and bf16, lambda: lstm_split_chunks(H, **sm) is not None),
        ("nsplit", (), USE_NSPLIT_LSTM_BWD and bf16 and path not in BWD_ROWS16,
         lambda: sm["n_seq"] <= NSPLIT_MAX_SEQ and sm["n_seq"] * sm["seq_len"] >= 4096 and lstm_nsplit_plan(H, sm["n_seq"]) is not None),
        ("stream", (), True, lambda: True)]


def _static(cands, N, Np, H, Hp, dtype):
    return [(name, lay, runs) for name, lay, ok, runs in cands if ok and all(lstm_layout_ok(x, N, Np, H, Hp, dtype) for x in lay)]


def lstm_fwd_kernel(H, Hp, N, Np, dtype, path, sm, bf16_copy=False):
    return next(name for name, _, runs in _static(_fwd_candidates(H, Hp, path, sm, bf16_copy, dtype), N, Np, H, Hp, dtype) if runs())


def lstm_bwd_kernel(H, Hp, N, Np, dtype, path, sm):
    return next(name for name, _, runs in _static(_bwd_candidates(H, Hp, path, sm, dtype), N, Np, H, Hp, dtype) if runs())


def lstm_layouts(H, Hp, N, Np, dtype, path):
    cands = _fwd_candidates(H, Hp, path, None, False, dtype) + _bwd_candidates(H, Hp, path, None, dtype)
    return {x for _, lay, _ in _static(cands, N, Np, H, Hp, dtype) for x in lay}


import ctypes as _ct


class _MRL1(torch.autograd.Function):
    @staticmethod
    def forward(ctx, estimate, target, windows, eps, td_weight, nan_guard=False):
        B, L = estimate.shape
        dev = estimate.device
        loss = torch.empty(B, device=dev, dtype=torch.float32)
        sums = torch.empty(B * 5, device=dev, dtype=torch.float64)
        acc = torch.empty(B * 2, device=dev, dtype=torch.float64)
        need = estimate.requires_grad
        G = torch.empty(B, L, device=dev, dtype=torch.float32) if need else None
        warr = (_ct.c_int32 * len(windows))(*windows)
        call("mrl1_loss_fwd", target, estimate, loss, G, sums, acc, B, L, warr, len(windows), float(eps),
             float(td_weight), stream_ptr())
        ctx.saved = (estimate, target, G, sums, eps, loss if nan_guard else None)
        return loss

    @staticmethod
    def backward(ctx, gl):
        estimate, target, G, sums, eps, loss = ctx.saved
        B, L = estimate.shape
        de = torch.empty_like(estimate)
        c1 = torch.empty(B, device=estimate.device, dtype=torch.float64)
        if loss is None:
            call("mrl1_loss_bwd", target, estimate, G, sums, _f32c(gl), de, c1, B, L, float(eps), stream_ptr())
        else:
            call("mrl1_loss_bwd_guarded", target, estimate, G, sums, _f32c(gl), loss, de, c1, B, L, float(eps), stream_ptr())
        ctx.saved = None
        return de, None, None, None, None, None


def mr_l1_loss(target, estimate, window_sz=(256, 512, 768, 1024), eps=1e-6, time_domain_weight=0.5, nan_guard=False):
    require_cuda(target, estimate)
    return _MRL1.apply(_f32c(estimate), _f32c(target), tuple(int(w) for w in window_sz), eps, time_domain_weight,
                       bool(nan_guard))


def si_snr_loss(ref, inf):
    require_cuda(ref, inf)
    ref, inf = _f32c(ref.detach()), _f32c(inf.detach())
    B, L = ref.shape
    loss = torch.empty(B, device=ref.device, dtype=torch.float32)
    sums = torch.empty(B * 5, device=ref.device, dtype=torch.float64)
    call("sisnr_fwd", ref, inf, loss, sums, B, L, stream_ptr())
    return loss


class FusedClipAdamW:

    def __init__(self, flat_params, flat_grads, lr=1e-3, betas=(0.9, 0.999), eps=1e-8, weight_decay=1e-6,
                 max_norm=0.5, core=None):
        require_cuda(flat_params, flat_grads)
        n = flat_params.numel()
        self.p, self.g = flat_params, flat_grads[:n]
        self.m = torch.zeros_like(flat_params)
        self.v = torch.zeros_like(flat_params)
        self.lr, self.betas, self.eps, self.wd, self.max_norm = lr, betas, eps, weight_decay, max_norm
        self.step_count = 0
        self.normsq = torch.zeros(1, device=flat_params.device, dtype=torch.float64)
        self.core = core
        if core is not None:
            dev = flat_params.device
            self.slot, self.used, self.n_slot = core.slot_map, core.used_flags, core.n_slot
            assert self.slot.numel() == n and flat_grads.numel() >= n + self.n_slot
            self.slot_steps = torch.zeros(self.n_slot, dtype=torch.int32, device=dev)
            self.bias_corr = torch.zeros(self.n_slot, 2, dtype=torch.float32, device=dev)
            self.skip_flag = kernel_error_flag(dev)

    def step(self, grad_scale=1.0, zero_grad=True):
        n = self.p.numel()
        self.step_count += 1
        call("grad_sumsq", self.g, self.normsq, n, stream_ptr())
        if self.core is not None:
            call("clip_adamw_step_slots", self.p, self.g, self.m, self.v, n, self.normsq, float(self.max_norm or 0.0),
                 float(self.lr), float(self.betas[0]), float(self.betas[1]), float(self.eps), float(self.wd), self.slot,
                 self.used, self.slot_steps, self.bias_corr, self.n_slot, self.skip_flag, float(grad_scale), int(zero_grad),
                 stream_ptr())
            return
        call("clip_adamw_step", self.p, self.g, self.m, self.v, n, self.normsq, float(self.max_norm or 0.0),
             float(self.lr), float(self.betas[0]), float(self.betas[1]), float(self.eps), float(self.wd),
             self.step_count, float(grad_scale), int(zero_grad), stream_ptr())

    def grad_norm(self):
        return self.normsq.sqrt()

    def state_dict(self):
        sd = {"exp_avg": self.m, "exp_avg_sq": self.v, "step": self.step_count, "lr": self.lr}
        if self.core is not None:
            sd["slot_steps"] = self.slot_steps
        return sd

    def load_state_dict(self, sd):
        self.m.copy_(sd["exp_avg"])
        self.v.copy_(sd["exp_avg_sq"])
        self.step_count = int(sd["step"])
        self.lr = float(sd.get("lr", self.lr))
        if self.core is not None:
            if "slot_steps" in sd:
                self.slot_steps.copy_(sd["slot_steps"])
            else:
                self.slot_steps.fill_(self.step_count)
```

Before: 256.3.

## Pair adjacent hidden units in band-path LSTM backward for wider vector loads

Adds a paired variant of the 32-row staged bf16 LSTM backward kernel at H=392. Each lane now handles two adjacent hidden units, so gates, cell state and dh come in as single 16/8/4-byte loads instead of separate narrow loads. Tiles are reassigned across the 8 waves, and a matching permuted recurrent-weight layout (whhTp) is packed, including in the multi-pack path. The paired kernel is on by default for the band (f) path. The cost is an extra weight buffer and pack launch, plus a hand-tuned wave/tile assignment whose load balance may differ from before.

```diff
diff --git a/include/urse.h b/include/urse.h
--- a/include/urse.h
+++ b/include/urse.h
@@ -161,6 +161,13 @@
 int urse_lstm_bidir_bwd(const void* dh, int64_t ldd, void* gates, int64_t ldg, const float* c, const void* whhT,
                         int H, int n_seq, int seq_len, int64_t inner, int64_t outer, int64_t stride, int dtype,
                         int rows16, void* stream);
+int urse_lstm_bwd_paired_supported(int H);
+int urse_lstm_bwd_pair_unit(int assign, int wave, int slot, int lane_col);
+int urse_lstm_pack_bwd_pairs(const float* whh, void* out, int H, void* stream);
+int urse_lstm_pack_bwd_pairs_multi(const void* table, int n_lstm, int H, void* stream);
+int urse_lstm_bidir_bwd_paired(const void* dh, int64_t ldd, void* gates, int64_t ldg, const float* c, const void* whhT, const void* whhTp,
+                               int assign, int H, int n_seq, int seq_len, int64_t inner, int64_t outer, int64_t stride, int dtype,
+                               int rows16, void* stream);
 
 int urse_bandsplit_norm_fwd(const float* spec, const int32_t* bands, const float* gamma, const float* beta, void* xnb,
                             double* stats, int B, int T, int F, int K, int ldx, float eps, int out_dtype,
diff --git a/urgent2026_challenge_track1_amd/bsrnn.py b/urgent2026_challenge_track1_amd/bsrnn.py
--- a/urgent2026_challenge_track1_amd/bsrnn.py
+++ b/urgent2026_challenge_track1_amd/bsrnn.py
@@ -325,7 +325,8 @@
         names = ["l%d%s." % (l, path) for l in range(self.num_layer) for path in "tf"]
         srcs = {p: (self._p(p + "wih", 8 * H * N), self._p(p + "whh", 8 * H * H), self._p(p + "bih", 8 * H), self._p(p + "bhh", 8 * H))
                 for p in names}
-        lays = {path: ops.lstm_layouts(H, d["Hp"], N, d["Np"], dtype, path) for path in "tf"}
+        lays = {path: ops.lstm_layouts(H, d["Hp"], N, d["Np"], dtype, path) | ({"whhTp"} if ops.lstm_bwd_paired(H, d["Hp"], N, d["Np"], dtype, path) else set())
+                for path in "tf"}
         multi = ops.PACK_MULTI and self._flat.is_cuda and all(
             p in self._lstm_bufs and lays[p[-2]] <= self._lstm_bufs[p].keys() and lays[p[-2]] <= ops.PACK_MULTI_LAYOUTS for p in names)
         if multi:
@@ -509,7 +510,7 @@
         elif kern == "nsplit":
             dg, self._cluster_err = ops.lstm_bwd_nsplit(dh, gates, c, pk[p + "whhT"], H, **sm)
         else:
-            dg = ops.lstm_bwd(dh, gates, c, pk[p + "whhT"], H, rows16=ops.BWD_ROWS16.get(path, 0), **sm)
+            dg = ops.lstm_bwd(dh, gates, c, pk[p + "whhT"], H, rows16=ops.BWD_ROWS16.get(path, 0), paired=pk.get(p + "whhTp"), **sm)
         if overlap and path == "t":
             self._join_deferred_wgrads(keep=ops.TN_JOIN_LAG)
         st, L = sm["stride"], sm["seq_len"]
diff --git a/urgent2026_challenge_track1_amd/csrc/lstm.hip b/urgent2026_challenge_track1_amd/csrc/lstm.hip
--- a/urgent2026_challenge_track1_amd/csrc/lstm.hip
+++ b/urgent2026_challenge_track1_amd/csrc/lstm.hip
@@ -225,9 +225,18 @@
   asm volatile("s_mov_b32 m0, %1\n\ts_nop 0\n\tglobal_load_lds_dwordx4 %0, off" :: "v"(gsrc), "s"(dst) : "memory", "m0");
 }
 #pragma clang diagnostic pop
+__host__ __device__ inline int bwd_pair_tile(int assign, int wave, int slot) {
+  if (slot < 2) return 2 * wave + slot;
+  if (assign == 1) return wave < 4 ? 2 * wave + 14 + slot : (wave == 4 && slot == 2 ? 24 : 25);
+  return slot == 2 ? 16 + wave : (wave == 0 ? 24 : 25);
+}
+__host__ __device__ inline int bwd_pair_unit(int tile, int lc) { return tile < 24 ? 32 * (tile >> 1) + 2 * lc + (tile & 1) : tile * 16 + lc; }
+
 template <typename T, int RT, int MAXUT, int NW, int HC = 0, int HPC = 0, int PF = 0, int STG = 0, int KH = 1>
 __global__ void __launch_bounds__(NW * 64) lstm_bwd_kernel(LstmBwdArgs p) {
   static_assert(KH == 1 || (KH == 2 && !HC && !HPC && !PF && !STG), "the half-tile form exists for the plain variant only");
+  constexpr int PAIR = PF == 5 ? 1 : (PF == 6 ? 2 : 0);
+  static_assert(!PAIR || (STG && RT == 2 && MAXUT == 4 && NW == 8 && sizeof(T) == 2 && KH == 1 && HPC == 392 && !HC), "PF 5 / 6: the 32-row staged-store bf16 form at H = 392");
 #ifdef BWSTAMP
   const bool stamp_on = blockIdx.x == BWSTAMP && (threadIdx.x >> 6) == 0;
 #endif
@@ -244,6 +253,10 @@
   const int H = HC ? HC : p.H, nut = (H + 15) >> 4, G4 = 4 * H;
   const int pitch = HPC ? lds_frag_pitch(4 * HPC * ES) : lds_frag_pitch(G4 / KH * ES);
   const int nbuf = (p.dbuf && KH == 1) ? 2 : 1;
+  const int ws = PAIR ? __builtin_amdgcn_readfirstlane(w) : w;
+  int lcv = lc, lrv = lr;
+  auto tile_of = [&](int ui) -> int { if constexpr (PAIR) return bwd_pair_tile(PAIR, ws, ui); else return w + NW * ui; };
+  auto unit_of = [&](int ui) -> int { if constexpr (PAIR) return bwd_pair_unit(tile_of(ui), lcv); else return (w + NW * ui) * 16 + lc; };
   float dcs[MAXUT][RT][4], dhr[MAXUT][RT][4], ccur[MAXUT][RT][4];
   int rowbase[RT][4];
 #pragma unroll
@@ -256,13 +269,22 @@
       const int rb = (int)((seq / p.m.inner) * p.m.outer + (seq % p.m.inner));
       rowbase[rt][r] = ok ? rb : -rb - 1;
     }
-  auto rowb = [&](int rt, int r) -> long { return rowbase[rt][r] >= 0 ? rowbase[rt][r] : -(rowbase[rt][r] + 1); };
+  auto rowb = [&](int rt, int r) -> long {
+    if constexpr (PAIR) {
+      const int* rowtab = reinterpret_cast<const int*>(smem + nbuf * R * pitch);
+      const int g = rowtab[rt * 16 + lr * 4 + r];
+      return g >= 0 ? g : rowtab[0];
+    } else {
+      return rowbase[rt][r] >= 0 ? rowbase[rt][r] : -(rowbase[rt][r] + 1);
+    }
+  };
   if constexpr (STG) {
     int* rowtab = reinterpret_cast<int*>(smem + nbuf * R * pitch);
     if (tid < R) {
       const int seq = s0 + tid;
       rowtab[tid] = seq < p.m.n_seq ? (int)((seq / p.m.inner) * p.m.outer + (seq % p.m.inner)) : -1;
     }
+    if constexpr (PAIR) __syncthreads();
   }
   const int nslab = G4 * ES / 64;
   const char* whhT = reinterpret_cast<const char*>(p.whhT) + ((long)dir * nut * nslab) * 1024 + lane * 16;
@@ -279,7 +301,7 @@
     const long toff0 = (long)(dir ? 0 : p.m.seq_len - 1) * p.m.stride;
 #pragma unroll
     for (int ui = 0; ui < MAXUT; ++ui) {
-      const int u = (w + NW * ui) * 16 + lc;
+      const int u = unit_of(ui);
       const int uc = u < H ? u : H - 1;
 #pragma unroll
       for (int rt = 0; rt < RT; ++rt)
@@ -291,14 +313,14 @@
         }
     }
   }
-  constexpr int PU = PF == 3 ? 2 : (PF == 4 ? 1 : (PF ? MAXUT : 1));
+  constexpr int PU = PF == 3 ? 2 : ((PF == 4 || PAIR) ? 1 : (PF ? MAXUT : 1));
   static_assert(PF != 4 || (STG && RT == 2 && sizeof(T) == 2 && KH == 1 && HPC), "PF 4: the 32-row staged-store bf16 form (row table in LDS)");
   V4 gpf[PU][RT][4];
   float cpf[PU][RT][4];
   T dhpf[PU][RT][4];
   V4 dgk[KH == 2 ? MAXUT : 1][RT][4];
   auto load_step = [&](int ui, int slot, int tt) {
-    const int u = (w + NW * ui) * 16 + lc;
+    const int u = unit_of(ui);
     const bool first_ = dir ? (tt == p.m.seq_len - 1) : (tt == 0);
 #pragma unroll
     for (int rt = 0; rt < RT; ++rt)
@@ -311,7 +333,8 @@
         const int row = rt * 16 + lr * 4 + r + 0 * tt;
 #endif
 #else
-        const int row = (int)rowb(rt, r) + tt * stride_i;
+        int row = (int)rowb(rt, r) + tt * stride_i;
+        if constexpr (PAIR) asm volatile("" : "+v"(row));
 #endif
 #ifdef BABL_NO_P1LOAD
         gpf[slot][rt][r] = V4{}; cpf[slot][rt][r] = (float)row; dhpf[slot][rt][r] = T(row & 1);
@@ -380,18 +403,95 @@
       bw_glds16(reinterpret_cast<const char*>(dh) + ((long)(grow + toff_) * ldd_i + (hcol_i + utd * 16)) * 2 + chc * 16, __builtin_amdgcn_readfirstlane(pfb_u + 6144u));
     }
   };
+  auto cell_bwd = [&](int ui, int rt, int r, V4 g, float cprev, T dhv) __attribute__((always_inline)) -> V4 {
+    float a[4];
+    Vec4<T>::unpack(g, a);
+    const float iv = a[0], fv = a[1], gv = a[2], ov = a[3];
+    const float dht = to_f32<T>(dhv) + dhr[ui][rt][r];
+    const float tc = tanhf_(ccur[ui][rt][r]);
+    float dct, dg[4];
+    if constexpr (PAIR) {
+#pragma clang fp contract(off)
+      dct = __builtin_fmaf(dht * ov, __builtin_fmaf(-tc, tc, 1.f), dcs[ui][rt][r]);
+      dg[0] = dct * gv * iv * (1.f - iv);
+      dg[1] = dct * cprev * fv * (1.f - fv);
+      dg[2] = dct * iv * (1.f - gv * gv);
+      dg[3] = dht * tc * ov * (1.f - ov);
+    } else {
+      dct = dcs[ui][rt][r] + dht * ov * (1.f - tc * tc);
+      dg[0] = dct * gv * iv * (1.f - iv);
+      dg[1] = dct * cprev * fv * (1.f - fv);
+      dg[2] = dct * iv * (1.f - gv * gv);
+      dg[3] = dht * tc * ov * (1.f - ov);
+    }
+    dcs[ui][rt][r] = dct * fv;
+    ccur[ui][rt][r] = cprev;
+    return Vec4<T>::pack(dg);
+  };
   if constexpr (PF == 1) load_all(dir ? 0 : p.m.seq_len - 1);
   if constexpr (PF == 4) __syncthreads();
   for (int step = 0; step < p.m.seq_len; ++step) {
     const int t = dir ? step : (p.m.seq_len - 1 - step);
     char* tile = smem + (step % nbuf) * R * pitch;
     BWST(0);
+    if constexpr (PAIR) {
+      const bool first_ = dir ? (t == p.m.seq_len - 1) : (t == 0);
+      lcv = lc; lrv = lr;
+      asm volatile("" : "+v"(lcv), "+v"(lrv));
+#pragma unroll
+      for (int pi = 0; pi < MAXUT / 2; ++pi) {
+        if (pi == 0 || (PAIR == 1 && ws < 4)) {
+          const int u0 = bwd_pair_unit(tile_of(2 * pi), lcv);
+          uint4 g2[RT][4];
+          float2 c2[RT][4];
+          unsigned d2[RT][4];
+#pragma unroll
+          for (int rt = 0; rt < RT; ++rt)
+#pragma unroll
+            for (int r = 0; r < 4; ++r) {
+              int row = (int)rowb(rt, r) + t * stride_i;
+              asm volatile("" : "+v"(row));
+              g2[rt][r] = *reinterpret_cast<const uint4*>(gates + ((long)row * ldg_i + (gcol_i + u0 * 4)));
+              c2[rt][r] = *reinterpret_cast<const float2*>(p.c + ((long)(row + (first_ ? 0 : prev_i)) * ldc_i + (hcol_i + u0)));
+              d2[rt][r] = *reinterpret_cast<const unsigned*>(dh + ((long)row * ldd_i + (hcol_i + u0)));
+            }
+#pragma unroll
+          for (int rt = 0; rt < RT; ++rt) {
+#pragma unroll
+            for (int r = 0; r < 4; ++r) {
+              const V4 pk0 = cell_bwd(2 * pi, rt, r, V4{g2[rt][r].x, g2[rt][r].y}, first_ ? 0.f : c2[rt][r].x, (T)(d2[rt][r] & 0xffffu));
+              const V4 pk1 = cell_bwd(2 * pi + 1, rt, r, V4{g2[rt][r].z, g2[rt][r].w}, first_ ? 0.f : c2[rt][r].y, (T)(d2[rt][r] >> 16));
+              *reinterpret_cast<uint4*>(tile + (rt * 16 + lrv * 4 + r) * pitch + (u0 * 4) * ES) = uint4{pk0.x, pk0.y, pk1.x, pk1.y};
+              asm volatile("" : "+v"(dcs[2 * pi][rt][r]), "+v"(dcs[2 * pi + 1][rt][r]));
+            }
+          }
+          BWST(1 + 2 * pi);
+          BWST(2 + 2 * pi);
+        } else {
+#pragma unroll
+          for (int ui = 2 * pi; ui < 2 * pi + 2; ++ui) {
+            const int u = unit_of(ui);
+            if (u < H) {
+              load_step(ui, 0, t);
+#pragma unroll
+              for (int rt = 0; rt < RT; ++rt)
+#pragma unroll
+                for (int r = 0; r < 4; ++r) {
+                  *reinterpret_cast<V4*>(tile + (rt * 16 + lrv * 4 + r) * pitch + (u * 4) * ES) = cell_bwd(ui, rt, r, gpf[0][rt][r], cpf[0][rt][r], dhpf[0][rt][r]);
+                  asm volatile("" : "+v"(dcs[ui][rt][r]));
+                }
+            }
+            BWST(1 + ui);
+          }
+        }
+      }
+    }
     if constexpr (PF == 2) load_all(t);
     if constexpr (PF == 3) {
       if (w * 16 + lc < H) load_step(0, 0, t);
     }
 #pragma unroll
-    for (int ui = 0; ui < MAXUT; ++ui) {
+    for (int ui = 0; ui < (PAIR ? 0 : MAXUT); ++ui) {
       const int ut = w + NW * ui;
       if (ut < nut) {
         const int u = ut * 16 + lc;
@@ -431,20 +531,7 @@
           for (int rt = 0; rt < RT; ++rt)
 #pragma unroll
             for (int r = 0; r < 4; ++r) {
-              float a[4];
-              Vec4<T>::unpack(gpre[rt][r], a);
-              const float iv = a[0], fv = a[1], gv = a[2], ov = a[3];
-              const float dht = to_f32<T>(dhpre[rt][r]) + dhr[ui][rt][r];
-              const float tc = tanhf_(ccur[ui][rt][r]);
-              const float dct = dcs[ui][rt][r] + dht * ov * (1.f - tc * tc);
-              float dg[4];
-              dg[0] = dct * gv * iv * (1.f - iv);
-              dg[1] = dct * cpre[rt][r] * fv * (1.f - fv);
-              dg[2] = dct * iv * (1.f - gv * gv);
-              dg[3] = dht * tc * ov * (1.f - ov);
-              dcs[ui][rt][r] = dct * fv;
-              ccur[ui][rt][r] = cpre[rt][r];
-              const V4 pk = Vec4<T>::pack(dg);
+              const V4 pk = cell_bwd(ui, rt, r, gpre[rt][r], cpre[rt][r], dhpre[rt][r]);
               if constexpr (KH == 2) dgk[ui][rt][r] = pk;
               else *reinterpret_cast<V4*>(tile + (rt * 16 + lr * 4 + r) * pitch + (u * 4) * ES) = pk;
 #ifndef BABL_NO_STORE
@@ -543,7 +630,7 @@
 #endif
 #pragma unroll
     for (int ui = 0; ui < MAXUT; ++ui) {
-      const int ut = w + NW * ui;
+      const int ut = tile_of(ui);
       if (ut < nut) {
         f32x4_t acc[RT];
 #pragma unroll
@@ -577,7 +664,10 @@
 #ifndef URSE_BWD_KB3
 #define URSE_BWD_KB3 13
 #endif
-        constexpr int KB = (sizeof(T) == 2) ? (RT >= 3 ? URSE_BWD_KB3 : RT >= 2 ? (PF == 3 ? URSE_BWD_KB2_PF3 : (PF == 4 ? URSE_BWD_KB2_PF4 : (STG ? URSE_BWD_KB2_STG : URSE_BWD_KB2))) : (NW == 8 ? URSE_BWD_KB8 : (PF == 1 ? (NW == 12 ? URSE_BWD_KBPF12 : URSE_BWD_KBPF16) : URSE_BWD_KB))) : 8;
+#ifndef URSE_BWD_KB2_PAIR
+#define URSE_BWD_KB2_PAIR 25
+#endif
+        constexpr int KB = (sizeof(T) == 2) ? (RT >= 3 ? URSE_BWD_KB3 : RT >= 2 ? (PF == 3 ? URSE_BWD_KB2_PF3 : (PF == 4 ? URSE_BWD_KB2_PF4 : (PAIR ? URSE_BWD_KB2_PAIR : (STG ? URSE_BWD_KB2_STG : URSE_BWD_KB2)))) : (NW == 8 ? URSE_BWD_KB8 : (PF == 1 ? (NW == 12 ? URSE_BWD_KBPF12 : URSE_BWD_KBPF16) : URSE_BWD_KB))) : 8;
         #pragma unroll 1
         for (int k0 = 0; k0 < nslab; k0 += KB) {
           uint4 b[KB];
@@ -922,6 +1012,25 @@
   }
 }
 
+template <typename TB, bool PAIRED>
+__device__ __forceinline__ void lstm_pack_whhT_dev(const float* __restrict__ whh, TB* __restrict__ whhT_f, int H, long i0, long stride) {
+  constexpr int ES = sizeof(TB), EPL = 16 / ES, SK = 64 / ES;
+  const int nut = (H + 15) >> 4, G4 = 4 * H;
+  const int nslab = G4 / SK;
+  const long total = (long)2 * nut * nslab * 64 * EPL;
+  for (long idx = i0; idx < total; idx += stride) {
+    long q = idx;
+    const int j = (int)(q % EPL); q /= EPL;
+    const int lane = (int)(q % 64); q /= 64;
+    const int ks = (int)(q % nslab); q /= nslab;
+    const int ut = (int)(q % nut);
+    const int d = (int)(q / nut);
+    const int n = PAIRED ? bwd_pair_unit(ut, lane & 15) : ut * 16 + (lane & 15), kk = ks * SK + EPL * (lane >> 4) + j;
+    const int up = kk >> 2, gp = kk & 3;
+    whhT_f[idx] = from_f32<TB>(n < H ? whh[((long)d * G4 + gp * H + up) * H + n] : 0.f);
+  }
+}
+
 template <typename T, typename TB = T>
 __device__ __forceinline__ void lstm_pack_dev(const float* __restrict__ wih, const float* __restrict__ whh,
                                               const float* __restrict__ bih, const float* __restrict__ bhh,
@@ -966,20 +1075,16 @@
       whh_f[idx] = from_f32<T>((u < H && k < H) ? whh[((long)d * G4 + g * H + u) * H + k] : 0.f);
     }
   } else {
-    const int nslab = G4 / SK;
-    const long total = (long)2 * nut * nslab * 64 * EPL;
-    for (long idx = i0; idx < total; idx += stride) {
-      long q = idx;
-      const int j = (int)(q % EPL); q /= EPL;
-      const int lane = (int)(q % 64); q /= 64;
-      const int ks = (int)(q % nslab); q /= nslab;
-      const int ut = (int)(q % nut);
-      const int d = (int)(q / nut);
-      const int n = ut * 16 + (lane & 15), kk = ks * SK + EPL * (lane >> 4) + j;
-      const int up = kk >> 2, gp = kk & 3;
-      whhT_f[idx] = from_f32<TB>(n < H ? whh[((long)d * G4 + gp * H + up) * H + n] : 0.f);
-    }
-  }
+    lstm_pack_whhT_dev<TB, false>(whh, whhT_f, H, i0, stride);
+  }
+}
+
+__global__ void __launch_bounds__(256) lstm_pack_bwd_pairs_kernel(const float* __restrict__ whh, bf16_t* __restrict__ out, int H) {
+  lstm_pack_whhT_dev<bf16_t, true>(whh, out, H, (long)blockIdx.x * blockDim.x + threadIdx.x, (long)gridDim.x * blockDim.x);
+}
+__global__ void __launch_bounds__(256) lstm_pack_bwd_pairs_multi_kernel(const PackRow* __restrict__ tab, int H) {
+  const PackRow r = tab[blockIdx.y];
+  if (r.whhTp) lstm_pack_whhT_dev<bf16_t, true>(r.whh, (bf16_t*)r.whhTp, H, (long)blockIdx.x * blockDim.x + threadIdx.x, (long)gridDim.x * blockDim.x);
 }
 
 template <typename T, typename TB = T>
@@ -1031,7 +1136,7 @@
 #endif
 
 template <typename T, int RT, int NW>
-static int launch_bwd(const LstmBwdArgs& p, hipStream_t st) {
+static int launch_bwd(const LstmBwdArgs& p, hipStream_t st, const void* whhTp = nullptr, int assign = 0) {
   constexpr int R = 16 * RT;
   size_t lds = (size_t)R * lds_frag_pitch(4 * p.H * (int)sizeof(T));
   if constexpr (sizeof(T) == 4 && RT == 1 && NW == 16) {
@@ -1098,7 +1203,18 @@
         hipLaunchKernelGGL((lstm_bwd_kernel<T, 2, 4, 8, 0, 392, 4, 1>), grid, dim3(NW * 64), lds + R * sizeof(int) + NW * 7168, st, pa);
       } else
 #endif
-      if (stg) {
+      if (stg && whhTp && (assign == 1 || assign == 2) && p.ldd % 2 == 0 && (reinterpret_cast<uintptr_t>(p.dh) % 4) == 0 && (reinterpret_cast<uintptr_t>(p.c) % 8) == 0) {
+        pa.whhT = whhTp;
+        if (assign == 1) {
+          static bool once = (allow_big_lds(lstm_bwd_kernel<T, 2, 4, 8, 0, 392, 5, 1>), true);
+          (void)once;
+          hipLaunchKernelGGL((lstm_bwd_kernel<T, 2, 4, 8, 0, 392, 5, 1>), grid, dim3(NW * 64), lds + R * sizeof(int), st, pa);
+        } else {
+          static bool once = (allow_big_lds(lstm_bwd_kernel<T, 2, 4, 8, 0, 392, 6, 1>), true);
+          (void)once;
+          hipLaunchKernelGGL((lstm_bwd_kernel<T, 2, 4, 8, 0, 392, 6, 1>), grid, dim3(NW * 64), lds + R * sizeof(int), st, pa);
+        }
+      } else if (stg) {
         static bool once = (allow_big_lds(lstm_bwd_kernel<T, 2, 4, 8, 0, 392, 0, 1>), true);
         (void)once;
         hipLaunchKernelGGL((lstm_bwd_kernel<T, 2, 4, 8, 0, 392, 0, 1>), grid, dim3(NW * 64), lds + R * sizeof(int), st, pa);
@@ -1269,9 +1385,8 @@
   return launch_fwd<float, 1, 16>(p, st);
 }
 
-extern "C" int urse_lstm_bidir_bwd(const void* dh, int64_t ldd, void* gates, int64_t ldg, const float* c,
-                                   const void* whhT, int H, int n_seq, int seq_len, int64_t inner, int64_t outer,
-                                   int64_t stride, int dtype, int rows16, void* stream) {
+static int bidir_bwd(const void* dh, int64_t ldd, void* gates, int64_t ldg, const float* c, const void* whhT, const void* whhTp, int assign, int H,
+                     int n_seq, int seq_len, int64_t inner, int64_t outer, int64_t stride, int dtype, int rows16, void* stream) {
   URSE_CHECK_ARG(dh && gates && c && whhT, "urse_lstm_bidir_bwd: null pointer");
   LstmBwdArgs p;
   p.dh = dh; p.ldd = ldd; p.gates = gates; p.ldg = ldg; p.c = c; p.whhT = whhT; p.H = H;
@@ -1301,11 +1416,48 @@
 #endif
   note_launch(dtype == URSE_BF16 && rt >= 2 && fits2 ? URSE_KV_LSTM_BWD_STREAM32 : URSE_KV_LSTM_BWD_STREAM16);
   if (dtype == URSE_BF16) {
-    if (nw8) return (rt >= 2 && fits2) ? launch_bwd<bf16_t, 2, 8>(p, st) : launch_bwd<bf16_t, 1, 8>(p, st);
+    if (nw8) return (rt >= 2 && fits2) ? launch_bwd<bf16_t, 2, 8>(p, st, whhTp, assign) : launch_bwd<bf16_t, 1, 8>(p, st);
     if (rt >= 2 && fits2) return launch_bwd<bf16_t, 2, 16>(p, st);
     return launch_bwd<bf16_t, 1, 16>(p, st);
   }
   return launch_bwd<float, 1, 16>(p, st);
+}
+
+extern "C" int urse_lstm_bidir_bwd(const void* dh, int64_t ldd, void* gates, int64_t ldg, const float* c,
+                                   const void* whhT, int H, int n_seq, int seq_len, int64_t inner, int64_t outer,
+                                   int64_t stride, int dtype, int rows16, void* stream) {
+  return bidir_bwd(dh, ldd, gates, ldg, c, whhT, nullptr, 0, H, n_seq, seq_len, inner, outer, stride, dtype, rows16, stream);
+}
+
+extern "C" int urse_lstm_bidir_bwd_paired(const void* dh, int64_t ldd, void* gates, int64_t ldg, const float* c, const void* whhT,
+                                          const void* whhTp, int assign, int H, int n_seq, int seq_len, int64_t inner, int64_t outer,
+                                          int64_t stride, int dtype, int rows16, void* stream) {
+  URSE_CHECK_ARG(whhTp && (assign == 1 || assign == 2) && H == 392 && dtype == URSE_BF16,
+                 "urse_lstm_bidir_bwd_paired: needs whhTp, assignment 1 | 2, H = 392, bf16 (H=%d assign=%d dtype=%d)", H, assign, dtype);
+  return bidir_bwd(dh, ldd, gates, ldg, c, whhT, whhTp, assign, H, n_seq, seq_len, inner, outer, stride, dtype, rows16, stream);
+}
+
+extern "C" int urse_lstm_bwd_paired_supported(int H) { return H == 392; }
+
+extern "C" int urse_lstm_bwd_pair_unit(int assign, int wave, int slot, int lane_col) {
+  if ((assign != 1 && assign != 2) || wave < 0 || wave >= 8 || slot < 0 || slot >= 4 || lane_col < 0 || lane_col >= 16) return -1;
+  const int tile = bwd_pair_tile(assign, wave, slot);
+  const int u = tile < 25 ? bwd_pair_unit(tile, lane_col) : -1;
+  return u < 392 ? u : -1;
+}
+
+extern "C" int urse_lstm_pack_bwd_pairs(const float* whh, void* out, int H, void* stream) {
+  URSE_CHECK_ARG(whh && out && H == 392, "urse_lstm_pack_bwd_pairs: null pointer or H != 392 (H=%d)", H);
+  hipLaunchKernelGGL(lstm_pack_bwd_pairs_kernel, dim3(256), dim3(256), 0, (hipStream_t)stream, whh, (bf16_t*)out, H);
+  URSE_CHECK_LAUNCH("urse_lstm_pack_bwd_pairs");
+  return URSE_OK;
+}
+
+extern "C" int urse_lstm_pack_bwd_pairs_multi(const void* table, int n_lstm, int H, void* stream) {
+  URSE_CHECK_ARG(table && n_lstm > 0 && n_lstm < 65536 && H == 392, "urse_lstm_pack_bwd_pairs_multi: bad argument (H=%d)", H);
+  hipLaunchKernelGGL(lstm_pack_bwd_pairs_multi_kernel, dim3(256, (unsigned)n_lstm), dim3(256), 0, (hipStream_t)stream, (const PackRow*)table, H);
+  URSE_CHECK_LAUNCH("urse_lstm_pack_bwd_pairs_multi");
+  return URSE_OK;
 }
 
 #ifdef BWSTAMP
diff --git a/urgent2026_challenge_track1_amd/csrc/urse_common.h b/urgent2026_challenge_track1_amd/csrc/urse_common.h
--- a/urgent2026_challenge_track1_amd/csrc/urse_common.h
+++ b/urgent2026_challenge_track1_amd/csrc/urse_common.h
@@ -133,6 +133,7 @@
   void* wih_p; void* wihT_p; float* bias; void* whh_f; void* whhT_f;
   void* whhq; void* whhb; void* wx;
   void* wihq;
+  void* whhTp;
 };
 
 }
diff --git a/urgent2026_challenge_track1_amd/ops.py b/urgent2026_challenge_track1_amd/ops.py
--- a/urgent2026_challenge_track1_amd/ops.py
+++ b/urgent2026_challenge_track1_amd/ops.py
@@ -281,8 +281,8 @@
     return dy, sums
 
 
-LSTM_LAYOUTS = ("whhq", "wihq", "whhb", "wx", "whhTq")
-PACK_MULTI_LAYOUTS = {"whhq", "wihq", "whhb", "wx"}
+LSTM_LAYOUTS = ("whhq", "wihq", "whhb", "wx", "whhTq", "whhTp")
+PACK_MULTI_LAYOUTS = {"whhq", "wihq", "whhb", "wx", "whhTp"}
 
 
 def lstm_layout_ok(name, N, Np, H, Hp, dtype):
@@ -297,6 +297,8 @@
         return bool(lib.urse_lstm_rwx_supported(N, Np, H, Hp))
     if dtype != torch.bfloat16:
         return False
+    if name == "whhTp":
+        return bool(lib.urse_lstm_bwd_paired_supported(H))
     if name == "whhb":
         return bool(lib.urse_lstm_wide_supported(H, Hp))
     return name == "whhTq" and H % 8 == 0
@@ -332,6 +334,8 @@
     if want("whhTq"):
         C = ((H + 3) // 4 + 13) // 14
         call("lstm_pack_bwd_quads", whh, buf("whhTq", 2 * C * 4 * (H // 8) * 512), H, C, stream_ptr())
+    if want("whhTp"):
+        call("lstm_pack_bwd_pairs", whh, buf("whhTp", 2 * nu * 4 * H), H, stream_ptr())
     return out
 
 
@@ -344,7 +348,7 @@
     dev = entries[0][0].device
     ptr = lambda t: 0 if t is None else t.data_ptr()
     rows = [[ptr(wih), ptr(whh), ptr(bih), ptr(bhh), ptr(o["wih"]), ptr(o["wihT"]), ptr(o["bias"]), ptr(o["whh"]), ptr(o["whhT"]),
-             ptr(o.get("whhq")), ptr(o.get("whhb")), ptr(o.get("wx")), ptr(o.get("wihq"))] for wih, whh, bih, bhh, o in entries]
+             ptr(o.get("whhq")), ptr(o.get("whhb")), ptr(o.get("wx")), ptr(o.get("wihq")), ptr(o.get("whhTp"))] for wih, whh, bih, bhh, o in entries]
     if table is None or table[1] != rows:
         table = (upload(torch.tensor(rows, dtype=torch.int64), dev, cached=True), rows)
     n = len(rows)
@@ -359,6 +363,8 @@
         call("lstm_pack_blocks_x_multi", table[0], n, N, Np, H, Hp, fdt, stream_ptr())
     if any(r[12] for r in rows):
         call("lstm_pack_quads_x_multi", table[0], n, N, Np, H, fdt, stream_ptr())
+    if any(r[13] for r in rows):
+        call("lstm_pack_bwd_pairs_multi", table[0], n, H, stream_ptr())
     return table
 
 
@@ -817,8 +823,12 @@
 _tail_streams = {}
 
 
-def lstm_bwd(dh, gates, c, whhT, H, n_seq, seq_len, inner, outer, stride, rows16=0):
+def lstm_bwd(dh, gates, c, whhT, H, n_seq, seq_len, inner, outer, stride, rows16=0, paired=None, assign=None):
     tname = "lstm_bwd_time" if stride > 1 else "lstm_bwd_band"
+    if paired is not None:
+        timed_call(tname, "lstm_bidir_bwd_paired", dh, dh.stride(0), gates, gates.stride(0), c, whhT, paired, assign or BWD_BAND_PAIRED or 1, H, n_seq,
+                   seq_len, inner, outer, stride, _dt(gates), rows16, stream_ptr())
+        return gates
     if BAND_TAIL_SPLIT and gates.is_cuda and rows16 == 0 and inner == 1 and stride == 1 and outer == seq_len and n_seq >= 32 * 128 \
             and gates.dtype == torch.bfloat16:
         per_dir = -(-n_seq // 32)
@@ -888,6 +898,13 @@
         ("stream", (), True, lambda: True)]
 
 
+BWD_BAND_PAIRED = int(os.environ.get("URSE_BWD_BAND_PAIRED", "1"))
+
+
+def lstm_bwd_paired(H, Hp, N, Np, dtype, path):
+    return BWD_BAND_PAIRED in (1, 2) and path == "f" and dtype == torch.bfloat16 and lstm_layout_ok("whhTp", N, Np, H, Hp, dtype)
+
+
 def _static(cands, N, Np, H, Hp, dtype):
     return [(name, lay, runs) for name, lay, ok, runs in cands if ok and all(lstm_layout_ok(x, N, Np, H, Hp, dtype) for x in lay)]
 
```

Measured after the change: 257.0, median of 2. No clear change (+0.3%).
